# wvangansbeke/LaneDetection_End2End

Hardware: AMD Instinct MI355X
Metric: images/sec fwd+bwd, 256x512 2-lane bs32 (higher is better)
Workload: dtype f32; 1 GPU; BEV ERFNet + fused WLS fit + Area loss, 2 lanes, 256x512, batch 32 per GPU, fp32, train mode (BN batch stats, Dropout2d on), fwd+bwd, optimizer excluded; global_batch=32, parallelism=dp1, grad_allreduce=none

## Files before the change

### lanedetection_end2end_amd/_lib.py

```python
import ctypes
import os
from ctypes import c_char_p, c_double, c_int, c_long, c_size_t, c_void_p

import torch

_HERE = os.path.dirname(os.path.abspath(__file__))
LIB_PATH = os.path.join(_HERE, "liblanefit_hip.so")
_lib = None


class LaneFitLibraryError(RuntimeError):
    pass


def _declare(lib):
    P, I, L, D = c_void_p, c_int, c_long, c_double
    sig = {
        "lf_abi_version": (c_int, []),
        "lf_last_error": (c_char_p, []),
        "lf_wls_workspace_bytes": (c_size_t, [I, I, I]),
        "lf_wls_fwd": (I, [P, P, L, I, I, I, I, I, I, D, D, I, I, P, P, P, P, P, P]),
        "lf_wls_bwd": (I, [P, P, L, I, I, I, I, I, I, D, I, P, P, P, P, P]),
        "lf_gels_workspace_bytes": (c_size_t, [I, I]),
        "lf_gels_fwd": (I, [P, P, I, L, I, P, P, P, P, P]),
        "lf_gels_bwd": (I, [P, P, P, P, P, I, L, I, P, P, P]),
        "lf_area_loss": (I, [P, L, P, I, I, I, I, P, P, P]),
        "lf_mse_loss": (I, [P, P, L, I, P, P, P]),
        "lf_backproj_loss": (I, [P, L, P, P, P, P, P, I, I, I, P, P, P, P]),
        "lf_ce2d_fwd": (I, [P, P, P, I, I, I, I, P, P, P]),
        "lf_ce2d_bwd": (I, [P, P, P, I, I, I, I, P, P, P, P]),
        "lf_erfnet_plan_create": (P, [I, I, I, I, I, I]),
        "lf_erfnet_plan_destroy": (None, [P]),
        "lf_erfnet_workspace_bytes": (c_size_t, [P]),
        "lf_erfnet_workspace_bytes_for": (c_size_t, [P, I]),
        "lf_erfnet_activation_floats": (L, [P]),
        "lf_erfnet_num_params": (I, [P]),
        "lf_erfnet_num_bn": (I, [P]),
        "lf_erfnet_num_dropout": (I, [P]),
        "lf_erfnet_dropmask_floats": (L, [P]),
        "lf_erfnet_dropmask_offset": (L, [P, I]),
        "lf_erfnet_dropmask_channels": (I, [P, I]),
        "lf_erfnet_encoder_offset": (L, [P]),
        "lf_erfnet_activation_offset": (L, [P, I, I]),
        "lf_erfnet_bn_vector_offset": (L, [P, I, I, I]),
        "lf_erfnet_forward": (I, [P, P, P, P, P, P, I, I, P, P, c_size_t, P]),
        "lf_erfnet_backward": (I, [P, P, P, P, P, P, P, I, I, P, c_size_t, P]),
        "lf_convchain_plan_create": (P, [I, I, I, I, P, P]),
        "lf_convchain_plan_destroy": (None, [P]),
        "lf_convchain_workspace_bytes": (c_size_t, [P]),
        "lf_convchain_forward": (I, [P, P, P, P, P, I, ctypes.c_float, ctypes.c_float, P, P, c_size_t, P]),
        "lf_convchain_backward": (I, [P, P, P, P, P, P, P, I, P, c_size_t, P]),
        "lf_poolflat_fwd": (I, [P, I, I, I, I, I, P, P]),
        "lf_poolflat_bwd": (I, [P, P, I, I, I, I, I, P, P]),
        "lf_convchain_workspace_bytes_for": (c_size_t, [P, I]),
        "lf_convchain_set_precision": (I, [P, I]),
        "lf_poolflat_bf16_fwd": (I, [P, I, I, I, I, I, P, P]),
        "lf_poolflat_bf16_bwd": (I, [P, P, I, I, I, I, I, P, P]),
        "lf_lane_decode": (I, [P, P, P, P, D, P, P, D, D, D, I, I, I, I, P, P, P]),
        "lf_trapezoid": (I, [P, P, I, D, D, I, I, P, P]),
        "lf_pipeline_plan_create": (P, [I, I, I, I, I, I]),
        "lf_pipeline_plan_destroy": (None, [P]),
        "lf_pipeline_table_bytes": (c_size_t, [P]),
        "lf_pipeline_upload": (I, [P, P, P]),
        "lf_pipeline_tables_host": (I, [P, P, P, P, P, P, P, P, P]),
        "lf_pipeline_image": (I, [P, P, I, P, P, P, P]),
        "lf_pipeline_label": (I, [P, P, I, P, P, I, P, P, P, P]),
        "lf_pipeline_image_indexed": (I, [P, P, L, P, I, P, P, P, P, P]),
        "lf_pipeline_label_indexed": (I, [P, P, L, P, I, P, P, I, P, P, P, P, P]),
        "lf_nhwc_to_nchw": (I, [P, P, I, I, I, I, P]),
        "lf_pointwise_fwd": (I, [P, P, P, P, I, I, I, I, I, P]),
        "lf_pointwise_scratch_floats": (L, [I, I, I, I, I]),
        "lf_pointwise_bwd": (I, [P, P, P, P, P, P, I, I, I, I, I, P, P]),
        "lf_pointwise_bf16_fwd": (I, [P, P, P, P, I, I, I, I, I, P]),
        "lf_pointwise_bf16_bwd": (I, [P, P, P, P, P, P, I, I, I, I, I, P, P]),
        "lf_adam_chunk": (I, []),
        "lf_adam_step": (I, [P, P, I, ctypes.c_float, ctypes.c_float, ctypes.c_float, ctypes.c_float, ctypes.c_float,
                             I, ctypes.c_float, P]),
        "lf_sgd_step": (I, [P, P, I, ctypes.c_float, ctypes.c_float, ctypes.c_float, ctypes.c_float, P]),
        "lf_rmsprop_step": (I, [P, P, I, ctypes.c_float, ctypes.c_float, ctypes.c_float, ctypes.c_float, ctypes.c_float,
                                ctypes.c_float, P]),
        "lf_conv1d_scratch_floats": (L, [I, I, I, I]),
        "lf_conv1d_fwd": (I, [P, P, P, P, I, I, I, I, I, I, I, P, P]),
        "lf_conv1d_bwd_data": (I, [P, P, P, P, I, I, I, I, I, I, P, P]),
        "lf_conv1d_bwd_weight": (I, [P, P, P, P, I, I, I, I, I, I, P, P]),
        "lf_erfnet_num_layers": (I, [P]),
        "lf_erfnet_range_workspace_bytes": (c_size_t, [P, I, I]),
        "lf_erfnet_layer_io": (I, [P, I, P]),
        "lf_erfnet_forward_range": (I, [P, I, I, I, P, P, P, P, P, I, P, P, c_size_t, P]),
        "lf_erfnet_backward_range": (I, [P, I, I, I, P, P, P, P, P, I, P, P, c_size_t, P]),
        "lf_linear_fwd": (I, [P, P, P, P, I, I, I, I, P]),
        "lf_linear_bwd": (I, [P, P, P, P, P, P, P, I, I, I, I, P]),
        "lf_seg_maps": (I, [P, P, P, I, I, I, I, I, I, P]),
        "lf_erfnet_set_precision": (I, [P, I]),
        "lf_erfnet_profile": (I, [P, I]),
        "lf_erfnet_profile_read": (I, [P, P, c_char_p]),
        "lf_erfnet_infer_workspace_bytes": (c_size_t, [P, I]),
        "lf_erfnet_infer_encoder_offset": (L, [P]),
        "lf_erfnet_infer": (I, [P, P, P, P, P, I, P, P, c_size_t, P]),
        "lf_erfnet_infer_range_workspace_bytes": (c_size_t, [P, I, I, I]),
        "lf_erfnet_infer_range": (I, [P, I, I, I, P, P, P, P, P, P, c_size_t, P]),
        "lf_convchain_infer_workspace_bytes": (c_size_t, [P, I]),
        "lf_convchain_infer": (I, [P, P, P, P, P, ctypes.c_float, P, P, c_size_t, P]),
        "lf_head_fit": (I, [P, I, P, P, P, L, I, I, I, I, I, I, D, D, I, I, P, P, P, P, P, P]),
        "lf_lane_infer_workspace_bytes": (c_size_t, [P, I, I, I]),
        "lf_lane_infer": (I, [P, P, P, P, P, P, L, I, I, D, D, I, I, P, P, P, P, c_size_t, P]),
        "lf_theta_grid": (I, [P, L, P, P, I, I, I, P, P]),
        "lf_theta_grid_bwd_workspace_bytes": (c_size_t, [I]),
        "lf_theta_grid_bwd": (I, [P, L, P, P, P, I, I, I, P, P, P]),
        "lf_wls_fwd_theta": (I, [P, P, L, P, P, I, I, I, I, I, I, D, D, I, I, P, P, P, P, P, P]),
        "lf_wls_bwd_theta_workspace_bytes": (c_size_t, [I, I]),
        "lf_wls_bwd_theta": (I, [P, P, L, P, P, I, I, I, I, I, I, D, I, P, P, P, P, P, P, P]),
        "lf_wls_bwd_grid": (I, [P, P, L, I, I, I, I, I, I, D, I, P, P, P, P, P]),
        "lf_lane_eval": (I, [P, P, P, P, P, P, L, P, I, I, I, I, I, D, D, P, P, P, P, P, P]),
        "lf_lane_decode_bev": (I, [P, I, P, P, P, P, L, P, P, I, D, P, P, I, I, I, I, I, I, I, I, I, I, P, P, P]),
        "lf_step_loss_workspace_bytes": (c_size_t, []),
        "lf_step_loss": (I, [I, I, I, I, I, I, I, P, L, I, P, P, L, I, P, P, P, P, P, P, P, I, D, D, P, P, P, P, P, P]),
        "lf_step_loss_bwd": (I, [P, I, L, L, P, P, P]),
        "lf_seg_step_workspace_bytes": (c_size_t, [I, I, I, I, I, I]),
        "lf_seg_step": (I, [P, P, P, P, L, P, I, I, I, I, I, I, I, D, D, I, P, P, P, P, P, P, P, P]),
        "lf_seg_step_bwd": (I, [P, L, P, P]),
        "lf_label_batch_bp": (I, [P, P, P, P, P, P, P, L, P, P, I, I, P, P, P, P, P, P, P, P, P]),
        "lf_label_batch_bev": (I, [P, P, P, P, P, L, P, P, I, P, P, P, P, P, P, P]),
    }
    dbg = {
        "lf_debug_set_split_any_size": (None, [I]),
        "lf_debug_set_bf16_lds": (None, [I]),
        "lf_debug_set_bf16_no_partial_fast": (None, [I]),
        "lf_debug_stride2_epi": (I, [I, I, P, P, P, P, I, P, P, P, P, I, I, I, I, I, P, P]),
        "lf_debug_stride2_wgrad_scratch_floats": (L, [I, I, I, I, I, I, I]),
        "lf_debug_stride2_wgrad": (I, [I, I, P, P, P, P, I, I, I, I, I, P, P]),
        "lf_debug_stem_wgrad_scratch_floats": (L, [I, I, I, I]),
        "lf_debug_stem_wgrad": (I, [I, P, P, P, P, I, I, I, I, P, P]),
        "lf_debug_head_wgrad_scratch_floats": (L, [I, I, I, I]),
        "lf_debug_head_wgrad": (I, [I, P, P, P, P, I, I, I, I, P, P]),
        "lf_debug_set_ops_precision": (None, [I]),
        "lf_debug_conv1d_fwd_phases": (I, [P, P, P, P, I, I, I, I, I, I, P, P, P]),
        "lf_debug_conv1d_wgrad_phases": (I, [P, P, I, I, I, I, I, I, P, P, P]),
        "lf_debug_conv1d_fwd_pro": (I, [P, P, P, P, P, P, I, I, I, I, I, I, P, P]),
        "lf_debug_set_wgrad_ro": (None, [I, I, I]),
        "lf_debug_set_fp32_stream": (None, [I, I]),
        "lf_debug_conv1d_bwd_data_epi3": (I, [P, P, P, P, P, P, P, I, I, I, I, I, I, P, P]),
        "lf_debug_conv1d_epi": (I, [P, P, P, P, I, I, P, P, P, P, P, P, I, I, I, I, I, I, P, P]),
        "lf_debug_conv1d_wgrad_pro": (I, [P, P, P, P, P, P, I, I, I, I, I, I, P, P]),
        "lf_debug_bias_residual_launches": (L, []),
        "lf_debug_partial_fast_launches": (L, []),
    }
    for table in (sig, dbg):
        for name, (res, args) in table.items():
            fn = getattr(lib, name)
            fn.restype = res
            fn.argtypes = args
    return sig


def exported_symbols():
    return list(_declare(load()).keys()) + list(_extra_symbols)


_extra_symbols = []


def load():
    global _lib
    if _lib is None:
        if not os.path.exists(LIB_PATH):
            raise LaneFitLibraryError(
                "%s not found: build it with `python -m lanedetection_end2end_amd.build` "
                "(there is no fallback path)" % LIB_PATH)
        lib = ctypes.CDLL(LIB_PATH)
        _declare(lib)
        _lib = lib
    return _lib


def check(rc, what):
    if rc != 0:
        raise LaneFitLibraryError("%s failed: %s" % (what, load().lf_last_error().decode()))


def ptr(t, rows=False):
    if t is None:
        return None
    if not t.is_cuda:
        raise LaneFitLibraryError("lanefit ops need tensors on the MI355X (got a %s tensor); "
                                  "there is no CPU path" % t.device)
    if rows:
        assert t.dim() == 2 and t.stride(1) == 1, "internal: tensor rows must be contiguous"
    else:
        assert t.is_contiguous(), "internal: tensor must be contiguous"
    return c_void_p(t.data_ptr())


def stream():
    return c_void_p(torch.cuda.current_stream().cuda_stream)


class DeferredRead:

    def __init__(self, t):
        if t.is_cuda:
            self.host = torch.empty(t.shape, dtype=t.dtype, pin_memory=True)
            self.host.copy_(t, non_blocking=True)
            self.event = torch.cuda.Event()
            self.event.record()
        else:
            self.host = t.detach().clone()
            self.event = None

    def ready(self):
        return self.event is None or self.event.query()

    def get(self):
        if self.event is not None:
            self.event.synchronize()
        return self.host
```

### lanedetection_end2end_amd/csrc/lf_conv.h

```cpp
#pragma once
#include "lf_common.h"

#define LF_MAX_TAPS 9
struct TapIdx { int v[LF_MAX_TAPS]; };

struct LfTapGeom {
    int N, Hl, Wl;
    int Hs, Ws, s_pix, s_choff;
    int ssh, ssw;
    int Hd, Wd, d_pix, d_choff;
    int dsh, dsw, dah, daw;
    int Cs, Cd;
    int ntaps;
    int tdh[LF_MAX_TAPS], tdw[LF_MAX_TAPS];
};

enum { LF_PRO_NONE = 0, LF_PRO_BNRELU = 1 };
enum {
    LF_EPI_RELU = 1,
    LF_EPI_MASK = 2,
    LF_EPI_ADD = 4,
    LF_EPI_STATS_SQ = 8,
    LF_EPI_MASKBN = 16,
    LF_EPI_STATS_XHAT = 32,
    LF_EPI_BIAS = 64
};

struct LfTapArgs {
    const float* src;
    const float* wp;
    int s16;
    const void* wp16;
    int split;
    const void* wp48;
    const float* bias;
    float* dst;
    const float* pro_sc;
    const float* pro_sh;
    const float* mask_src;
    const float* add_src;
    const float* aux;
    const float* msc;
    const float* msh;
    const float* asc;
    const float* ash;
    const float* dm;
    float* stats;
    int stats_ld;
    unsigned long long* dbg;
};

void lf_tapgemm_set_split_any_size(int v);
void lf_tapgemm_set_bf16_lds(int v);
void lf_tapgemm_set_bf16_no_partial_fast(int v);
long lf_tapgemm_partial_fast_launches();
void lf_tapgemm_set_fp32_stream(int mode, int max_workgroups);
int lf_tapgemm_stat_rows(const LfTapGeom& g);
int lf_tapgemm_stat_rows_for(const LfTapGeom& g, const LfTapArgs& a);
int lf_tapgemm_launch(const LfTapGeom& g, const LfTapArgs& a, int pro, int epi, hipStream_t st);
int lf_tapgemm_launch_unordered(const LfTapGeom& g, const LfTapArgs& a, int pro, int epi, hipStream_t st);

struct LfWgradArgs {
    const float* x;
    const float* g;
    const float* pro_sc;
    const float* pro_sh;
    int s16;
    int split;
    float* partial;
    float* bias_partial;
    unsigned long long* dbg = nullptr;
};
int lf_tapwgrad_splits(const LfTapGeom& g);
int lf_tapwgrad_splits_bound(const LfTapGeom& g, int s16);
int lf_tapwgrad_splits_for(const LfTapGeom& g, const LfWgradArgs& a, int pro);
int lf_tapwgrad_launch(const LfTapGeom& g, const LfWgradArgs& a, int pro, hipStream_t st);

bool lf_tapwgrad_ro_ok(const LfTapGeom& g, int s16);
int lf_tapwgrad_ro_rows_bound(const LfTapGeom& g);
int lf_tapwgrad_ro_rows(const LfTapGeom& g);
int lf_tapwgrad_ro_launch(const LfTapGeom& g, const LfWgradArgs& a, int pro, hipStream_t st);
void lf_tapwgrad_ro_set(int mode, int cap64, int cap128);

int lf_wgrad_reduce_launch(const float* partial, int splits, int ntaps, int Cs, int Cd, float* grad, long sk, long sn,
                           const int* tapidx_host, const float* bias_rows, int n_bias_rows, float* bias_grad,
                           int bias_accumulate, hipStream_t st);
#define LF_REDUCE_BATCH 32
struct LfReduceJob {
    const float* partial; float* grad; const float* bias_rows; float* bias_grad;
    long sk, sn;
    int splits, ntaps, Cs, Cd, n_bias_rows;
    int tapidx[LF_MAX_TAPS];
};
int lf_wgrad_reduce_batch_launch(const LfReduceJob* jobs_host, int njobs, hipStream_t st);
int lf_rows_reduce_launch(const float* rows, int nrows, int C, float* dst, int accumulate, hipStream_t st);

struct LfPackEntry {
    long src_off;
    long dst_off;
    int Kc, Nc, ntaps;
    long sk, sn;
    int tapidx[LF_MAX_TAPS];
    int param;
    long dst16_off;
};
int lf_pack_weights_launch(const LfPackEntry* entries_dev, int nentries, const float* const* params_dev, float* arena,
                           hipStream_t st);
long lf_pack_bf16_elems(int Kc, int Nc, int ntaps);
int lf_pack_weights_split_launch(const LfPackEntry* entries_dev, int nentries, const float* const* params_dev, void* arena48,
                                 hipStream_t st);
bool lf_tapgemm_split_ok(const LfTapGeom& g);
long lf_tapgemm_bias_residual_launches();

struct LfFoldEntry {
    LfPackEntry pk;
    int ch_off, C;
    const float* gamma;
    const float* beta;
    const float* mean;
    const float* var;
    const float* bias;
    long out_off;
};
int lf_fold_pack_launch(const LfFoldEntry* entries_dev, int nentries, const float* const* params_dev, float eps, float* vec, float* arena,
                        void* arena16, void* arena48, hipStream_t st);
int lf_pack_weights_bf16_launch(const LfPackEntry* entries_dev, int nentries, const float* const* params_dev, void* arena16,
                                hipStream_t st);
```

### lanedetection_end2end_amd/csrc/lf_conv.hip

```cpp
#include <stdlib.h>
#include <string.h>

#include <atomic>
#include <map>
#include <mutex>
#include <tuple>
#include <type_traits>
#include <utility>

#include <hip/hip_ext.h>

#include "lf_conv.h"
#include "lf_ldsdma.h"
#include "lf_types.h"

typedef float f32x4 __attribute__((ext_vector_type(4)));

namespace {

constexpr int MT = 4;
constexpr int WG_WAVES = 4;
constexpr int PIX_PER_WG = WG_WAVES * MT * 16;

__device__ __forceinline__ f32x4 ldg4(const float* p) { return *reinterpret_cast<const f32x4*>(p); }
// ... 1834 lines not shown
                const int sy = pi[m] * g.ssh + dh, sx = pj[m] * g.ssw + dw;
                in3[t][m] = pv[m] && sy >= 0 && sy < g.Hs && sx >= 0 && sx < g.Ws;
                const int syc = min(max(sy, 0), g.Hs - 1), sxc = min(max(sx, 0), g.Ws - 1);
                const unsigned off = (unsigned)(((pn[m] * g.Hs + syc) * g.Ws + sxc) * g.s_pix + g.s_choff + kq * 4) * 4u;
                x3[t][m] = ldb4(rxl, (PROC == 0 && !in3[t][m]) ? LF_OOB : off, 0u);
            }
        }
        f32x4 sc = zero4(), sh = zero4();
        if (pro == LF_PRO_BNRELU) { sc = ldg4(a.pro_sc + kq * 4); sh = ldg4(a.pro_sh + kq * 4); }
#pragma unroll
        for (int t = 0; t < 3; ++t) {
            if constexpr (PROC != 0) {
#pragma unroll
                for (int m = 0; m < MT; ++m) {
                    f32x4 v = x3[t][m];
                    if (pro == LF_PRO_BNRELU) v = max0(v * sc + sh);
                    v.x = in3[t][m] ? v.x : 0.f; v.y = in3[t][m] ? v.y : 0.f; v.z = in3[t][m] ? v.z : 0.f; v.w = in3[t][m] ? v.w : 0.f;
                    x3[t][m] = v;
                }
            }
            f32x4 part[NT][MT];
#pragma unroll
            for (int s4 = 0; s4 < 4; ++s4)
#pragma unroll
                for (int n = 0; n < NT; ++n)
#pragma unroll
                    for (int m = 0; m < MT; ++m)
                        part[n][m] = __builtin_amdgcn_mfma_f32_16x16x4f32(w3[t][n][s4], x3[t][m][s4], s4 ? part[n][m] : zero4(), 0, 0, 0);
#pragma unroll
            for (int n = 0; n < NT; ++n)
#pragma unroll
                for (int m = 0; m < MT; ++m) acc[n][m] = t ? acc[n][m] + part[n][m] : part[n][m];
        }
    } else
    for (int t = 0; t < g.ntaps; ++t) {
        const int dh = g.tdh[t], dw = g.tdw[t];
        unsigned xo[MT];
        bool in[MT];
#pragma unroll
        for (int m = 0; m < MT; ++m) {
            const int sy = pi[m] * g.ssh + dh, sx = pj[m] * g.ssw + dw;
            in[m] = pv[m] && sy >= 0 && sy < g.Hs && sx >= 0 && sx < g.Ws;
            const int syc = min(max(sy, 0), g.Hs - 1), sxc = min(max(sx, 0), g.Ws - 1);
            xo[m] = (unsigned)(((pn[m] * g.Hs + syc) * g.Ws + sxc) * g.s_pix + g.s_choff + kq * 4);
        }
        for (int cg = 0; cg < ncg; ++cg) {
            f32x4 w[NT], x[MT];
#pragma unroll
            for (int n = 0; n < NT; ++n) w[n] = ldg4(wp + n * 64);
            wp += (long)g.Cd * 16;
#pragma unroll
            for (int m = 0; m < MT; ++m) x[m] = ldg4(a.src + xo[m] + cg * 16);
            if (pro == LF_PRO_BNRELU) {
                const f32x4 sc = ldg4(a.pro_sc + cg * 16 + kq * 4), sh = ldg4(a.pro_sh + cg * 16 + kq * 4);
#pragma unroll
                for (int m = 0; m < MT; ++m) x[m] = max0(x[m] * sc + sh);
            }
#pragma unroll
            for (int m = 0; m < MT; ++m) {
                x[m].x = in[m] ? x[m].x : 0.f; x[m].y = in[m] ? x[m].y : 0.f;
                x[m].z = in[m] ? x[m].z : 0.f; x[m].w = in[m] ? x[m].w : 0.f;
            }
            if ((cg & 1) == 0) {
#pragma unroll
                for (int n = 0; n < NT; ++n)
#pragma unroll
                    for (int m = 0; m < MT; ++m) { acc[n][m] += seg[n][m]; seg[n][m] = zero4(); }
            }
#pragma unroll
            for (int s = 0; s < 4; ++s)
#pragma unroll
                for (int n = 0; n < NT; ++n)
#pragma unroll
                    for (int m = 0; m < MT; ++m)
                        seg[n][m] = __builtin_amdgcn_mfma_f32_16x16x4f32(w[n][s], x[m][s], seg[n][m], 0, 0, 0);
        }
    }
    if (!(g.Cs == 16 && g.ntaps == 3)) {
#pragma unroll
        for (int n = 0; n < NT; ++n)
#pragma unroll
            for (int m = 0; m < MT; ++m) acc[n][m] += seg[n][m];
    }
    LF_TAPGEMM_EPILOGUE
}

int g_split_any_size = 0;
std::atomic<long> g_bres_launches{0};
int g_bf16_lds = 4;
std::atomic<long> g_part_fast_launches{0};
int g_bf16_no_partial_fast = 0;

int pick_nt(int Cd) {
    const int tiles = Cd / 16;
    if (tiles % 4 == 0) return 4;
    if (tiles % 3 == 0) return 3;
    if (tiles % 2 == 0) return 2;
    return 1;
}

}

void lf_tapgemm_set_split_any_size(int v) { g_split_any_size = v; }
long lf_tapgemm_bias_residual_launches() { return g_bres_launches.load(); }
void lf_tapgemm_set_bf16_lds(int v) { g_bf16_lds = v; }
void lf_tapgemm_set_bf16_no_partial_fast(int v) { g_bf16_no_partial_fast = v; }
long lf_tapgemm_partial_fast_launches() { return g_part_fast_launches.load(); }

bool lf_tapgemm_split_ok(const LfTapGeom& g) {
    const long npix = (long)g.N * g.Hl * g.Wl;
    const long wgs = npix / (2 * PIX_PER_WG) * (g.Cd / 64);
    return g.Cs % 32 == 0 && g.Cd % 64 == 0 && g.s_pix % 4 == 0 && g.s_choff % 4 == 0 && npix % (2 * PIX_PER_WG) == 0 &&
           (wgs >= 192 || g_split_any_size);
}

int lf_tapgemm_stat_rows(const LfTapGeom& g) {
    const long npix = (long)g.N * g.Hl * g.Wl;
    return lf_cdiv(npix, PIX_PER_WG);
}
int lf_tapgemm_stat_rows_for(const LfTapGeom& g, const LfTapArgs& a) {
    (void)a;
    return lf_cdiv((long)g.N * g.Hl * g.Wl, PIX_PER_WG);
}

namespace {
std::mutex g_launch_state_mutex;
int current_device() {
    int dev = 0;
    return hipGetDevice(&dev) == hipSuccess ? dev : -1;
}
template <typename K>
int resident_workgroups(K kernel, size_t lds, int block = 256) {
    static std::map<std::tuple<int, const void*, size_t>, int> cache;
    const int dev = current_device();
    const std::tuple<int, const void*, size_t> key(dev, reinterpret_cast<const void*>(kernel), lds);
    std::lock_guard<std::mutex> lock(g_launch_state_mutex);
    auto it = cache.find(key);
    if (it != cache.end()) return it->second;
    int cus = 0, nb = 0;
    if (dev < 0 || hipDeviceGetAttribute(&cus, hipDeviceAttributeMultiprocessorCount, dev) != hipSuccess ||
        hipOccupancyMaxActiveBlocksPerMultiprocessor(&nb, kernel, block, lds) != hipSuccess || nb < 1 || cus < 1)
        return cache[key] = 1 << 30;
    return cache[key] = nb * cus;
}
bool allow_big_lds(const void* kernel, int bytes) {
    static std::map<std::pair<int, const void*>, bool> done;
    const std::pair<int, const void*> key(current_device(), kernel);
    std::lock_guard<std::mutex> lock(g_launch_state_mutex);
    auto it = done.find(key);
    if (it != done.end()) return it->second;
    return done[key] = hipFuncSetAttribute(kernel, hipFuncAttributeMaxDynamicSharedMemorySize, bytes) == hipSuccess;
}
thread_local unsigned g_launch_flags = 0;
template <typename K, typename... Args>
bool launch_resident(K kernel, dim3 grid, unsigned block, size_t lds, int lds_attr, unsigned max_wgs, unsigned flags, hipStream_t st, const Args&... args) {
    if (lds_attr > 0 && !allow_big_lds(reinterpret_cast<const void*>(kernel), lds_attr)) return false;
    const unsigned res = (unsigned)resident_workgroups(kernel, lds, (int)block) / grid.y;
    if (grid.x > res && res >= 8) grid.x = res & ~7u;
    if (max_wgs > 0 && grid.x > max_wgs) grid.x = max_wgs;
    if (flags) hipExtLaunchKernelGGL(kernel, grid, dim3(block), (unsigned)lds, st, nullptr, nullptr, flags, args...);
    else hipLaunchKernelGGL(kernel, grid, dim3(block), lds, st, args...);
    return true;
}
constexpr int BIG_LDS = 160 * 1024 - 4096;
template <typename K>
void launch_tapgemm(K kernel, dim3 grid, size_t lds, hipStream_t st, const LfTapGeom& g, const LfTapArgs& a, int pro, int epi) {
    launch_resident(kernel, grid, 256, lds, 0, 0, g_launch_flags, st, g, a, pro, epi);
}
template <int EPIV, bool DBGV = false>
void launch_bf16_ring(unsigned nitems, hipStream_t st, const LfTapGeom& g, const LfTapArgs& a, int pro, int epi) {
    launch_resident(tapgemm_bf16_ring_kernel<EPIV, DBGV>, dim3(nitems), 256, (size_t)LB_STAGES * LB_STAGE_BYTES, 0, 0, 0, st, g, a, pro, epi);
}
template <int CBV, int EPIV, int PROV = 0>
bool launch_bf16_wl(unsigned nitems, hipStream_t st, const LfTapGeom& g, const LfTapArgs& a, int pro, int epi) {
    return launch_resident(tapgemm_bf16_wl_kernel<CBV, EPIV, PROV>, dim3(nitems), 256, WlCfg<CBV, EPIV, PROV>::LDS, BIG_LDS, 0, 0, st, g, a, pro, epi);
}
template <int EPIV>
bool launch_bf16_wv(unsigned ntiles, hipStream_t st, const LfTapGeom& g, const LfTapArgs& a, int pro, int epi) {
    return launch_resident(tapgemm_bf16_wv_kernel<EPIV>, dim3(ntiles), 256, WvCfg<EPIV>::LDS, BIG_LDS, 0, 0, st, g, a, pro, epi);
}
std::atomic<int> g_stream_mode{1}, g_stream_cap{0};
enum { LF_STREAM_RELU = 1, LF_STREAM_STATS = 2, LF_STREAM_MASK = 4, LF_STREAM_PRO = 8, LF_STREAM_X48 = 16, LF_STREAM_X38 = 32 };
constexpr int g_stream_routed[2] = {LF_STREAM_RELU | LF_STREAM_STATS | LF_STREAM_MASK | LF_STREAM_PRO | LF_STREAM_X48 | LF_STREAM_X38,
                                    0};
template <int CS, int PROV, int EPIV>
bool launch_tapstream(hipStream_t st, const LfTapGeom& g, const LfTapArgs& a) {
    constexpr int G = CS == 128 ? 2 : 1;
    const size_t lds = (size_t)3 * (CS / 16) * 4096 + (PROV == LF_PRO_BNRELU ? 2 * CS * sizeof(float) : 0);
    const unsigned ntiles = (unsigned)lf_cdiv((long)g.N * g.Hl * g.Wl, PIX_PER_WG);
    return launch_resident(tapstream_kernel<CS, PROV, EPIV, G>, dim3((ntiles + G - 1) / G, CS / 64), 256 * G, lds, BIG_LDS,
                           (unsigned)g_stream_cap.load(), g_launch_flags, st, g, a);
}
template <int CS>
bool route_tapstream(int variant, hipStream_t st, const LfTapGeom& g, const LfTapArgs& a) {
    switch (variant) {
        case LF_STREAM_RELU: return launch_tapstream<CS, 0, LF_EPI_RELU>(st, g, a);
        case LF_STREAM_STATS: return launch_tapstream<CS, 0, LF_EPI_STATS_SQ>(st, g, a);
        case LF_STREAM_MASK: return launch_tapstream<CS, 0, LF_EPI_MASK>(st, g, a);
        case LF_STREAM_PRO: return launch_tapstream<CS, 1, LF_EPI_RELU>(st, g, a);
        case LF_STREAM_X48: if constexpr (CS == 64) return launch_tapstream<CS, 0, LF_EPI_MASKBN | LF_EPI_STATS_XHAT>(st, g, a); else return false;
        case LF_STREAM_X38: if constexpr (CS == 64) return launch_tapstream<CS, 0, LF_EPI_ADD | LF_EPI_MASK | LF_EPI_STATS_XHAT>(st, g, a); else return false;
        default: return false;
    }
}

constexpr int BRES = LF_EPI_ADD | LF_EPI_RELU | LF_EPI_BIAS;
template <int V> using IntC = std::integral_constant<int, V>;
template <bool WITH_BRES, typename F>
auto with_epi(int epis, F&& f) {
    switch (epis) {
        case 0: return f(IntC<0>{});
        case LF_EPI_RELU: return f(IntC<LF_EPI_RELU>{});
        case LF_EPI_MASK: return f(IntC<LF_EPI_MASK>{});
        case LF_EPI_ADD: return f(IntC<LF_EPI_ADD>{});
        case LF_EPI_STATS_SQ: return f(IntC<LF_EPI_STATS_SQ>{});
        case LF_EPI_MASK | LF_EPI_STATS_XHAT: return f(IntC<LF_EPI_MASK | LF_EPI_STATS_XHAT>{});
        case LF_EPI_ADD | LF_EPI_MASK | LF_EPI_STATS_XHAT: return f(IntC<LF_EPI_ADD | LF_EPI_MASK | LF_EPI_STATS_XHAT>{});
        case LF_EPI_MASKBN | LF_EPI_STATS_XHAT: return f(IntC<LF_EPI_MASKBN | LF_EPI_STATS_XHAT>{});
        case BRES: return f(IntC<WITH_BRES ? BRES : -1>{});
        default: return f(IntC<-1>{});
    }
}
template <bool WITH_BRES, typename F>
void with_pro_epi(int pro, int epi, int epis, F&& f) {
    if (pro == LF_PRO_BNRELU && epi == LF_EPI_RELU) f(IntC<1>{}, IntC<LF_EPI_RELU>{});
    else if (pro == LF_PRO_BNRELU) f(IntC<1>{}, IntC<-1>{});
    else with_epi<WITH_BRES>(epis, [&](auto e) { f(IntC<0>{}, e); });
}

int launch_split_route(const LfTapGeom& g, const LfTapArgs& a, int pro, int epi, int epis, long npix, hipStream_t st) {
    LF_REQUIRE(a.split == 9, "tapgemm: split must be 9 (got %d; the 6-term form was removed in round 6)", a.split);
    LfTapArgs b = a;
    b.wp16 = a.wp48;
    const dim3 grid2((unsigned)(npix / (2 * PIX_PER_WG)), g.Cd / 64);
    if (a.dbg) {
        LF_REQUIRE(pro == LF_PRO_NONE && epi == 0, "tapgemm: phase stamps are compiled into the plain convolution only");
        hipLaunchKernelGGL((tapgemm_split_kernel<4, 0, 0, true>), grid2, dim3(512), 0, st, g, b, pro, epi);
    } else {
        with_pro_epi<false>(pro, epi, epis, [&](auto p, auto e) {
            hipLaunchKernelGGL((tapgemm_split_kernel<4, decltype(p)::value, decltype(e)::value>), grid2, dim3(512), 0, st, g, b, pro, epi);
        });
    }
    LF_CHECK_LAUNCH("tapgemm_split");
    return 0;
}

template <int NTV, int PROV, int EPIV = -1, bool FAST = false>
void launch_bf16_stream(dim3 grid, hipStream_t st, const LfTapGeom& g, const LfTapArgs& a, int pro, int epi) {
    hipLaunchKernelGGL((tapgemm_bf16_kernel<NTV, PROV, EPIV, FAST>), grid, dim3(256), 0, st, g, a, pro, epi);
}
template <int NTV>
void launch_bf16_stream_rt(dim3 grid, hipStream_t st, const LfTapGeom& g, const LfTapArgs& a, int pro, int epi) {
    if (pro == LF_PRO_BNRELU) launch_bf16_stream<NTV, 1>(grid, st, g, a, pro, epi);
    else launch_bf16_stream<NTV, 0>(grid, st, g, a, pro, epi);
}

int launch_bf16_route(const LfTapGeom& g, const LfTapArgs& a, int pro, int epi, int epis, long npix, int nt, dim3 grid, hipStream_t st) {
    LF_REQUIRE(a.s16, "tapgemm: the bf16 matrix-core kernels take bf16 tensors (s16); bf16 operands on fp32 tensors were removed in round 6");
    LF_REQUIRE(g.Cs >= 8 && g.s_pix >= g.s_choff + 8, "tapgemm bf16: needs at least 8 source channels");
    const bool in_offsets = (long)g.N * g.Hs * g.Ws * g.s_pix * 2 < (long)LF_OOB;
    if (a.s16 && g_bf16_lds >= 3 && !a.dbg && g.Cs == 16 && g.Cd == 16 && g.ntaps == 3 && g.Wl % 16 == 0 && g.s_pix % 8 == 0 && g.s_choff % 8 == 0 && in_offsets) {
        with_epi<true>(epis, [&](auto e) {
            constexpr int E = decltype(e)::value;
            if (pro == LF_PRO_BNRELU) hipLaunchKernelGGL((tapgemm_bf16_lean_kernel<1, E>), grid, dim3(256), 0, st, g, a, pro, epi);
            else hipLaunchKernelGGL((tapgemm_bf16_lean_kernel<0, E>), grid, dim3(256), 0, st, g, a, pro, epi);
        });
        if (epis == BRES) ++g_bres_launches;
        LF_CHECK_LAUNCH("tapgemm_bf16_lean");
        return 0;
    }
    const bool fast16 = nt == 4 && a.s16 && pro != LF_PRO_BNRELU && g.Cs % 32 == 0 && in_offsets;
    const bool fast16p = nt == 4 && a.s16 && pro == LF_PRO_BNRELU && epi == LF_EPI_RELU && g.Cs == 128 && in_offsets;
    const bool line3 = g_bf16_lds >= 3 && !a.dbg && g.ntaps == 3 && g.Cs == g.Cd && (g.Cd == 64 || g.Cd == 128) && g.Wl % 16 == 0 &&
                       g.ssh == 1 && g.ssw == 1 && g.dsh == 1 && g.dsw == 1 && g.dah == 0 && g.daw == 0 && g.Hs == g.Hl && g.Ws == g.Wl &&
                       g.Hd == g.Hl && g.Wd == g.Wl && g.s_pix % 8 == 0 && g.s_choff % 8 == 0 && g.d_pix % 8 == 0 && g.d_choff % 8 == 0 &&
                       (long)g.N * g.Hd * g.Wd * g.d_pix * 2 < (long)LF_OOB;
    const bool wv = line3 && g_bf16_lds == 4 && g.Cd == 64 && fast16;
    const bool wl = line3 && (fast16 || fast16p);
    const unsigned ntiles = (unsigned)lf_cdiv(npix, PIX_PER_WG);
    if (wv) {
        const bool launched = with_epi<true>(epis, [&](auto e) {
            constexpr int E = decltype(e)::value;
            if constexpr (E == (LF_EPI_ADD | LF_EPI_MASK | LF_EPI_STATS_XHAT)) return false;
            else return launch_bf16_wv<E>(ntiles, st, g, a, pro, epi);
        });
        if (launched) {
            if (epis == BRES) ++g_bres_launches;
            LF_CHECK_LAUNCH("tapgemm_bf16_wv");
            return 0;
        }
    }
    if (wl && fast16p) {
        if (launch_bf16_wl<4, LF_EPI_RELU, 1>(ntiles, st, g, a, pro, epi)) {
            LF_CHECK_LAUNCH("tapgemm_bf16_wl (prologue)");
            return 0;
        }
    } else if (wl) {
        const bool launched = with_epi<true>(epis, [&](auto e) {
            constexpr int E = decltype(e)::value;
            return g.Cs == 128 ? launch_bf16_wl<4, E>(ntiles, st, g, a, pro, epi) : launch_bf16_wl<2, E>(ntiles, st, g, a, pro, epi);
        });
        if (launched) {
            if (epis == BRES) ++g_bres_launches;
            LF_CHECK_LAUNCH("tapgemm_bf16_wl");
            return 0;
        }
    }
    const bool part_fast = !g_bf16_no_partial_fast && g.ntaps * ((g.Cs + 31) / 32) <= LF_MAX_TAPS;
    const bool ring = fast16 && g_bf16_lds >= 2 && g.Wl % 16 == 0 && g.Cd % 64 == 0;
    const unsigned nitems = ntiles * (unsigned)(g.Cd / 64);
    if (ring && a.dbg) {
        LF_REQUIRE(epis == 0, "tapgemm bf16 ring: stamps are compiled into the plain convolution only");
        launch_bf16_ring<0, true>(nitems, st, g, a, pro, epi);
    } else if (ring) {
        with_epi<false>(epis, [&](auto e) { launch_bf16_ring<decltype(e)::value>(nitems, st, g, a, pro, epi); });
    } else if (fast16) {
        with_epi<false>(epis, [&](auto e) { launch_bf16_stream<4, 0, decltype(e)::value, true>(grid, st, g, a, pro, epi); });
    } else if (nt == 4 && a.s16 && pro != LF_PRO_BNRELU && g.Cs == 16 && (epis == (LF_EPI_MASK | LF_EPI_STATS_XHAT) || epis == 0) && part_fast && in_offsets) {
        if (epis == 0) launch_bf16_stream<4, 0, 0, true>(grid, st, g, a, pro, epi);
        else launch_bf16_stream<4, 0, LF_EPI_MASK | LF_EPI_STATS_XHAT, true>(grid, st, g, a, pro, epi);
        ++g_part_fast_launches;
    } else if (nt == 3 && a.s16 && pro != LF_PRO_BNRELU && g.Cs == 16 && (epis == LF_EPI_STATS_SQ || epis == LF_EPI_RELU || epis == 0) && part_fast && in_offsets) {
        if (epis == 0) launch_bf16_stream<3, 0, 0, true>(grid, st, g, a, pro, epi);
        else if (epis == LF_EPI_RELU) launch_bf16_stream<3, 0, LF_EPI_RELU, true>(grid, st, g, a, pro, epi);
        else launch_bf16_stream<3, 0, LF_EPI_STATS_SQ, true>(grid, st, g, a, pro, epi);
        ++g_part_fast_launches;
    } else if (nt == 4 && a.s16 && pro == LF_PRO_BNRELU && epi == LF_EPI_RELU) {
        launch_bf16_stream<4, 1, LF_EPI_RELU, false>(grid, st, g, a, pro, epi);
    } else if (nt == 1 && a.s16 && pro != LF_PRO_BNRELU && ((g.Cs + 31) / 32 * 32 + g.s_choff <= g.s_pix) && in_offsets &&
               (g.Cs % 32 == 0 || part_fast) &&
               (epis == 0 || epis == LF_EPI_STATS_SQ || epis == LF_EPI_ADD || epis == LF_EPI_RELU)) {
        if (epis == 0) launch_bf16_stream<1, 0, 0, true>(grid, st, g, a, pro, epi);
        else if (epis == LF_EPI_STATS_SQ) launch_bf16_stream<1, 0, LF_EPI_STATS_SQ, true>(grid, st, g, a, pro, epi);
        else if (epis == LF_EPI_RELU) launch_bf16_stream<1, 0, LF_EPI_RELU, true>(grid, st, g, a, pro, epi);
        else launch_bf16_stream<1, 0, LF_EPI_ADD, true>(grid, st, g, a, pro, epi);
        if (g.Cs % 32 != 0) ++g_part_fast_launches;
    } else {
        switch (nt) {
            case 4: launch_bf16_stream_rt<4>(grid, st, g, a, pro, epi); break;
            case 3: launch_bf16_stream_rt<3>(grid, st, g, a, pro, epi); break;
            case 2: launch_bf16_stream_rt<2>(grid, st, g, a, pro, epi); break;
            default: launch_bf16_stream_rt<1>(grid, st, g, a, pro, epi); break;
        }
    }
    LF_CHECK_LAUNCH("tapgemm_bf16");
    return 0;
}

template <int NTV>
void launch_tapgemm_rt(dim3 grid, size_t tap_lds, hipStream_t st, const LfTapGeom& g, const LfTapArgs& a, int pro, int epi) {
    if (pro == LF_PRO_BNRELU) launch_tapgemm(tapgemm_kernel<NTV, 1>, grid, tap_lds, st, g, a, pro, epi);
    else launch_tapgemm(tapgemm_kernel<NTV, 0>, grid, tap_lds, st, g, a, pro, epi);
}

int launch_fp32_route(const LfTapGeom& g, const LfTapArgs& a, int pro, int epi, int epis, int nt, dim3 grid, hipStream_t st) {
    const size_t tap_lds = LF_TAP_LDS_PER_TAP * g.ntaps;
    if (a.dbg) {
        LF_REQUIRE(nt == 4 && pro == LF_PRO_NONE && epi == 0 && !a.wp16, "tapgemm: phase stamps are compiled into the plain fp32 convolution only");
        if ((g.Wl & 63) == 0) hipLaunchKernelGGL((tapgemm_kernel<4, 0, 0, true, true>), grid, dim3(256), tap_lds, st, g, a, pro, epi);
        else hipLaunchKernelGGL((tapgemm_kernel<4, 0, 0, false, true>), grid, dim3(256), tap_lds, st, g, a, pro, epi);
        LF_CHECK_LAUNCH("tapgemm (stamps)");
        return 0;
    }
    if (g_stream_mode.load() != 0 && nt == 4 && g.ntaps == 3 && g.Cs == g.Cd && (g.Cs == 64 || g.Cs == 128) && (g.Wl & 63) == 0) {
        const int variant = pro == LF_PRO_BNRELU ? (epi == LF_EPI_RELU ? LF_STREAM_PRO : 0)
                          : epis == LF_EPI_RELU ? LF_STREAM_RELU : epis == LF_EPI_STATS_SQ ? LF_STREAM_STATS : epis == LF_EPI_MASK ? LF_STREAM_MASK
                          : epis == (LF_EPI_MASKBN | LF_EPI_STATS_XHAT) ? LF_STREAM_X48 : epis == (LF_EPI_ADD | LF_EPI_MASK | LF_EPI_STATS_XHAT) ? LF_STREAM_X38 : 0;
        if (variant && (g_stream_mode.load() == 2 || (g_stream_routed[g.Cs == 128] & variant)) &&
            (g.Cs == 64 ? route_tapstream<64>(variant, st, g, a) : route_tapstream<128>(variant, st, g, a))) {
            LF_CHECK_LAUNCH("tapstream");
            return 0;
        }
    }
    switch (nt) {
        case 4:
            with_pro_epi<true>(pro, epi, epis, [&](auto p, auto e) {
                constexpr int P = decltype(p)::value, E = decltype(e)::value;
                if ((g.Wl & 63) == 0) launch_tapgemm(tapgemm_kernel<4, P, E, true>, grid, tap_lds, st, g, a, pro, epi);
                else launch_tapgemm(tapgemm_kernel<4, P, E, false>, grid, tap_lds, st, g, a, pro, epi);
                if constexpr (E == BRES) ++g_bres_launches;
            });
            break;
        case 3: launch_tapgemm_rt<3>(grid, tap_lds, st, g, a, pro, epi); break;
        case 2: launch_tapgemm_rt<2>(grid, tap_lds, st, g, a, pro, epi); break;
        default:
            with_pro_epi<true>(pro, epi, epis, [&](auto p, auto e) {
                constexpr int P = decltype(p)::value, E = decltype(e)::value;
                hipLaunchKernelGGL((tapgemm_lean_kernel<1, P, E>), grid, dim3(256), 0, st, g, a, pro, epi);
                if constexpr (E == BRES) ++g_bres_launches;
            });
            break;
    }
    LF_CHECK_LAUNCH("tapgemm");
    return 0;
}
}

void lf_tapgemm_set_fp32_stream(int mode, int max_workgroups) { g_stream_mode = mode; g_stream_cap = max_workgroups > 0 ? max_workgroups : 0; }

int lf_tapgemm_launch_unordered(const LfTapGeom& g, const LfTapArgs& a, int pro, int epi, hipStream_t st) {
    g_launch_flags = hipExtAnyOrderLaunch;
    const int rc = lf_tapgemm_launch(g, a, pro, epi, st);
    g_launch_flags = 0;
    return rc;
}

int lf_tapgemm_launch(const LfTapGeom& g, const LfTapArgs& a, int pro, int epi, hipStream_t st) {
    LF_REQUIRE(g.Cs % 16 == 0 && g.Cd % 16 == 0, "tapgemm: channels must be multiples of 16 (Cs=%d Cd=%d)", g.Cs, g.Cd);
    LF_REQUIRE(g.s_pix % 4 == 0 && g.s_choff % 4 == 0 && g.d_pix % 4 == 0 && g.d_choff % 4 == 0, "tapgemm: unaligned channel layout");
    LF_REQUIRE(g.ntaps >= 1 && g.ntaps <= LF_MAX_TAPS, "tapgemm: bad tap count %d", g.ntaps);
    const long npix = (long)g.N * g.Hl * g.Wl;
    LF_REQUIRE(npix < (1L << 30), "tapgemm: too many pixels (%ld)", npix);
    const int nt = pick_nt(g.Cd);
    const dim3 grid(lf_cdiv(npix, PIX_PER_WG), g.Cd / (16 * nt));
    LF_REQUIRE((long)g.N * g.Hs * g.Ws * g.s_pix * 4 < (long)LF_OOB, "tapgemm: source tensor too large for 32-bit byte offsets");
    LF_REQUIRE((long)g.N * g.Hd * g.Wd * g.d_pix * 4 < (long)LF_OOB, "tapgemm: destination tensor too large for 32-bit byte offsets");
    const int epis = (epi == (LF_EPI_ADD | LF_EPI_RELU) && a.bias) ? BRES
                   : ((epi & (LF_EPI_MASK | LF_EPI_ADD | LF_EPI_MASKBN | LF_EPI_STATS_XHAT)) && a.bias) ? -2 : epi;
    LF_REQUIRE(!a.s16 || a.wp16, "tapgemm: bf16 tensors need the bf16 matrix-core kernel (wp16)");
    if (a.split && a.wp48 && !a.wp16 && lf_tapgemm_split_ok(g)) return launch_split_route(g, a, pro, epi, epis, npix, st);
    LF_REQUIRE(!a.s16 || (g.s_pix % 8 == 0 && g.s_choff % 8 == 0), "tapgemm: bf16 source layout must be 16-byte aligned per pixel");
    if (a.wp16) return launch_bf16_route(g, a, pro, epi, epis, npix, nt, grid, st);
    return launch_fp32_route(g, a, pro, epi, epis, nt, grid, st);
}

namespace {

template <bool S16>
__device__ __forceinline__ f32x4 wg_ld4(__amdgpu_buffer_rsrc_t r, unsigned off) { return epi_ld<S16>(r, off); }
template <bool S16>
__device__ __forceinline__ float wg_ld1(__amdgpu_buffer_rsrc_t r, unsigned off, unsigned soff = 0u) {
    if constexpr (S16) return __uint_as_float((unsigned)__builtin_amdgcn_raw_buffer_load_b16(r, (int)(off * 2u), (int)(soff * 2u), 0) << 16);
    else return __builtin_bit_cast(float, __builtin_amdgcn_raw_buffer_load_b32(r, (int)(off * 4u), (int)(soff * 4u), 0));
}
__device__ __forceinline__ uint2 wg_ldraw(__amdgpu_buffer_rsrc_t r, unsigned off) {
    return __builtin_bit_cast(uint2, __builtin_amdgcn_raw_buffer_load_b64(r, (int)(off * 2u), 0, 0));
}

typedef short s16x4 __attribute__((ext_vector_type(4)));

template <bool XV, bool GV, int XT, int GT, int U, bool S16, bool BFM = false, int PROT = -1, bool DBG = false>
__global__ __launch_bounds__(256, 2) void tapwgrad_kernel(const LfTapGeom g, const LfWgradArgs a, const int pro_rt,
                                                      const long pps, const int write_bias, const int gxs) {
    constexpr int XTiles = XV ? 4 : XT, GTiles = GV ? 4 : GT;
    const int pro = PROT >= 0 ? (PROT ? LF_PRO_BNRELU : LF_PRO_NONE) : pro_rt;
    constexpr int XB = XTiles * 16, GB = GTiles * 16;
    const int lane = threadIdx.x & 63, wave = threadIdx.x >> 6;
    const int pl = lane & 15, kq = lane >> 4;
    unsigned long long tstamp[4] = {0ull, 0ull, 0ull, 0ull};
    if constexpr (DBG) tstamp[0] = __builtin_amdgcn_s_memrealtime();
    const int ncob = g.Cd / GB;
    unsigned ord = blockIdx.x;
    if ((gridDim.x & 7u) == 0) ord = (ord & 7u) * (gridDim.x >> 3) + (ord >> 3);
    const unsigned nz = (unsigned)((g.Cs / XB) * ncob);
    const int t = (int)(ord % (unsigned)g.ntaps);
    const int bz = (int)((ord / (unsigned)g.ntaps) % nz);
    const unsigned bxs = ord / ((unsigned)g.ntaps * nz);
    (void)gxs;
    const int cib = bz / ncob, cob = bz % ncob;
    const long npix = (long)g.N * g.Hl * g.Wl;
    const int wave_u = __builtin_amdgcn_readfirstlane(wave);
    const long sub = (long)bxs * WG_WAVES + wave_u;
    const long p_begin = sub * pps;
    long p_end = p_begin + pps;
    if (p_end > npix) p_end = npix;
    const int niter = p_end > p_begin ? (int)((p_end - p_begin) / (4 * U)) : 0;

    f32x4 acc[XTiles][GTiles];
#pragma unroll
    for (int r = 0; r < XTiles; ++r)
#pragma unroll
        for (int q = 0; q < GTiles; ++q) acc[r][q] = zero4();
    float bsum[GTiles];
#pragma unroll
    for (int q = 0; q < GTiles; ++q) bsum[q] = 0.f;

    int pj, pi, pn;
    {
        const unsigned q = niter ? (unsigned)p_begin : 0u;
        const unsigned r = q / (unsigned)g.Wl;
        pj = (int)(q - r * (unsigned)g.Wl);
        pn = (int)(r / (unsigned)g.Hl);
        pi = (int)(r - (unsigned)pn * (unsigned)g.Hl);
        pj = __builtin_amdgcn_readfirstlane(pj); pi = __builtin_amdgcn_readfirstlane(pi); pn = __builtin_amdgcn_readfirstlane(pn);
    }
    const int dh = g.tdh[t], dw = g.tdw[t];
    const int xch = g.s_choff + cib * XB + (XV ? 4 * pl : pl);
    const int gch = g.d_choff + cob * GB + (GV ? 4 * pl : pl);
    const __amdgpu_buffer_rsrc_t rx = make_rsrc(a.x, (unsigned)((long)g.N * g.Hs * g.Ws * g.s_pix << (S16 ? 1 : 2))),
                                 rg = make_rsrc(a.g, (unsigned)((long)g.N * g.Hd * g.Wd * g.d_pix << (S16 ? 1 : 2)));
    f32x4 psc, psh;
    float psc1[XTiles], psh1[XTiles];
    if (pro == LF_PRO_BNRELU) {
        if constexpr (XV) { psc = ldg4(a.pro_sc + cib * XB + 4 * pl); psh = ldg4(a.pro_sh + cib * XB + 4 * pl); }
        else {
#pragma unroll
            for (int r = 0; r < XTiles; ++r) { psc1[r] = a.pro_sc[cib * XB + r * 16 + pl]; psh1[r] = a.pro_sh[cib * XB + r * 16 + pl]; }
        }
    }

    const unsigned gvoff = (unsigned)(kq * g.dsw * g.d_pix + gch), gstep = (unsigned)(4 * g.dsw * g.d_pix);
    const unsigned xvoff = (unsigned)(kq * g.ssw * g.s_pix + xch), xstep = (unsigned)(4 * g.ssw * g.s_pix);
    constexpr unsigned ESH = S16 ? 1 : 2;
    static_assert(!BFM || (S16 && XV && GV && U == 4), "BFM needs bf16 tensors, vector mode, U = 4");
    struct WStep {
        uint2 xr[BFM ? U : 1], gr[BFM ? U : 1];
        f32x4 x4[XV ? U : 1], g4[GV ? U : 1];
        float xs[XV ? 1 : U][XTiles], gs[GV ? 1 : U][GTiles];
        unsigned xmask;
    };
    constexpr unsigned OOBE = LF_OOB >> ESH;
    auto ldx = [&](WStep& S, int u, unsigned voff, unsigned soff) __attribute__((always_inline)) {
        if constexpr (BFM) S.xr[u] = __builtin_bit_cast(uint2, __builtin_amdgcn_raw_buffer_load_b64(rx, (int)(voff << 1), (int)(soff << 1), 0));
        else if constexpr (XV) {
            if constexpr (S16) S.x4[u] = epi_ld<true>(rx, voff, soff);
            else S.x4[u] = ldb4(rx, voff << 2, soff << 2);
        } else {
#pragma unroll
            for (int r = 0; r < XTiles; ++r) S.xs[u][r] = wg_ld1<S16>(rx, voff + r * 16, soff);
        }
    };
    auto wload = [&](WStep& S) __attribute__((always_inline)) {
        const unsigned gso = (unsigned)(((pn * g.Hd + pi * g.dsh + g.dah) * g.Wd + pj * g.dsw + g.daw) * g.d_pix);
#pragma unroll
        for (int u = 0; u < U; ++u) {
            const unsigned so = gso + u * gstep;
            if constexpr (BFM) S.gr[u] = __builtin_bit_cast(uint2, __builtin_amdgcn_raw_buffer_load_b64(rg, (int)(gvoff << 1), (int)(so << 1), 0));
            else if constexpr (GV) {
                if constexpr (S16) S.g4[u] = epi_ld<true>(rg, gvoff, so);
                else S.g4[u] = ldb4(rg, gvoff << 2, so << 2);
            } else {
#pragma unroll
                for (int q = 0; q < GTiles; ++q) S.gs[u][q] = wg_ld1<S16>(rg, gvoff + q * 16, so);
            }
        }
        const int sy = pi * g.ssh + dh;
        const bool yin = sy >= 0 && sy < g.Hs;
        const int sx0 = pj * g.ssw + dw, sxl = sx0 + (4 * U - 1) * g.ssw;
        if (yin && sx0 >= 0 && sxl < g.Ws) {
            const unsigned xso = (unsigned)(((pn * g.Hs + sy) * g.Ws + sx0) * g.s_pix);
#pragma unroll
            for (int u = 0; u < U; ++u) ldx(S, u, xvoff, xso + u * xstep);
            S.xmask = 0xfu;
        } else {
            const int syc = min(max(sy, 0), g.Hs - 1);
            const unsigned xso = (unsigned)((pn * g.Hs + syc) * g.Ws * g.s_pix);
            unsigned xm = 0;
#pragma unroll
            for (int u = 0; u < U; ++u) {
                const int sx = sx0 + (kq + 4 * u) * g.ssw;
                const bool in = yin && sx >= 0 && sx < g.Ws;
                xm |= (in ? 1u : 0u) << u;
                const unsigned oc = (unsigned)(min(max(sx, 0), g.Ws - 1) * g.s_pix + xch);
                ldx(S, u, (in || pro == LF_PRO_BNRELU) ? oc : OOBE, xso);
            }
            S.xmask = xm;
        }
    };
// ... 447 lines not shown
    long p_end = p_begin + pps;
    if (p_end > npix) p_end = npix;
    const int niter = p_end > p_begin ? (int)((p_end - p_begin + 15) / 16) : 0;
    f32x4 acc[NTAPS];
#pragma unroll
    for (int t = 0; t < NTAPS; ++t) acc[t] = zero4();
    float bsum = 0.f;
    const i32x4s rx = make_rsrc_words(a.x, (unsigned)min((long)g.N * g.Hs * g.Ws * g.s_pix * 4, (long)LF_OOB)),
                 rg = make_rsrc_words(a.g, (unsigned)min((long)g.N * g.Hd * g.Wd * g.d_pix * 4, (long)LF_OOB));
    const unsigned lds0 = (unsigned)(size_t)(__attribute__((address_space(3))) unsigned char*)lf_tap_lds + (unsigned)(wave * W16F_STAGES * W16F_STAGE);
    typedef __attribute__((address_space(3))) float* lds_f32_p;
    lds_f32_p const frag = (lds_f32_p)((__attribute__((address_space(3))) unsigned char*)lf_tap_lds + wave * W16F_STAGES * W16F_STAGE + kq * 64 + pl * 4);
    const int tdh0 = g.tdh[0], tdh1 = g.tdh[1], tdh2 = g.tdh[2], tdw0 = g.tdw[0], tdw1 = g.tdw[1], tdw2 = g.tdw[2];
    long p_ld = p_begin;
    int pj, pi, pn;
    {
        const unsigned q = niter ? (unsigned)p_begin : 0u;
        const unsigned r = q / (unsigned)g.Wl;
        pj = __builtin_amdgcn_readfirstlane((int)(q - r * (unsigned)g.Wl));
        pn = __builtin_amdgcn_readfirstlane((int)(r / (unsigned)g.Hl));
        pi = __builtin_amdgcn_readfirstlane((int)r) - pn * g.Hl;
    }
    int cj = pj, ci = pi;
    const int px = lane >> 2, chunk = lane & 3;
    auto issue = [&](const int slot) __attribute__((always_inline)) {
        const bool ok = p_ld < p_end;
        const int j = pj + px;
        const unsigned dst = lds0 + (unsigned)(slot * W16F_STAGE);
        const unsigned go = (unsigned)((((pn * g.Hd + pi * g.dsh + g.dah) * g.Wd + j * g.dsw + g.daw) * g.d_pix + g.d_choff + chunk * 4) * 4);
        lds_dma16(rg, dst, ok ? go : LF_OOB, 0u);
#pragma unroll
        for (int t = 0; t < NTAPS; ++t) {
            const int dh = t == 0 ? tdh0 : t == 1 ? tdh1 : tdh2, dw = t == 0 ? tdw0 : t == 1 ? tdw1 : tdw2;
            const int sy = pi * g.ssh + dh, sx = j * g.ssw + dw;
            const bool in = ok && sy >= 0 && sy < g.Hs && sx >= 0 && sx < g.Ws;
            const unsigned xo = (unsigned)((((pn * g.Hs + sy) * g.Ws + sx) * g.s_pix + g.s_choff + chunk * 4) * 4);
            lds_dma16(rx, dst + (unsigned)((1 + t) * 1024), in ? xo : LF_OOB, 0u);
        }
        p_ld += 16;
        pj += 16;
        if (pj >= g.Wl) { pj = 0; if (++pi >= g.Hl) { pi = 0; ++pn; } }
    };
    float psc = 1.f, psh = 0.f;
    if constexpr (PRO) {
        psc = a.pro_sc[pl]; psh = a.pro_sh[pl];
        asm volatile("" ::"v"(psc), "v"(psh) : "memory");
    }
#pragma unroll
    for (int q = 0; q < W16F_STAGES - 1; ++q) issue(q);
    for (int it0 = 0; it0 < niter; it0 += W16F_STAGES) {
#pragma unroll
        for (int sl = 0; sl < W16F_STAGES; ++sl) {
            if (it0 + sl >= niter) break;
            asm volatile("s_waitcnt vmcnt(8) lgkmcnt(0)" ::: "memory");
            issue((sl + W16F_STAGES - 1) % W16F_STAGES);
            float gv[4], xv[NTAPS][4];
#pragma unroll
            for (int u = 0; u < 4; ++u) {
                gv[u] = frag[(sl * W16F_STAGE + u * 256) / 4];
#pragma unroll
                for (int t = 0; t < NTAPS; ++t) xv[t][u] = frag[(sl * W16F_STAGE + (1 + t) * 1024 + u * 256) / 4];
            }
            if constexpr (PRO) {
#pragma unroll
                for (int t = 0; t < NTAPS; ++t) {
                    const int dh = t == 0 ? tdh0 : t == 1 ? tdh1 : tdh2, dw = t == 0 ? tdw0 : t == 1 ? tdw1 : tdw2;
                    const bool rowok = (unsigned)(ci * g.ssh + dh) < (unsigned)g.Hs;
                    const int c0 = cj * g.ssw + dw;
                    const bool edge = c0 < 0 || c0 + 15 * g.ssw >= g.Ws;
#pragma unroll
                    for (int u = 0; u < 4; ++u) {
                        float v = fmaxf(xv[t][u] * psc + psh, 0.f);
                        if (edge) v = (unsigned)(c0 + (4 * u + kq) * g.ssw) < (unsigned)g.Ws ? v : 0.f;
                        xv[t][u] = rowok ? v : 0.f;
                    }
                }
                cj += 16;
                if (cj >= g.Wl) { cj = 0; if (++ci >= g.Hl) ci = 0; }
            }
#pragma unroll
            for (int u = 0; u < 4; ++u) {
#pragma unroll
                for (int t = 0; t < NTAPS; ++t) acc[t] = __builtin_amdgcn_mfma_f32_16x16x4f32(xv[t][u], gv[u], acc[t], 0, 0, 0);
                bsum += gv[u];
            }
        }
    }
    asm volatile("s_waitcnt vmcnt(0)" ::: "memory");
    __shared__ float red[WG_WAVES - 1][NTAPS * 4][64];
    __shared__ float bred[WG_WAVES][64];
    if (wave > 0) {
#pragma unroll
        for (int t = 0; t < NTAPS; ++t)
#pragma unroll
            for (int e = 0; e < 4; ++e) red[wave - 1][t * 4 + e][lane] = acc[t][e];
    }
    bred[wave][lane] = bsum;
    __syncthreads();
    if (wave == 0) {
#pragma unroll
        for (int t = 0; t < NTAPS; ++t) {
            float* out = a.partial + ((long)blockIdx.x * NTAPS + t) * g.Cs * g.Cd;
#pragma unroll
            for (int e = 0; e < 4; ++e) {
                float v = acc[t][e];
#pragma unroll
                for (int w = 0; w < WG_WAVES - 1; ++w) v += red[w][t * 4 + e][lane];
                out[(long)(4 * kq + e) * g.Cd + pl] = v;
            }
        }
        if (write_bias && a.bias_partial) {
            float v = bred[0][lane] + bred[1][lane] + bred[2][lane] + bred[3][lane];
            v += __shfl_xor(v, 16, 64);
            v += __shfl_xor(v, 32, 64);
            if (kq == 0) a.bias_partial[(long)blockIdx.x * g.Cd + pl] = v;
        }
    }
}

struct WgradCfg { int xv, gv, xt, gt, gx, u; long pps; };

WgradCfg wgrad_cfg(const LfTapGeom& g) {
    WgradCfg c;
    c.xv = (g.Cs % 64 == 0);
    c.gv = (g.Cd % 64 == 0);
    c.xt = c.xv ? 4 : g.Cs / 16;
    c.gt = c.gv ? 4 : g.Cd / 16;
    const int xb = c.xt * 16, gb = c.gt * 16;
    const bool small16 = (g.Cs == 16 && g.Cd == 16 && g.ntaps == 3 && g.Wl % 16 == 0);
    const int jobs = small16 ? 1 : g.ntaps * (g.Cs / xb) * (g.Cd / gb);
    const long npix = (long)g.N * g.Hl * g.Wl;
    int gx = (small16 ? 4096 : 2048) / (jobs * WG_WAVES);
    if (gx < 1) gx = 1;
    const long maxgx = (npix + 64 * WG_WAVES - 1) / (64 * WG_WAVES);
    if (gx > maxgx) gx = (int)maxgx;
    if (gx < 1) gx = 1;
    if (!small16) {
        int mlt = 8;
        for (int d = 2; d <= 8; d *= 2) if (jobs % d == 0) mlt = 8 / d;
        if (gx >= mlt) gx = gx / mlt * mlt;
    }
    c.u = (g.Wl % 16 == 0) ? 4 : 1;
    const int gran = 4 * c.u;
    long pps = (npix + (long)gx * WG_WAVES - 1) / ((long)gx * WG_WAVES);
    pps = (pps + gran - 1) / gran * gran;
    c.gx = (int)((npix + pps * WG_WAVES - 1) / (pps * WG_WAVES));
    c.pps = pps;
    return c;
}

template <bool XV, bool GV, int XT, int GT>
void launch_wgrad(const LfTapGeom& g, const LfWgradArgs& a, int pro, const WgradCfg& c, dim3 grid, int wb, hipStream_t st) {
    constexpr bool VV = XV && GV;
    auto go = [&](auto kern) { hipLaunchKernelGGL(kern, grid, dim3(256), 0, st, g, a, pro, c.pps, wb, c.gx); };
    if (a.s16 && c.u == 4 && VV) go(tapwgrad_kernel<XV, GV, XT, GT, 4, true, VV>);
    else if (a.s16 && c.u == 4) go(tapwgrad_kernel<XV, GV, XT, GT, 4, true>);
    else if (a.s16) go(tapwgrad_kernel<XV, GV, XT, GT, 1, true>);
    else if (c.u == 4 && VV) {
        if constexpr (VV) {
            if (pro == LF_PRO_BNRELU) go(tapwgrad_kernel<XV, GV, XT, GT, 4, false, false, 1>);
            else go(tapwgrad_kernel<XV, GV, XT, GT, 4, false, false, 0>);
        }
    } else if (c.u == 4) go(tapwgrad_kernel<XV, GV, XT, GT, 4, false>);
    else go(tapwgrad_kernel<XV, GV, XT, GT, 1, false>);
}

}

int lf_tapwgrad_splits(const LfTapGeom& g) { return wgrad_cfg(g).gx; }
int lf_tapwgrad_splits_bound(const LfTapGeom& g, int s16) {
    const int a = lf_tapwgrad_splits(g), c = s16 ? lf_tapwgrad_ro_rows_bound(g) : 0;
    return a > c ? a : c;
}
int lf_tapwgrad_splits_for(const LfTapGeom& g, const LfWgradArgs& a, int pro) {
    if (lf_tapwgrad_ro_ok(g, a.s16) && !a.dbg) return lf_tapwgrad_ro_rows(g);
    (void)pro;
    return wgrad_cfg(g).gx;
}

int lf_tapwgrad_launch(const LfTapGeom& g, const LfWgradArgs& a, int pro, hipStream_t st) {
    LF_REQUIRE(g.Cs % 16 == 0 && g.Cd % 16 == 0, "tapwgrad: channels must be multiples of 16");
    LF_REQUIRE(g.Wl % 4 == 0, "tapwgrad: logical width %d must be a multiple of 4", g.Wl);
    LF_REQUIRE((long)g.N * g.Hs * g.Ws * g.s_pix < (long)(LF_OOB >> 2) && (long)g.N * g.Hd * g.Wd * g.d_pix < (long)(LF_OOB >> 2),
               "tapwgrad: tensor too large for 32-bit byte offsets");
    if (lf_tapwgrad_ro_ok(g, a.s16) && !a.dbg) return lf_tapwgrad_ro_launch(g, a, pro, st);
    const int wb = a.bias_partial != nullptr;
    const WgradCfg c = wgrad_cfg(g);
    const int xb = c.xt * 16, gb = c.gt * 16;
    if (g.Cs == 16 && g.Cd == 16 && g.ntaps == 3 && g.Wl % 16 == 0) {
        const bool ring_ok = g_bf16_lds >= 3 && g.s_pix % 8 == 0 && g.s_choff % 8 == 0 && g.d_pix % 8 == 0 && g.d_choff % 8 == 0 &&
                             (long)g.N * g.Hs * g.Ws * g.s_pix * (a.s16 ? 2 : 4) < (long)LF_OOB && (long)g.N * g.Hd * g.Wd * g.d_pix * (a.s16 ? 2 : 4) < (long)LF_OOB;
        const size_t ring_lds = (size_t)WG_WAVES * W16_STAGES * W16_STAGE;
        static_assert(W16F_STAGES * W16F_STAGE == W16_STAGES * W16_STAGE, "the two 16-channel rings share their LDS budget");
        const bool pr = pro == LF_PRO_BNRELU;
        auto ring = [&](auto kern) {
            if (!allow_big_lds(reinterpret_cast<const void*>(kern), 128 * 1024)) return false;
            hipLaunchKernelGGL(kern, dim3(c.gx), dim3(256), ring_lds, st, g, a, c.pps, wb);
            return true;
        };
        bool launched = false;
        if (ring_ok && a.s16) launched = pr ? ring(tapwgrad16_tr_kernel<true>) : ring(tapwgrad16_tr_kernel<false>);
        else if (ring_ok) launched = pr ? ring(tapwgrad16_f32_kernel<true>) : ring(tapwgrad16_f32_kernel<false>);
        if (!launched) {
            if (a.s16) hipLaunchKernelGGL((tapwgrad16_kernel<3, true>), dim3(c.gx), dim3(256), 0, st, g, a, pro, c.pps, wb);
            else hipLaunchKernelGGL((tapwgrad16_kernel<3, false>), dim3(c.gx), dim3(256), 0, st, g, a, pro, c.pps, wb);
        }
        LF_CHECK_LAUNCH("tapwgrad16");
        return 0;
    }
    dim3 grid(c.gx * g.ntaps * (g.Cs / xb) * (g.Cd / gb));
    if (a.dbg) {
        LF_REQUIRE(c.xv && c.gv && c.u == 4 && !a.s16 && pro == LF_PRO_NONE, "tapwgrad: phase stamps are compiled into the plain fp32 kernel only");
        hipLaunchKernelGGL((tapwgrad_kernel<true, true, 4, 4, 4, false, false, 0, true>), grid, dim3(256), 0, st, g, a, pro, c.pps, wb, c.gx);
        LF_CHECK_LAUNCH("tapwgrad (stamps)");
        return 0;
    }
    if (c.xv && c.gv) launch_wgrad<true, true, 4, 4>(g, a, pro, c, grid, wb, st);
    else if (c.xv && c.gt == 1) launch_wgrad<true, false, 4, 1>(g, a, pro, c, grid, wb, st);
    else if (c.xv && c.gt == 3) launch_wgrad<true, false, 4, 3>(g, a, pro, c, grid, wb, st);
    else if (!c.xv && c.xt == 1 && c.gv) launch_wgrad<false, true, 1, 4>(g, a, pro, c, grid, wb, st);
    else if (!c.xv && c.xt == 1 && c.gt == 1) launch_wgrad<false, false, 1, 1>(g, a, pro, c, grid, wb, st);
    else if (!c.xv && c.xt == 1 && c.gt == 3) launch_wgrad<false, false, 1, 3>(g, a, pro, c, grid, wb, st);
    else if (!c.xv && c.xt == 3 && c.gt == 1) launch_wgrad<false, false, 3, 1>(g, a, pro, c, grid, wb, st);
    else if (!c.xv && c.xt == 3 && c.gv) launch_wgrad<false, true, 3, 4>(g, a, pro, c, grid, wb, st);
    else return lf_fail("tapwgrad: unsupported channel combination Cs=%d Cd=%d", g.Cs, g.Cd);
    LF_CHECK_LAUNCH("tapwgrad");
    return 0;
}

namespace {

__global__ __launch_bounds__(1024) void wgrad_reduce_kernel(const float* __restrict__ partial, int splits, int ntaps,
                                                           int Cs, int Cd, float* __restrict__ grad, long sk, long sn,
                                                           TapIdx ti, int wblocks, const float* __restrict__ brows,
                                                           int nbrows, float* __restrict__ bgrad, int baccum) {
    constexpr int SG = 16;
    __shared__ float sw[SG][64];
    const int og = threadIdx.x & 63, sg = threadIdx.x >> 6;
    if ((int)blockIdx.x >= wblocks) {
        const int c = (blockIdx.x - wblocks) * 64 + og;
        float s = 0.f;
        if (c < Cd)
            for (int r = sg; r < nbrows; r += SG) s += brows[(long)r * Cd + c];
        sw[sg][og] = s;
        __syncthreads();
        if (sg == 0 && c < Cd) {
            float v = 0.f;
#pragma unroll
            for (int k = 0; k < SG; ++k) v += sw[k][og];
            bgrad[c] = baccum ? bgrad[c] + v : v;
        }
        return;
    }
    const long per = (long)ntaps * Cs * Cd;
    for (long base = (long)blockIdx.x * 64; base < per; base += (long)wblocks * 64) {
        const long i = base + og;
        float s0 = 0.f, s1 = 0.f;
        if (i < per) {
            int r = sg;
            for (; r + SG < splits; r += 2 * SG) { s0 += partial[(long)r * per + i]; s1 += partial[(long)(r + SG) * per + i]; }
            for (; r < splits; r += SG) s0 += partial[(long)r * per + i];
        }
        sw[sg][og] = s0 + s1;
        __syncthreads();
        if (sg == 0 && i < per) {
            float v = 0.f;
#pragma unroll
            for (int k = 0; k < SG; ++k) v += sw[k][og];
            const int n = (int)(i % Cd);
            const long r2 = i / Cd;
            const int k2 = (int)(r2 % Cs), t = (int)(r2 / Cs);
            grad[k2 * sk + n * sn + ti.v[t]] = v;
        }
        __syncthreads();
    }
}

struct ReduceBatch { LfReduceJob j[LF_REDUCE_BATCH]; int blk0[LF_REDUCE_BATCH + 1]; };

__global__ __launch_bounds__(256) void wgrad_reduce_batch_kernel(const ReduceBatch B) {
    __shared__ float sw[4][64];
    int jb = 0;
    while (jb + 1 < LF_REDUCE_BATCH && (int)blockIdx.x >= B.blk0[jb + 1]) ++jb;
    const LfReduceJob& J = B.j[jb];
    const int blk = blockIdx.x - B.blk0[jb];
    const int og = threadIdx.x & 63, sg = threadIdx.x >> 6;
    const long per = (long)J.ntaps * J.Cs * J.Cd;
    const int wblocks = (int)((per + 63) / 64);
    const float* __restrict__ rows;
    long width, i;
    int nrows;
    if (blk < wblocks) { rows = J.partial; width = per; i = (long)blk * 64 + og; nrows = J.splits; }
    else { rows = J.bias_rows; width = J.Cd; i = (long)(blk - wblocks) * 64 + og; nrows = J.n_bias_rows; }
    float s0 = 0.f, s1 = 0.f, s2 = 0.f, s3 = 0.f;
    if (i < width) {
        int r = sg;
        for (; r + 12 < nrows; r += 16) {
            s0 += rows[(long)r * width + i]; s1 += rows[(long)(r + 4) * width + i];
            s2 += rows[(long)(r + 8) * width + i]; s3 += rows[(long)(r + 12) * width + i];
        }
        for (; r < nrows; r += 4) s0 += rows[(long)r * width + i];
    }
    sw[sg][og] = (s0 + s1) + (s2 + s3);
    __syncthreads();
    if (sg == 0 && i < width) {
        const float v = (sw[0][og] + sw[1][og]) + (sw[2][og] + sw[3][og]);
        if (blk < wblocks) {
            const int n = (int)(i % J.Cd);
            const long r2 = i / J.Cd;
            const int k2 = (int)(r2 % J.Cs), t = (int)(r2 / J.Cs);
            J.grad[k2 * J.sk + n * J.sn + J.tapidx[t]] = v;
        } else {
            J.bias_grad[i] = v;
        }
    }
}

__global__ __launch_bounds__(256) void rows_reduce_kernel(const float* __restrict__ rows, int nrows, int C,
                                                         float* __restrict__ dst, int accumulate) {
    const int c = blockIdx.x * 64 + (threadIdx.x & 63), rg = threadIdx.x >> 6;
    __shared__ float sb[4][64];
    float s0 = 0.f, s1 = 0.f;
    if (c < C) {
        int r = rg;
        for (; r + 4 < nrows; r += 8) { s0 += rows[(long)r * C + c]; s1 += rows[(long)(r + 4) * C + c]; }
        for (; r < nrows; r += 4) s0 += rows[(long)r * C + c];
    }
    sb[rg][threadIdx.x & 63] = s0 + s1;
    __syncthreads();
    if (rg == 0 && c < C) {
        const float v = (sb[0][threadIdx.x] + sb[1][threadIdx.x]) + (sb[2][threadIdx.x] + sb[3][threadIdx.x]);
        dst[c] = accumulate ? dst[c] + v : v;
    }
}

__global__ __launch_bounds__(256) void pack_weights_kernel(const LfPackEntry* __restrict__ entries,
                                                          const float* const* __restrict__ params,
                                                          float* __restrict__ arena) {
    const LfPackEntry e = entries[blockIdx.x];
    const float* w = params[e.param];
    float* dst = arena + e.dst_off;
    const unsigned total = (unsigned)(e.ntaps * e.Kc * e.Nc), Nc = (unsigned)e.Nc, kbn = (unsigned)(e.Kc >> 2);
    for (unsigned i = blockIdx.y * 256u + threadIdx.x; i < total; i += gridDim.y * 256u) {
        const unsigned k4 = i & 3u, r = i >> 2, r2 = r / Nc, n = r - r2 * Nc, t = r2 / kbn, kb = r2 - t * kbn;
        const unsigned k = kb * 4u + k4;
        dst[i] = w[(long)k * e.sk + (long)n * e.sn + e.tapidx[t]];
    }
}

__global__ __launch_bounds__(256) void pack_weights_bf16_kernel(const LfPackEntry* __restrict__ entries,
                                                               const float* const* __restrict__ params,
                                                               __bf16* __restrict__ arena) {
    const LfPackEntry e = entries[blockIdx.x];
    const float* w = params[e.param];
    __bf16* dst = arena + e.dst16_off;
    const int kb_per_tap = ((e.Kc + 31) >> 5) * 4;
    const unsigned total = (unsigned)(e.ntaps * kb_per_tap * e.Nc * 8), Nc = (unsigned)e.Nc, kbn = (unsigned)kb_per_tap;
    for (unsigned i = blockIdx.y * 256u + threadIdx.x; i < total; i += gridDim.y * 256u) {
        const unsigned k8 = i & 7u, r = i >> 3, r2 = r / Nc, n = r - r2 * Nc, t = r2 / kbn, kb = r2 - t * kbn;
        const int k = (int)(kb * 8u + k8);
        dst[i] = (__bf16)(k < e.Kc ? w[(long)k * e.sk + (long)n * e.sn + e.tapidx[t]] : 0.f);
    }
}

__global__ __launch_bounds__(256) void pack_weights_split_kernel(const LfPackEntry* __restrict__ entries,
                                                                const float* const* __restrict__ params,
                                                                __bf16* __restrict__ arena) {
    const LfPackEntry e = entries[blockIdx.x];
    if (e.Kc % 32 != 0) return;
    const float* w = params[e.param];
    __bf16* dst = arena + 3 * e.dst16_off;
    const int kb_per_tap = e.Kc >> 3;
    const long total = (long)e.ntaps * kb_per_tap * e.Nc * 8;
    for (long i = (long)blockIdx.y * 256 + threadIdx.x; i < total; i += (long)gridDim.y * 256) {
        const int k8 = (int)(i & 7);
        long r = i >> 3;
        const int n = (int)(r % e.Nc);
        const long row = r;
        r /= e.Nc;
        const int kb = (int)(r % kb_per_tap);
        const int t = (int)(r / kb_per_tap);
        const float v = w[(kb * 8 + k8) * e.sk + n * e.sn + e.tapidx[t]];
        const __bf16 vh = (__bf16)v;
        const float r1 = v - (float)vh;
        const __bf16 vm = (__bf16)r1;
        const float r2 = r1 - (float)vm;
        dst[row * 24 + k8] = vh; dst[row * 24 + 8 + k8] = vm; dst[row * 24 + 16 + k8] = (__bf16)r2;
    }
}

__device__ __forceinline__ double fold_scale(const LfFoldEntry& f, int n, float eps) {
    if (!f.gamma) return 1.0;
    const int c = f.ch_off + n;
    return (double)f.gamma[c] / sqrt((double)f.var[c] + (double)eps);
}
__device__ __forceinline__ float fold_w(const LfFoldEntry& f, const float* w, int k, int n, int t, float eps) {
    const float v = w[(long)k * f.pk.sk + (long)n * f.pk.sn + f.pk.tapidx[t]];
    return f.gamma ? (float)((double)v * fold_scale(f, n, eps)) : v;
}
__global__ __launch_bounds__(256) void fold_pack_kernel(const LfFoldEntry* __restrict__ entries, const float* const* __restrict__ params,
                                                       float eps, float* __restrict__ vec, float* __restrict__ arena, __bf16* __restrict__ arena16,
                                                       __bf16* __restrict__ arena48) {
    const LfFoldEntry f = entries[blockIdx.x];
    const LfPackEntry& e = f.pk;
    if (blockIdx.y == 0) {
        for (int n = threadIdx.x; n < f.C; n += 256) {
            const double s = fold_scale(f, n, eps);
            const int c = f.ch_off + n;
            float* out = vec + f.out_off;
            if (e.ntaps > 0) {
                out[n] = f.gamma ? (float)(((double)f.bias[n] - (double)f.mean[c]) * s + (double)f.beta[c]) : f.bias[n];
            } else {
                out[n] = (float)s;
                out[f.C + n] = (float)((double)f.beta[c] - (double)f.mean[c] * s);
            }
        }
    }
    if (e.ntaps == 0) return;
    const float* w = params[e.param];
    const unsigned Nc = (unsigned)e.Nc;
    if (arena) {
        float* dst = arena + e.dst_off;
        const unsigned total = (unsigned)(e.ntaps * e.Kc * e.Nc), kbn = (unsigned)(e.Kc >> 2);
        for (unsigned i = blockIdx.y * 256u + threadIdx.x; i < total; i += gridDim.y * 256u) {
            const unsigned k4 = i & 3u, r = i >> 2, r2 = r / Nc, n = r - r2 * Nc, t = r2 / kbn, kb = r2 - t * kbn;
            dst[i] = fold_w(f, w, (int)(kb * 4u + k4), (int)n, (int)t, eps);
        }
    }
    if (arena16) {
        __bf16* dst = arena16 + e.dst16_off;
        const unsigned kbn = (unsigned)(((e.Kc + 31) >> 5) * 4), total = (unsigned)e.ntaps * kbn * Nc * 8u;
        for (unsigned i = blockIdx.y * 256u + threadIdx.x; i < total; i += gridDim.y * 256u) {
            const unsigned k8 = i & 7u, r = i >> 3, r2 = r / Nc, n = r - r2 * Nc, t = r2 / kbn, kb = r2 - t * kbn;
            const int k = (int)(kb * 8u + k8);
            dst[i] = (__bf16)(k < e.Kc ? fold_w(f, w, k, (int)n, (int)t, eps) : 0.f);
        }
    }
    if (arena48 && e.Kc % 32 == 0) {
        __bf16* dst = arena48 + 3 * e.dst16_off;
        const unsigned kbn = (unsigned)(e.Kc >> 3), total = (unsigned)e.ntaps * kbn * Nc * 8u;
        for (unsigned i = blockIdx.y * 256u + threadIdx.x; i < total; i += gridDim.y * 256u) {
            const unsigned k8 = i & 7u, row = i >> 3, r2 = row / Nc, n = row - r2 * Nc, t = r2 / kbn, kb = r2 - t * kbn;
            const float v = fold_w(f, w, (int)(kb * 8u + k8), (int)n, (int)t, eps);
            const __bf16 vh = (__bf16)v;
            const float r1 = v - (float)vh;
            const __bf16 vm = (__bf16)r1;
            dst[row * 24u + k8] = vh; dst[row * 24u + 8u + k8] = vm; dst[row * 24u + 16u + k8] = (__bf16)(r1 - (float)vm);
        }
    }
}

}

int lf_fold_pack_launch(const LfFoldEntry* entries_dev, int nentries, const float* const* params_dev, float eps, float* vec, float* arena,
                        void* arena16, void* arena48, hipStream_t st) {
    if (nentries <= 0) return 0;
    LF_REQUIRE(vec, "fold_pack: null vector region");
    hipLaunchKernelGGL(fold_pack_kernel, dim3(nentries, 16), dim3(256), 0, st, entries_dev, params_dev, eps, vec, arena,
                       reinterpret_cast<__bf16*>(arena16), reinterpret_cast<__bf16*>(arena48));
    LF_CHECK_LAUNCH("fold_pack");
    return 0;
}

int lf_wgrad_reduce_launch(const float* partial, int splits, int ntaps, int Cs, int Cd, float* grad, long sk, long sn,
                           const int* tapidx_host, const float* bias_rows, int n_bias_rows, float* bias_grad,
                           int bias_accumulate, hipStream_t st) {
    TapIdx ti;
    for (int i = 0; i < LF_MAX_TAPS; ++i) ti.v[i] = i < ntaps ? tapidx_host[i] : 0;
    const long per = (long)ntaps * Cs * Cd;
    int wblocks = lf_cdiv(per, 64);
    if (wblocks > 4096) wblocks = 4096;
    const int bblocks = (bias_rows && bias_grad) ? lf_cdiv(Cd, 64) : 0;
    hipLaunchKernelGGL(wgrad_reduce_kernel, dim3(wblocks + bblocks), dim3(1024), 0, st, partial, splits, ntaps, Cs, Cd, grad,
                       sk, sn, ti, wblocks, bias_rows, n_bias_rows, bias_grad, bias_accumulate);
    LF_CHECK_LAUNCH("wgrad_reduce");
    return 0;
}

int lf_wgrad_reduce_batch_launch(const LfReduceJob* jobs_host, int njobs, hipStream_t st) {
    for (int j0 = 0; j0 < njobs; j0 += LF_REDUCE_BATCH) {
        const int n = njobs - j0 < LF_REDUCE_BATCH ? njobs - j0 : LF_REDUCE_BATCH;
        ReduceBatch B;
        memset(&B, 0, sizeof(B));
        int blocks = 0;
        for (int i = 0; i < LF_REDUCE_BATCH; ++i) {
            B.blk0[i] = blocks;
            if (i >= n) continue;
            const LfReduceJob& J = jobs_host[j0 + i];
            B.j[i] = J;
            blocks += lf_cdiv((long)J.ntaps * J.Cs * J.Cd, 64) + ((J.bias_rows && J.bias_grad) ? lf_cdiv(J.Cd, 64) : 0);
        }
        B.blk0[LF_REDUCE_BATCH] = blocks;
        hipLaunchKernelGGL(wgrad_reduce_batch_kernel, dim3(blocks), dim3(256), 0, st, B);
        LF_CHECK_LAUNCH("wgrad_reduce_batch");
    }
    return 0;
}

int lf_rows_reduce_launch(const float* rows, int nrows, int C, float* dst, int accumulate, hipStream_t st) {
    hipLaunchKernelGGL(rows_reduce_kernel, dim3(lf_cdiv(C, 64)), dim3(256), 0, st, rows, nrows, C, dst, accumulate);
    LF_CHECK_LAUNCH("rows_reduce");
    return 0;
}

int lf_pack_weights_launch(const LfPackEntry* entries_dev, int nentries, const float* const* params_dev, float* arena,
                           hipStream_t st) {
    hipLaunchKernelGGL(pack_weights_kernel, dim3(nentries, 16), dim3(256), 0, st, entries_dev, params_dev, arena);
    LF_CHECK_LAUNCH("pack_weights");
    return 0;
}

int lf_pack_weights_bf16_launch(const LfPackEntry* entries_dev, int nentries, const float* const* params_dev, void* arena16,
                                hipStream_t st) {
    hipLaunchKernelGGL(pack_weights_bf16_kernel, dim3(nentries, 16), dim3(256), 0, st, entries_dev, params_dev,
                       reinterpret_cast<__bf16*>(arena16));
    LF_CHECK_LAUNCH("pack_weights_bf16");
    return 0;
}

int lf_pack_weights_split_launch(const LfPackEntry* entries_dev, int nentries, const float* const* params_dev, void* arena48,
                                 hipStream_t st) {
    hipLaunchKernelGGL(pack_weights_split_kernel, dim3(nentries, 16), dim3(256), 0, st, entries_dev, params_dev,
                       reinterpret_cast<__bf16*>(arena48));
    LF_CHECK_LAUNCH("pack_weights_split");
    return 0;
}

long lf_pack_bf16_elems(int Kc, int Nc, int ntaps) { return (long)ntaps * (((Kc + 31) >> 5) * 32) * Nc; }
```

### lanedetection_end2end_amd/csrc/lf_debug.h

```cpp
#pragma once
#ifdef __cplusplus
extern "C" {
#endif
void lf_debug_set_split_any_size(int v);
void lf_debug_set_bf16_lds(int v);
void lf_debug_set_bf16_no_partial_fast(int v);
long lf_debug_partial_fast_launches(void);
void lf_debug_set_ops_precision(int mode);
int lf_debug_conv1d_fwd_phases(const float* x, const float* w, const float* bias, float* y, int N, int H, int W, int C,
                               int axis, int dilation, float* scratch, unsigned long long* dbg, void* stream);
int lf_debug_conv1d_fwd_pro(const float* x, const float* w, const float* bias, const float* sc, const float* sh, float* y, int N, int H,
                            int W, int C, int axis, int dilation, float* scratch, void* stream);
void lf_debug_set_wgrad_ro(int mode, int cap64, int cap128);
void lf_debug_set_fp32_stream(int mode, int max_workgroups);
int lf_debug_conv1d_wgrad_pro(const float* x, const float* gy, const float* sc, const float* sh, float* gw, float* gb, int N, int H, int W,
                              int C, int axis, int dilation, float* scratch, void* stream);
int lf_debug_conv1d_bwd_data_epi3(const float* gy, const float* w, const float* mask_src, const float* add_src, const float* aux,
                                  float* gx, float* stats, int N, int H, int W, int C, int axis, int dilation, float* scratch, void* stream);
int lf_debug_conv1d_epi(const float* src, const float* w, const float* bias, float* dst, int transposed, int epi, const float* mask_src,
                        const float* add_src, const float* aux, const float* msc, const float* msh, float* stats, int N, int H, int W, int C,
                        int axis, int dilation, float* scratch, void* stream);
int lf_debug_stride2_epi(int kind, int phase, const float* src, const float* w, const float* bias, float* dst, int epi, const float* mask_src,
                         const float* add_src, const float* aux, float* stats, int N, int H, int W, int Cin, int Cout, float* scratch,
                         void* stream);
long lf_debug_stride2_wgrad_scratch_floats(int kind, int reduce, int N, int H, int W, int Cin, int Cout);
int lf_debug_stride2_wgrad(int kind, int reduce, const float* x, const float* g, float* gw, float* gb, int N, int H, int W, int Cin,
                           int Cout, float* scratch, void* stream);
long lf_debug_stem_wgrad_scratch_floats(int N, int Cin, int H, int W);
int lf_debug_stem_wgrad(int reduce, const float* img, const float* gcat, float* gw, float* gb, int N, int Cin, int H, int W, float* scratch,
                        void* stream);
long lf_debug_head_wgrad_scratch_floats(int N, int h, int w, int K);
int lf_debug_head_wgrad(int reduce, const float* x, const float* gout, float* gw, float* gb, int N, int h, int w, int K, float* scratch,
                        void* stream);
long lf_debug_bias_residual_launches(void);
int lf_debug_conv1d_wgrad_phases(const float* x, const float* gy, int N, int H, int W, int C, int axis, int dilation,
                                 float* scratch, unsigned long long* dbg, void* stream);
#ifdef __cplusplus
}
#endif
```

### lanedetection_end2end_amd/csrc/lf_eltwise.hip

```cpp
#include "lf_eltwise.h"
#include "lf_types.h"
#include "lf_plan.h"

typedef float f32x4 __attribute__((ext_vector_type(4)));

namespace {

__device__ __forceinline__ f32x4 ld4(const float* p) { return *reinterpret_cast<const f32x4*>(p); }
__device__ __forceinline__ void st4(float* p, f32x4 v) { *reinterpret_cast<f32x4*>(p) = v; }
__device__ __forceinline__ f32x4 z4() { f32x4 z = {0.f, 0.f, 0.f, 0.f}; return z; }
__device__ __forceinline__ f32x4 relu4(f32x4 v) {
    v.x = fmaxf(v.x, 0.f); v.y = fmaxf(v.y, 0.f); v.z = fmaxf(v.z, 0.f); v.w = fmaxf(v.w, 0.f); return v;
}
__device__ __forceinline__ f32x4 pos4(f32x4 v, f32x4 m) {
    v.x = m.x > 0.f ? v.x : 0.f; v.y = m.y > 0.f ? v.y : 0.f; v.z = m.z > 0.f ? v.z : 0.f; v.w = m.w > 0.f ? v.w : 0.f; return v;
}

template <int NQ>
__device__ __forceinline__ void block_reduce_quads(f32x4 (&a1)[NQ], f32x4 (&a2)[NQ], int U, float (*sm)[8 * NQ]) {
    const int tid = threadIdx.x;
#pragma unroll
    for (int q = 0; q < NQ; ++q) {
        sm[tid][8 * q + 0] = a1[q].x; sm[tid][8 * q + 1] = a1[q].y; sm[tid][8 * q + 2] = a1[q].z; sm[tid][8 * q + 3] = a1[q].w;
        sm[tid][8 * q + 4] = a2[q].x; sm[tid][8 * q + 5] = a2[q].y; sm[tid][8 * q + 6] = a2[q].z; sm[tid][8 * q + 7] = a2[q].w;
// ... 368 lines not shown
            for (int ci = 0; ci < 16; ++ci)
#pragma unroll
                for (int ab = 0; ab < 4; ++ab) o[ab] = fmaf(xv[ci], sw[(ci * K + k) * 4 + ab], o[ab]);
            float* op = out + (((long)n * K + k) * (2 * h) + 2 * i) * (2 * wd) + 2 * j;
            *reinterpret_cast<float2*>(op) = make_float2(o[0], o[1]);
            *reinterpret_cast<float2*>(op + 2 * wd) = make_float2(o[2], o[3]);
        }
    }
}

template <typename T>
__global__ __launch_bounds__(256) void head_bwd_data_kernel(const float* __restrict__ gout, const float* __restrict__ w,
                                                           T* __restrict__ gx, int N, int h, int wd, int K) {
    __shared__ float sw[16 * HEAD_MAXK * 4];
    for (int i = threadIdx.x; i < 16 * K * 4; i += 256) sw[i] = w[i];
    __syncthreads();
    const long npix = (long)N * h * wd;
    for (long p = (long)blockIdx.x * 256 + threadIdx.x; p < npix; p += (long)gridDim.x * 256) {
        const int j = (int)(p % wd);
        const long r = p / wd;
        const int i = (int)(r % h), n = (int)(r / h);
        float acc[16];
#pragma unroll
        for (int ci = 0; ci < 16; ++ci) acc[ci] = 0.f;
        for (int k = 0; k < K; ++k) {
            const float* gp = gout + (((long)n * K + k) * (2 * h) + 2 * i) * (2 * wd) + 2 * j;
            const float2 g0 = *reinterpret_cast<const float2*>(gp);
            const float2 g1 = *reinterpret_cast<const float2*>(gp + 2 * wd);
#pragma unroll
            for (int ci = 0; ci < 16; ++ci) {
                const float* wk = sw + (ci * K + k) * 4;
                acc[ci] = fmaf(g0.x, wk[0], fmaf(g0.y, wk[1], fmaf(g1.x, wk[2], fmaf(g1.y, wk[3], acc[ci]))));
            }
        }
#pragma unroll
        for (int q = 0; q < 4; ++q) {
            f32x4 v = {acc[q * 4], acc[q * 4 + 1], acc[q * 4 + 2], acc[q * 4 + 3]};
            lf_stv(gx + p * 16 + q * 4, v);
        }
    }
}

constexpr int LF_STREAM_BLOCKS = 16384;
inline int grid_for(long units, int cap) {
    long g = (units + 255) / 256;
    if (g > cap) g = cap;
    if (g < 1) g = 1;
    return (int)g;
}
inline bool quad_ok(int C) { return C % 4 == 0 && 256 % (C / 4) == 0; }
inline bool oct_ok(int s16, int C) { return s16 && C % 8 == 0 && 256 % (C / 8) == 0; }
template <typename T> inline const T* as(const float* p) { return reinterpret_cast<const T*>(p); }
template <typename T> inline T* as(float* p) { return reinterpret_cast<T*>(p); }
#define LF_BY_STORAGE(s16, CALL_BF16, CALL_F32) do { if (s16) { CALL_BF16; } else { CALL_F32; } } while (0)
#define LF_BY_STORAGE3(s16, oct, CALL_BF16X8, CALL_BF16, CALL_F32) do { if (oct) { CALL_BF16X8; } else if (s16) { CALL_BF16; } else { CALL_F32; } } while (0)

}

int lf_bn_finalize_fwd(const LfStatPart* parts, int nparts, int C, double count, const float* gamma, const float* beta,
                       float* running_mean, float* running_var, float momentum, float eps, int training, float* scale,
                       float* shift, float* asc, float* ash, hipStream_t st) {
    LF_REQUIRE(nparts >= 0 && nparts <= 2, "bn_finalize: at most 2 partial sources");
    StatParts sp;
    sp.n = nparts;
    for (int i = 0; i < nparts; ++i) sp.p[i] = parts[i];
    for (int i = 0; i < nparts; ++i) LF_REQUIRE(parts[i].C % 4 == 0 && parts[i].ch_off % 4 == 0, "bn_finalize: channel ranges must be multiples of 4");
    for (int i = 0; i < nparts; ++i)
        LF_REQUIRE(parts[i].tile_pix == 0 || (parts[i].seg_rows > 0 && parts[i].seg_pix > 0 && parts[i].nrows % parts[i].seg_rows == 0),
                   "bn_finalize: centred rows need the launch geometry (seg_rows, seg_pix)");
    for (int i = 0; i < nparts; ++i)
        LF_REQUIRE(parts[i].ld >= parts[i].nrows && parts[i].ld % 4 == 0 && ((size_t)parts[i].rows & 15) == 0,
                   "bn_finalize: channel-major rows need a 16-byte aligned base and a leading dimension >= nrows, multiple of 4 (ld=%d nrows=%d)", parts[i].ld, parts[i].nrows);
    hipLaunchKernelGGL(bn_finalize_fwd_kernel, dim3(C), dim3(FIN_THREADS), 0, st, sp, C, count, gamma, beta,
                       running_mean, running_var, momentum, eps, training, scale, shift, asc, ash);
    LF_CHECK_LAUNCH("bn_finalize_fwd");
    return 0;
}

int lf_bn_act(const float* x, const float* sc, const float* sh, const float* dm, const float* res, float* y, long npix,
              int C, long pix_per_image, int s16, hipStream_t st) {
    LF_REQUIRE(C % 4 == 0, "bn_act: C %% 4");
    const bool oct = oct_ok(s16, C);
    const int V = oct ? 8 : 4;
    const long units = npix * (C / V);
    const dim3 grid(grid_for(units, LF_STREAM_BLOCKS));
    LF_BY_STORAGE3(s16, oct,
        hipLaunchKernelGGL((bn_act_kernel<lf_bf16, 2>), grid, dim3(256), 0, st, as<lf_bf16>(x), sc, sh, dm, as<lf_bf16>(res), as<lf_bf16>(y), units, C / V, pix_per_image),
        hipLaunchKernelGGL((bn_act_kernel<lf_bf16, 1>), grid, dim3(256), 0, st, as<lf_bf16>(x), sc, sh, dm, as<lf_bf16>(res), as<lf_bf16>(y), units, C / V, pix_per_image),
        hipLaunchKernelGGL((bn_act_kernel<float, 1>), grid, dim3(256), 0, st, x, sc, sh, dm, res, y, units, C / V, pix_per_image));
    LF_CHECK_LAUNCH("bn_act");
    return 0;
}

int lf_bn_bwd_reduce_rows(long npix) { return grid_for(npix * 4, 1024); }

int lf_bn_bwd_reduce(const float* g, const float* y, const float* t, const float* asc, const float* ash, const float* dm,
                     float* rows, int ld, long npix, int C, long pix_per_image, int s16, hipStream_t st) {
    LF_REQUIRE(quad_ok(C), "bn_bwd_reduce: unsupported channel count %d", C);
    const dim3 grid(lf_bn_bwd_reduce_rows(npix));
    const bool oct = oct_ok(s16, C);
    const int V = oct ? 8 : 4;
    LF_BY_STORAGE3(s16, oct,
        hipLaunchKernelGGL((bn_bwd_reduce_kernel<lf_bf16, 2>), grid, dim3(256), 0, st, as<lf_bf16>(g), as<lf_bf16>(y), as<lf_bf16>(t), asc, ash, dm, rows, ld, npix, C / V, pix_per_image),
        hipLaunchKernelGGL((bn_bwd_reduce_kernel<lf_bf16, 1>), grid, dim3(256), 0, st, as<lf_bf16>(g), as<lf_bf16>(y), as<lf_bf16>(t), asc, ash, dm, rows, ld, npix, C / V, pix_per_image),
        hipLaunchKernelGGL((bn_bwd_reduce_kernel<float, 1>), grid, dim3(256), 0, st, g, y, t, asc, ash, dm, rows, ld, npix, C / V, pix_per_image));
    LF_CHECK_LAUNCH("bn_bwd_reduce");
    return 0;
}

int lf_bn_bwd_finalize(const LfStatPart* parts, int nparts, int C, double count, const float* asc, const float* ash, float* c1,
                       float* c2, float* ggamma, float* gbeta, int training, hipStream_t st) {
    LF_REQUIRE(nparts >= 1 && nparts <= 2, "bn_bwd_finalize: 1..2 partial sources");
    StatParts sp;
    sp.n = nparts;
    for (int i = 0; i < nparts; ++i) sp.p[i] = parts[i];
    for (int i = 0; i < nparts; ++i) LF_REQUIRE(parts[i].C % 4 == 0 && parts[i].ch_off % 4 == 0, "bn_bwd_finalize: channel ranges must be multiples of 4");
    for (int i = 0; i < nparts; ++i)
        LF_REQUIRE(parts[i].ld >= parts[i].nrows && parts[i].ld % 4 == 0 && ((size_t)parts[i].rows & 15) == 0,
                   "bn_bwd_finalize: channel-major rows need a 16-byte aligned base and a leading dimension >= nrows, multiple of 4 (ld=%d nrows=%d)", parts[i].ld, parts[i].nrows);
    hipLaunchKernelGGL(bn_bwd_finalize_kernel, dim3(C), dim3(FIN_THREADS), 0, st, sp, C, training ? 1.0 / count : 0.0, asc, ash,
                       c1, c2, ggamma, gbeta);
    LF_CHECK_LAUNCH("bn_bwd_finalize");
    return 0;
}

int lf_bn_bwd_apply(const float* g, const float* y, const float* t, const float* asc, const float* ash, const float* gamma,
                    const float* c1, const float* c2, const float* dm, float* g_t, float* g_z, long npix, int C,
                    long pix_per_image, int s16, hipStream_t st) {
    LF_REQUIRE(C % 4 == 0, "bn_bwd_apply: C %% 4");
    const bool oct = oct_ok(s16, C);
    const int V = oct ? 8 : 4;
    const long units = npix * (C / V);
    const dim3 grid(grid_for(units, LF_STREAM_BLOCKS));
    LF_BY_STORAGE3(s16, oct,
        hipLaunchKernelGGL((bn_bwd_apply_kernel<lf_bf16, 2>), grid, dim3(256), 0, st, as<lf_bf16>(g), as<lf_bf16>(y), as<lf_bf16>(t), asc, ash, gamma, c1, c2, dm, as<lf_bf16>(g_t), as<lf_bf16>(g_z), units, C / V, pix_per_image),
        hipLaunchKernelGGL((bn_bwd_apply_kernel<lf_bf16, 1>), grid, dim3(256), 0, st, as<lf_bf16>(g), as<lf_bf16>(y), as<lf_bf16>(t), asc, ash, gamma, c1, c2, dm, as<lf_bf16>(g_t), as<lf_bf16>(g_z), units, C / V, pix_per_image),
        hipLaunchKernelGGL((bn_bwd_apply_kernel<float, 1>), grid, dim3(256), 0, st, g, y, t, asc, ash, gamma, c1, c2, dm, g_t, g_z, units, C / V, pix_per_image));
    LF_CHECK_LAUNCH("bn_bwd_apply");
    return 0;
}

int lf_pool_rows(long npix_out) { return grid_for(npix_out * 4, 1024); }

int lf_pool_concat_fwd(const float* x, int N, int H, int W, int Cin, float* cat, int cat_pix, int choff, float* rows, int ld,
                       int s16, hipStream_t st) {
    LF_REQUIRE(quad_ok(Cin) && H % 2 == 0 && W % 2 == 0, "pool_concat: unsupported shape");
    const long npo = (long)N * (H / 2) * (W / 2);
    const dim3 grid(lf_pool_rows(npo));
    const bool oct = oct_ok(s16, Cin) && cat_pix % 8 == 0 && choff % 8 == 0;
    const int V = oct ? 8 : 4;
    LF_BY_STORAGE3(s16, oct,
        hipLaunchKernelGGL((pool_concat_fwd_kernel<lf_bf16, 2>), grid, dim3(256), 0, st, as<lf_bf16>(x), N, H, W, Cin / V, as<lf_bf16>(cat), cat_pix, choff, rows, ld),
        hipLaunchKernelGGL((pool_concat_fwd_kernel<lf_bf16, 1>), grid, dim3(256), 0, st, as<lf_bf16>(x), N, H, W, Cin / V, as<lf_bf16>(cat), cat_pix, choff, rows, ld),
        hipLaunchKernelGGL((pool_concat_fwd_kernel<float, 1>), grid, dim3(256), 0, st, x, N, H, W, Cin / V, cat, cat_pix, choff, rows, ld));
    LF_CHECK_LAUNCH("pool_concat_fwd");
    return 0;
}

int lf_pool_affine_fwd(const float* x, int N, int H, int W, int Cin, float* cat, int cat_pix, int choff, const float* sc,
                       const float* sh, int s16, hipStream_t st) {
    LF_REQUIRE(quad_ok(Cin) && H % 2 == 0 && W % 2 == 0 && sc && sh, "pool_affine: unsupported shape");
    const long npo = (long)N * (H / 2) * (W / 2);
    const bool oct = oct_ok(s16, Cin) && cat_pix % 8 == 0 && choff % 8 == 0;
    const int V = oct ? 8 : 4;
    const long units = npo * (Cin / V);
    const dim3 grid(grid_for(units, LF_STREAM_BLOCKS));
    LF_BY_STORAGE3(s16, oct,
        hipLaunchKernelGGL((pool_affine_fwd_kernel<lf_bf16, 2>), grid, dim3(256), 0, st, as<lf_bf16>(x), N, H, W, Cin / V, as<lf_bf16>(cat), cat_pix, choff, sc, sh, units),
        hipLaunchKernelGGL((pool_affine_fwd_kernel<lf_bf16, 1>), grid, dim3(256), 0, st, as<lf_bf16>(x), N, H, W, Cin / V, as<lf_bf16>(cat), cat_pix, choff, sc, sh, units),
        hipLaunchKernelGGL((pool_affine_fwd_kernel<float, 1>), grid, dim3(256), 0, st, x, N, H, W, Cin / V, cat, cat_pix, choff, sc, sh, units));
    LF_CHECK_LAUNCH("pool_affine_fwd");
    return 0;
}

int lf_pool_bwd(const float* x, const float* gcat, int N, int H, int W, int Cin, int cat_pix, int choff, float* gx,
                int s16, hipStream_t st) {
    const bool oct = oct_ok(s16, Cin) && cat_pix % 8 == 0 && choff % 8 == 0;
    const int V = oct ? 8 : 4;
    const long units = (long)N * (H / 2) * (W / 2) * (Cin / V);
    const dim3 grid(grid_for(units, 4096));
    LF_BY_STORAGE3(s16, oct,
        hipLaunchKernelGGL((pool_bwd_kernel<lf_bf16, 2>), grid, dim3(256), 0, st, as<lf_bf16>(x), as<lf_bf16>(gcat), N, H, W, Cin / V, cat_pix, choff, as<lf_bf16>(gx)),
        hipLaunchKernelGGL((pool_bwd_kernel<lf_bf16, 1>), grid, dim3(256), 0, st, as<lf_bf16>(x), as<lf_bf16>(gcat), N, H, W, Cin / V, cat_pix, choff, as<lf_bf16>(gx)),
        hipLaunchKernelGGL((pool_bwd_kernel<float, 1>), grid, dim3(256), 0, st, x, gcat, N, H, W, Cin / V, cat_pix, choff, gx));
    LF_CHECK_LAUNCH("pool_bwd");
    return 0;
}

int lf_head_fwd(const float* x, const float* w, const float* b, float* out, int N, int h, int w_, int K, int s16,
                hipStream_t st) {
    LF_REQUIRE(K >= 1 && K <= HEAD_MAXK, "head: out_channels %d not in 1..%d", K, HEAD_MAXK);
    const dim3 grid(grid_for((long)N * h * w_, 4096));
    LF_BY_STORAGE(s16,
        hipLaunchKernelGGL(head_fwd_kernel<lf_bf16>, grid, dim3(256), 0, st, as<lf_bf16>(x), w, b, out, N, h, w_, K),
        hipLaunchKernelGGL(head_fwd_kernel<float>, grid, dim3(256), 0, st, x, w, b, out, N, h, w_, K));
    LF_CHECK_LAUNCH("head_fwd");
    return 0;
}

int lf_head_bwd_data(const float* gout, const float* w, float* gx, int N, int h, int w_, int K, int s16, hipStream_t st) {
    LF_REQUIRE(K >= 1 && K <= HEAD_MAXK, "head: out_channels %d not in 1..%d", K, HEAD_MAXK);
    const dim3 grid(grid_for((long)N * h * w_, 4096));
    LF_BY_STORAGE(s16,
        hipLaunchKernelGGL(head_bwd_data_kernel<lf_bf16>, grid, dim3(256), 0, st, gout, w, as<lf_bf16>(gx), N, h, w_, K),
        hipLaunchKernelGGL(head_bwd_data_kernel<float>, grid, dim3(256), 0, st, gout, w, gx, N, h, w_, K));
    LF_CHECK_LAUNCH("head_bwd_data");
    return 0;
}

namespace {
constexpr int PW_MAXK = 8, PW_MAXC = 256;

template <typename T>
__global__ __launch_bounds__(256) void pointwise_fwd_kernel(const T* __restrict__ x, const float* __restrict__ w,
                                                           const float* __restrict__ b, float* __restrict__ y, long npix,
                                                           long pix_per_image, int C, int K) {
    __shared__ float sw[PW_MAXK * PW_MAXC];
    for (int i = threadIdx.x; i < K * C; i += 256) sw[i] = w[i];
    __syncthreads();
    for (long p = (long)blockIdx.x * 256 + threadIdx.x; p < npix; p += (long)gridDim.x * 256) {
        float acc[PW_MAXK];
        for (int k = 0; k < K; ++k) acc[k] = b ? b[k] : 0.f;
        const T* xp = x + p * C;
        for (int c = 0; c < C; c += 4) {
            const lf_f32x4 v = lf_ldv(xp + c);
            for (int k = 0; k < K; ++k) {
                const float* wk = sw + k * C + c;
                acc[k] = fmaf(v.x, wk[0], fmaf(v.y, wk[1], fmaf(v.z, wk[2], fmaf(v.w, wk[3], acc[k]))));
            }
        }
        const long n = p / pix_per_image, q = p - n * pix_per_image;
        for (int k = 0; k < K; ++k) y[(n * K + k) * pix_per_image + q] = acc[k];
    }
}

template <typename T>
__global__ __launch_bounds__(256) void pointwise_bwd_data_kernel(const float* __restrict__ gy, const float* __restrict__ w,
                                                                T* __restrict__ gx, long npix, long pix_per_image, int C,
                                                                int K) {
    __shared__ float sw[PW_MAXK * PW_MAXC];
    for (int i = threadIdx.x; i < K * C; i += 256) sw[i] = w[i];
    __syncthreads();
    for (long p = (long)blockIdx.x * 256 + threadIdx.x; p < npix; p += (long)gridDim.x * 256) {
        const long n = p / pix_per_image, q = p - n * pix_per_image;
        float g[PW_MAXK];
        for (int k = 0; k < K; ++k) g[k] = gy[(n * K + k) * pix_per_image + q];
        T* gp = gx + p * C;
        for (int c = 0; c < C; c += 4) {
            lf_f32x4 v = {0.f, 0.f, 0.f, 0.f};
            for (int k = 0; k < K; ++k) {
                const float* wk = sw + k * C + c;
                v.x = fmaf(g[k], wk[0], v.x); v.y = fmaf(g[k], wk[1], v.y); v.z = fmaf(g[k], wk[2], v.z); v.w = fmaf(g[k], wk[3], v.w);
            }
            lf_stv(gp + c, v);
        }
    }
}

template <typename T>
__global__ __launch_bounds__(256) void pointwise_wgrad_kernel(const T* __restrict__ x, const float* __restrict__ gy,
                                                             float* __restrict__ wrows, float* __restrict__ brows, long npix,
                                                             long pix_per_image, int C, int K, int pix_per_block) {
    const int c = threadIdx.x;
    const long p0 = (long)blockIdx.x * pix_per_block;
    float acc[PW_MAXK], bs[PW_MAXK];
    for (int k = 0; k < K; ++k) { acc[k] = 0.f; bs[k] = 0.f; }
    for (int i = 0; i < pix_per_block; ++i) {
        const long p = p0 + i;
        if (p >= npix) break;
        const long n = p / pix_per_image, q = p - n * pix_per_image;
        const float xv = c < C ? lf_ld1(x + p * C + c) : 0.f;
        for (int k = 0; k < K; ++k) {
            const float g = gy[(n * K + k) * pix_per_image + q];
            acc[k] = fmaf(g, xv, acc[k]);
            bs[k] += g;
        }
    }
    if (c < C)
        for (int k = 0; k < K; ++k) wrows[((long)blockIdx.x * K + k) * C + c] = acc[k];
    if (c == 0)
        for (int k = 0; k < K; ++k) brows[(long)blockIdx.x * K + k] = bs[k];
}
}

extern "C" {
int lf_pointwise_fwd(const float* x, const float* w, const float* b, float* y, int N, int h, int w_, int C, int K, void* stream) {
    LF_REQUIRE(x && w && y && C % 4 == 0 && C <= PW_MAXC && K >= 1 && K <= PW_MAXK, "lf_pointwise_fwd: bad arguments (C=%d K=%d)", C, K);
    const long npix = (long)N * h * w_;
    hipLaunchKernelGGL(pointwise_fwd_kernel<float>, dim3(grid_for(npix, 4096)), dim3(256), 0, (hipStream_t)stream, x, w, b, y, npix,
                       (long)h * w_, C, K);
    LF_CHECK_LAUNCH("pointwise_fwd");
    return 0;
}
long lf_pointwise_scratch_floats(int N, int h, int w_, int C, int K) {
    const long npix = (long)N * h * w_;
    return (long)lf_cdiv(npix, 256) * (K * C + K);
}
int lf_pointwise_bwd(const float* x, const float* gy, const float* w, float* gx, float* gw, float* gb, int N, int h, int w_,
                     int C, int K, float* scratch, void* stream) {
    LF_REQUIRE(x && gy && w && C % 4 == 0 && C <= PW_MAXC && K >= 1 && K <= PW_MAXK, "lf_pointwise_bwd: bad arguments (C=%d K=%d)", C, K);
    hipStream_t st = (hipStream_t)stream;
    const long npix = (long)N * h * w_;
    if (gx) {
        hipLaunchKernelGGL(pointwise_bwd_data_kernel<float>, dim3(grid_for(npix, 4096)), dim3(256), 0, st, gy, w, gx, npix, (long)h * w_, C, K);
        LF_CHECK_LAUNCH("pointwise_bwd_data");
    }
    if (gw || gb) {
        LF_REQUIRE(scratch, "lf_pointwise_bwd: scratch missing");
        const int rows = lf_cdiv(npix, 256);
        float* brows = scratch + (long)rows * K * C;
        hipLaunchKernelGGL(pointwise_wgrad_kernel<float>, dim3(rows), dim3(256), 0, st, x, gy, scratch, brows, npix, (long)h * w_, C, K, 256);
        LF_CHECK_LAUNCH("pointwise_wgrad");
        if (gw) LF_TRY(lf_rows_reduce_launch(scratch, rows, K * C, gw, 0, st));
        if (gb) LF_TRY(lf_rows_reduce_launch(brows, rows, K, gb, 0, st));
    }
    return 0;
}

int lf_pointwise_bf16_fwd(const uint16_t* x, const float* w, const float* b, float* y, int N, int h, int w_, int C, int K, void* stream) {
    LF_REQUIRE(x && w && y && C % 8 == 0 && C <= PW_MAXC && K >= 1 && K <= PW_MAXK, "lf_pointwise_bf16_fwd: bad arguments (C=%d K=%d)", C, K);
    const long npix = (long)N * h * w_;
    hipLaunchKernelGGL(pointwise_fwd_kernel<lf_bf16>, dim3(grid_for(npix, 4096)), dim3(256), 0, (hipStream_t)stream,
                       reinterpret_cast<const lf_bf16*>(x), w, b, y, npix, (long)h * w_, C, K);
    LF_CHECK_LAUNCH("pointwise_bf16_fwd");
    return 0;
}
int lf_pointwise_bf16_bwd(const uint16_t* x, const float* gy, const float* w, uint16_t* gx, float* gw, float* gb, int N, int h, int w_,
                          int C, int K, float* scratch, void* stream) {
    LF_REQUIRE(x && gy && w && C % 8 == 0 && C <= PW_MAXC && K >= 1 && K <= PW_MAXK, "lf_pointwise_bf16_bwd: bad arguments (C=%d K=%d)", C, K);
    hipStream_t st = (hipStream_t)stream;
    const long npix = (long)N * h * w_;
    const lf_bf16* xb = reinterpret_cast<const lf_bf16*>(x);
    if (gx) {
        hipLaunchKernelGGL(pointwise_bwd_data_kernel<lf_bf16>, dim3(grid_for(npix, 4096)), dim3(256), 0, st, gy, w,
                           reinterpret_cast<lf_bf16*>(gx), npix, (long)h * w_, C, K);
        LF_CHECK_LAUNCH("pointwise_bf16_bwd_data");
    }
    if (gw || gb) {
        LF_REQUIRE(scratch, "lf_pointwise_bf16_bwd: scratch missing");
        const int rows = lf_cdiv(npix, 256);
        float* brows = scratch + (long)rows * K * C;
        hipLaunchKernelGGL(pointwise_wgrad_kernel<lf_bf16>, dim3(rows), dim3(256), 0, st, xb, gy, scratch, brows, npix, (long)h * w_, C, K, 256);
        LF_CHECK_LAUNCH("pointwise_bf16_wgrad");
        if (gw) LF_TRY(lf_rows_reduce_launch(scratch, rows, K * C, gw, 0, st));
        if (gb) LF_TRY(lf_rows_reduce_launch(brows, rows, K, gb, 0, st));
    }
    return 0;
}
}
```

### lanedetection_end2end_amd/csrc/lf_erfnet.hip

```cpp
#include <stdlib.h>

#include <vector>

#include "lf_conv.h"
#include "lf_eltwise.h"
#include "lf_plan.h"
#include "lf_types.h"

namespace {

constexpr float BN_EPS = 1e-3f, BN_MOM = 0.1f;
enum { K_DOWN = 0, K_NB = 1, K_UP = 2 };

struct GemmOp {
    LfTapGeom geom;
    int pack;
};
struct BNRef {
    int p_g, p_b, idx, C;
    long sc, sh, asc, ash, c1, c2;
};
struct ConvRef {
    int p_w, p_b;
    GemmOp fwd;
    GemmOp dg[4];
    int ndg;
    GemmOp fph[4];
    int nfph;
};
struct Layer {
    int kind, Cin, Cout, Hin, Win, Hout, Wout, dil, drop_idx;
    long reg_lo;
    long x;
    long b[5];
    ConvRef cv[4];
    BNRef bn[2];
    int fi[4];
    int fv;
};
struct FoldSrc {
    int p_g, p_b, bn;
    int p_bias;
    long out_off;
};

}

struct lf_erfnet_plan {
    int N, H, W, Cin, Cout;
    std::vector<Layer> layers;
    std::vector<LfPackEntry> packs;
    int n_params, n_bn, n_drop;
    int p_head_w[2], p_head_b[2], n_heads;
    long off_entries, off_packed, packed_floats;
    long off_packed16, packed16_elems;
    long off_packed48;
    mutable int precision = 0;
    long off_stat0, off_stat1, stat_floats;
    long off_wpart, wpart_floats, off_bpart, bpart_floats;
    long off_wpart_all, wpart_all_floats[2], bpart_all_floats[2];
    long off_globals;
    long off_gA, off_gB, off_gC, gbuf_floats;
    long total_floats;
    long head_in;
    std::vector<long> drop_off;
    long drop_floats;
    mutable int prof_on = 0;
    struct ProfRec { hipEvent_t a, b; int family; double flops; int layer; int Cs, Cd, ntaps; long npix; int epi; };
    mutable int prof_layer = -1;
    mutable std::vector<ProfRec> prof;
    std::vector<LfFoldEntry> fold;
    std::vector<FoldSrc> fold_src;
    long infer_packed_floats = 0, infer_packed16_elems = 0, infer_vec_floats = 0;
    long infer_enc_floats = 0;
    mutable std::vector<LfFoldEntry> fold_call;
    mutable std::vector<const void*> fold_key;
};

namespace {

int add_pack(lf_erfnet_plan* P, int param, int Kc, int Nc, long sk, long sn, const LfTapGeom& g, const int* tapidx) {
    LfPackEntry e;
    memset(&e, 0, sizeof(e));
    e.param = param; e.Kc = Kc; e.Nc = Nc; e.ntaps = g.ntaps; e.sk = sk; e.sn = sn;
    for (int t = 0; t < g.ntaps; ++t) e.tapidx[t] = tapidx[t];
    e.dst_off = P->packed_floats;
    P->packed_floats += (long)g.ntaps * Kc * Nc;
    e.dst16_off = P->packed16_elems;
    P->packed16_elems += lf_pack_bf16_elems(Kc, Nc, g.ntaps);
    P->packs.push_back(e);
    return (int)P->packs.size() - 1;
}

void build_conv1d(lf_erfnet_plan* P, ConvRef& c, int N, int H, int W, int C, int axis, int d) {
    LfTapGeom g = lf_base_geom(N, H, W, H, W, C, H, W, C, C, C);
    g.ntaps = 3;
    int idx_f[3], idx_d[3];
    for (int t = 0; t < 3; ++t) {
        g.tdh[t] = axis == 0 ? (t - 1) * d : 0;
        g.tdw[t] = axis == 1 ? (t - 1) * d : 0;
        idx_f[t] = t;
        idx_d[t] = 2 - t;
    }
    c.fwd.geom = g;
    c.fwd.pack = add_pack(P, c.p_w, C, C,  3,  (long)C * 3, g, idx_f);
    c.nfph = 0;
    c.ndg = 1;
    c.dg[0].geom = g;
    c.dg[0].pack = add_pack(P, c.p_w, C, C,  (long)C * 3,  3, g, idx_d);
}

int add_pack(lf_erfnet_plan* P, int param, const LfStride2Op& op) {
    return add_pack(P, param, op.Kc, op.Nc, op.sk, op.sn, op.geom, op.tapidx);
}

void build_down_conv(lf_erfnet_plan* P, ConvRef& c, int N, int H, int W, int Cin, int Cc, int Ccat) {
    LfStride2Op fwd, dg[4];
    lf_down_conv_ops(N, H, W, Cin, Cc, Ccat, fwd, dg);
    c.fwd.geom = fwd.geom;
    c.fwd.pack = add_pack(P, c.p_w, fwd);
    c.nfph = 0;
    c.ndg = 4;
    for (int i = 0; i < 4; ++i) {
        c.dg[i].geom = dg[i].geom;
        c.dg[i].pack = add_pack(P, c.p_w, dg[i]);
    }
}

void build_up_conv(lf_erfnet_plan* P, ConvRef& c, int N, int Hi, int Wi, int Cin, int Co) {
    LfStride2Op fph[4], dg;
    lf_up_conv_ops(N, Hi, Wi, Cin, Co, fph, dg);
    c.nfph = 4;
    for (int i = 0; i < 4; ++i) {
        c.fph[i].geom = fph[i].geom;
        c.fph[i].pack = add_pack(P, c.p_w, fph[i]);
    }
    c.ndg = 1;
    c.dg[0].geom = dg.geom;
    c.dg[0].pack = add_pack(P, c.p_w, dg);
    c.fwd = c.fph[0];
}

void bn_alloc(LfBump& ws, BNRef& b) {
    b.sc = ws.take(b.C); b.sh = ws.take(b.C); b.asc = ws.take(b.C); b.ash = ws.take(b.C);
    b.c1 = ws.take(b.C); b.c2 = ws.take(b.C);
}

void account_fwd_stats(lf_erfnet_plan* P, const LfTapGeom& g) {
    P->stat_floats = lf_maxl(P->stat_floats, (long)lf_tapgemm_stat_rows(g) * 2 * g.Cd);
}
long wneed_of(const LfTapGeom& g, int s16) { return lf_wgrad_wneed(g, s16); }
long bneed_of(const LfTapGeom& g, int s16) { return lf_wgrad_bneed(g, s16); }
void account_wgrad(lf_erfnet_plan* P, const LfTapGeom& g) {
    for (int s16 = 0; s16 < 2; ++s16) {
// ... 103 lines not shown
        P->layers.push_back(L);
        cur = L.b[1]; h /= 2; w /= 2;
    };
    auto add_nb = [&](int c, float pdrop, int d) {
        Layer L;
        memset(&L, 0, sizeof(L));
        L.kind = K_NB; L.Cin = c; L.Cout = c; L.Hin = L.Hout = h; L.Win = L.Wout = w; L.dil = d;
        L.drop_idx = pdrop > 0.f ? drop++ : -1;
        L.x = cur; L.reg_lo = ws.cur;
        const long sz = (long)N * h * w * c;
        for (int i = 0; i < 5; ++i) L.b[i] = ws.take(sz);
        const int axis[4] = {0, 1, 0, 1}, dil[4] = {1, 1, d, d};
        for (int i = 0; i < 4; ++i) {
            if (i == 2) { L.bn[0].p_g = param++; L.bn[0].p_b = param++; L.bn[0].idx = bn++; L.bn[0].C = c; }
            L.cv[i].p_w = param++; L.cv[i].p_b = param++;
            build_conv1d(P, L.cv[i], N, h, w, c, axis[i], dil[i]);
        }
        L.bn[1].p_g = param++; L.bn[1].p_b = param++; L.bn[1].idx = bn++; L.bn[1].C = c;
        bn_alloc(ws, L.bn[0]); bn_alloc(ws, L.bn[1]);
        account_fwd_stats(P, L.cv[0].fwd.geom);
        for (int i = 0; i < 4; ++i) account_wgrad(P, L.cv[i].fwd.geom);
        if (L.drop_idx >= 0) { P->drop_off.push_back(P->drop_floats); P->drop_floats += (long)N * c; }
        P->layers.push_back(L);
        cur = L.b[4];
    };
    auto add_up = [&](int cin, int cout) {
        Layer L;
        memset(&L, 0, sizeof(L));
        L.kind = K_UP; L.Cin = cin; L.Cout = cout; L.Hin = h; L.Win = w; L.Hout = 2 * h; L.Wout = 2 * w; L.drop_idx = -1;
        L.x = cur; L.reg_lo = ws.cur;
        L.cv[0].p_w = param++; L.cv[0].p_b = param++;
        L.bn[0].p_g = param++; L.bn[0].p_b = param++; L.bn[0].idx = bn++; L.bn[0].C = cout;
        const long sz = (long)N * 2 * h * 2 * w * cout;
        L.b[0] = ws.take(sz); L.b[1] = ws.take(sz);
        bn_alloc(ws, L.bn[0]);
        build_up_conv(P, L.cv[0], N, h, w, cin, cout);
        long rows4 = 0;
        for (int ph = 0; ph < 4; ++ph) { rows4 += lf_tapgemm_stat_rows(L.cv[0].fph[ph].geom); account_wgrad(P, L.cv[0].fph[ph].geom); }
        P->stat_floats = lf_maxl(P->stat_floats, rows4 * 2 * cout);
        P->layers.push_back(L);
        cur = L.b[1]; h *= 2; w *= 2;
    };
    add_down(in_channels, 16);
    add_down(16, 64);
    for (int i = 0; i < 5; ++i) add_nb(64, 0.03f, 1);
    add_down(64, 128);
    const int dils[8] = {2, 4, 8, 16, 2, 4, 8, 16};
    for (int i = 0; i < 8; ++i) add_nb(128, 0.3f, dils[i]);
    param += 2;
    add_up(128, 64);
    add_nb(64, 0.f, 1); add_nb(64, 0.f, 1);
    add_up(64, 16);
    add_nb(16, 0.f, 1); add_nb(16, 0.f, 1);
    for (int i = 0; i < n_heads; ++i) { P->p_head_w[i] = param++; P->p_head_b[i] = param++; }
    P->head_in = cur;
    P->n_params = param; P->n_bn = bn; P->n_drop = drop;

    const long npix1 = (long)N * (H / 2) * (W / 2);
    P->stat_floats = lf_maxl(P->stat_floats, (long)lf_stem_rows(N, H, W) * 2 * 16);
    P->stat_floats = lf_maxl(P->stat_floats, (long)lf_pool_rows(npix1) * 2 * 128);
    P->stat_floats = lf_maxl(P->stat_floats, (long)lf_bn_bwd_reduce_rows(npix1) * 2 * 128);
    P->wpart_floats = lf_maxl(P->wpart_floats, (long)lf_stem_wgrad_rows(N, H, W) * 16 * 36);
    P->wpart_floats = lf_maxl(P->wpart_floats, (long)lf_head_wgrad_rows(N, H / 2, W / 2) * 16 * 5 * 4);
    P->bpart_floats = lf_maxl(P->bpart_floats, (long)lf_stem_wgrad_rows(N, H, W) * 16);
    P->bpart_floats = lf_maxl(P->bpart_floats, (long)lf_head_wgrad_rows(N, H / 2, W / 2) * 8);
    for (int s16 = 0; s16 < 2; ++s16) {
        P->wpart_all_floats[s16] += ((long)lf_stem_wgrad_rows(N, H, W) * 16 * 36 + 63) / 64 * 64 + ((long)lf_head_wgrad_rows(N, H / 2, W / 2) * 16 * 5 * 4 + 63) / 64 * 64;
        P->bpart_all_floats[s16] += ((long)lf_stem_wgrad_rows(N, H, W) * 16 + 63) / 64 * 64 + ((long)lf_head_wgrad_rows(N, H / 2, W / 2) * 8 + 63) / 64 * 64;
    }

    P->off_globals = ws.cur;
    P->off_entries = ws.take((long)(P->packs.size() * sizeof(LfPackEntry) + 3) / 4);
    P->off_packed = ws.take(P->packed_floats);
    P->off_packed16 = ws.take((P->packed16_elems + 1) / 2);
    P->off_packed48 = ws.take((3 * P->packed16_elems + 1) / 2);
    P->stat_floats += 2 * 128 * 4;
    P->off_stat0 = ws.take((P->stat_floats + 3) / 4 * 4);
    P->off_stat1 = ws.take((P->stat_floats + 3) / 4 * 4);
    P->off_wpart = ws.take(P->wpart_floats);
    P->off_bpart = ws.take(P->bpart_floats);
    P->gbuf_floats = (long)N * (H / 2) * (W / 2) * 16;
    P->off_gA = ws.take(P->gbuf_floats);
    P->off_gB = ws.take(P->gbuf_floats);
    P->off_gC = ws.take(P->gbuf_floats);
    P->off_wpart_all = ws.cur;
    P->total_floats = wpart_all_end(P, 1);
    build_infer(P);
    return P;
}

void lf_erfnet_plan_destroy(lf_erfnet_plan* P) {
    if (!P) return;
    delete P;
}
size_t lf_erfnet_workspace_bytes(const lf_erfnet_plan* P) { return (size_t)wpart_all_end(P, P->precision == 2) * sizeof(float); }
size_t lf_erfnet_workspace_bytes_for(const lf_erfnet_plan* P, int mode) {
    if (!P || !(mode == 0 || mode == 2 || mode == 3)) return 0;
    return (size_t)wpart_all_end(P, mode == 2) * sizeof(float);
}
int lf_erfnet_set_precision(const lf_erfnet_plan* P, int mode) {
    LF_REQUIRE(P && (mode == 0 || mode == 2 || mode == 3), "lf_erfnet_set_precision: mode must be 0 (fp32 cores), 2 (bf16 tensors) or "
               "3 (fp32 from 9-term split operands on the bf16 cores); modes 1 and 4 were removed in round 6");
    P->precision = mode;
    return 0;
}
long lf_erfnet_activation_floats(const lf_erfnet_plan* P) { return P->off_globals; }
int lf_erfnet_num_params(const lf_erfnet_plan* P) { return P->n_params; }
int lf_erfnet_num_bn(const lf_erfnet_plan* P) { return P->n_bn; }
long lf_erfnet_dropmask_floats(const lf_erfnet_plan* P) { return P->drop_floats; }
int lf_erfnet_num_dropout(const lf_erfnet_plan* P) { return P->n_drop; }
long lf_erfnet_dropmask_offset(const lf_erfnet_plan* P, int i) { return P->drop_off[i]; }
int lf_erfnet_dropmask_channels(const lf_erfnet_plan* P, int i) {
    int k = 0;
    for (const Layer& L : P->layers)
        if (L.drop_idx >= 0 && k++ == i) return L.Cout;
    return -1;
}
long lf_erfnet_encoder_offset(const lf_erfnet_plan* P) {
    for (const Layer& L : P->layers)
        if (L.kind == K_UP) return L.x;
    return -1;
}
long lf_erfnet_activation_offset(const lf_erfnet_plan* P, int layer, int slot) {
    if (layer < 0 || layer >= (int)P->layers.size() || slot < 0 || slot > 4) return -1;
    return P->layers[layer].b[slot];
}
long lf_erfnet_bn_vector_offset(const lf_erfnet_plan* P, int layer, int bn, int which) {
    if (layer < 0 || layer >= (int)P->layers.size() || bn < 0 || bn > 1 || which < 0 || which > 3) return -1;
    const Layer& L = P->layers[layer];
    if (bn == 1 && L.kind != K_NB) return -1;
    const BNRef& b = L.bn[bn];
    return which == 0 ? b.sc : which == 1 ? b.sh : which == 2 ? b.asc : b.ash;
}

}

namespace {

struct Ctx {
    const lf_erfnet_plan* P;
    float* ws;
    const float* const* params;
    float* const* grads;
    float* const* running;
    const float* dropmask;
    int training;
    hipStream_t st;
    const float* g_enc = nullptr;
    int s16 = 0;
    mutable std::vector<LfReduceJob> reduce_jobs;
    mutable long wpart_used = 0, bpart_used = 0;
    mutable int last_rows = 0;
    mutable bool wgrad_launched = false;
    long lo = 0, hi = 0, cut = 0;
    bool no_batch = false;
    float* at(long off) const { return off < cut ? ws + (off - lo) : ws + (hi - lo) + (off - cut); }
    const float* packed(int pack) const { return at(P->off_packed + P->packs[pack].dst_off); }
};

double gemm_flops(const LfTapGeom& g) { return 2.0 * (double)g.N * g.Hl * g.Wl * g.Cs * g.Cd * g.ntaps; }

struct ProfScope {
    const Ctx& c; int idx = -1;
    hipStream_t pst;
    ProfScope(const Ctx& ctx, int family, const LfTapGeom& g, int epi, hipStream_t stream) : c(ctx), pst(stream) {
        if (!c.P->prof_on) return;
        lf_erfnet_plan::ProfRec r;
        r.family = family; r.flops = gemm_flops(g);
        r.layer = c.P->prof_layer; r.Cs = g.Cs; r.Cd = g.Cd; r.ntaps = g.ntaps; r.npix = (long)g.N * g.Hl * g.Wl; r.epi = epi;
        if (hipEventCreate(&r.a) != hipSuccess || hipEventCreate(&r.b) != hipSuccess) return;
        (void)hipEventRecord(r.a, pst);
        c.P->prof.push_back(r);
        idx = (int)c.P->prof.size() - 1;
    }
    ~ProfScope() { if (idx >= 0) (void)hipEventRecord(c.P->prof[idx].b, pst); }
};

int run_gemm(const Ctx& c, const GemmOp& op, const float* src, float* dst, const float* bias, int pro, int epi,
             LfTapArgs extra, bool beside_wgrad = false) {
    extra.src = src; extra.dst = dst; extra.bias = bias; extra.wp = c.packed(op.pack);
    extra.s16 = c.s16;
    if (c.P->precision == 2)
        extra.wp16 = reinterpret_cast<const unsigned short*>(c.at(c.P->off_packed16)) + c.P->packs[op.pack].dst16_off;
    if (c.P->precision == 3) {
        extra.split = 9;
        extra.wp48 = reinterpret_cast<const unsigned short*>(c.at(c.P->off_packed48)) + 3 * c.P->packs[op.pack].dst16_off;
    }
    c.last_rows = lf_tapgemm_stat_rows_for(op.geom, extra);
    ProfScope ps(c, 0, op.geom, epi | (pro << 8), c.st);
    if (beside_wgrad && c.wgrad_launched && !c.P->prof_on) return lf_tapgemm_launch_unordered(op.geom, extra, pro, epi, c.st);
    return lf_tapgemm_launch(op.geom, extra, pro, epi, c.st);
}

int bn_finalize(const Ctx& c, const BNRef& b, const LfStatPart* parts, int nparts, double count) {
    return lf_bn_finalize_fwd(parts, nparts, b.C, count, c.params[b.p_g], c.params[b.p_b], c.running[2 * b.idx],
                              c.running[2 * b.idx + 1], BN_MOM, BN_EPS, c.training, c.at(b.sc), c.at(b.sh), c.at(b.asc),
                              c.at(b.ash), c.st);
}

int encoder_layers(const lf_erfnet_plan* P) {
    int n = 0;
    for (const Layer& L : P->layers) { if (L.kind == K_UP) break; ++n; }
    return n;
}

int forward_layers(const Ctx& c, const float* img, int nlayers, int first = 0) {
    const lf_erfnet_plan* P = c.P;
    const int N = P->N;
    float* stat0 = c.at(P->off_stat0);
    float* stat1 = c.at(P->off_stat1);
    int layer_idx = 0;
    for (const Layer& L : P->layers) {
        if (layer_idx >= nlayers) break;
        if (layer_idx < first) { ++layer_idx; continue; }
        P->prof_layer = layer_idx++;
        const long npo = (long)N * L.Hout * L.Wout;
        if (L.kind == K_DOWN) {
            LfStatPart parts[2];
            int np = 0;
            if (L.x < 0) {
                const int srows = lf_stem_rows(N, L.Hin, L.Win);
                LF_TRY(lf_stem_fwd(img, N, L.Cin, L.Hin, L.Win, c.params[L.cv[0].p_w], c.params[L.cv[0].p_b], c.at(L.b[0]),
                                   c.training ? stat0 : nullptr, lf_stat_ld(srows), c.s16, c.st));
                parts[np++] = {stat0, srows, 16, 0, lf_stat_ld(srows)};
            } else {
                LfTapArgs a = lf_no_args();
                a.stats = stat0; a.stats_ld = lf_stat_ld(lf_tapgemm_stat_rows(L.cv[0].fwd.geom));
                LF_TRY(run_gemm(c, L.cv[0].fwd, c.at(L.x), c.at(L.b[0]), c.params[L.cv[0].p_b], LF_PRO_NONE,
                                c.training ? LF_EPI_STATS_SQ : 0, a));
                parts[np++] = lf_stat_part_tiles(stat0, c.last_rows, a.stats_ld, L.Cout - L.Cin, 0, c.last_rows, npo);
                const int prows = lf_pool_rows(npo);
                LF_TRY(lf_pool_concat_fwd(c.at(L.x), N, L.Hin, L.Win, L.Cin, c.at(L.b[0]), L.Cout, L.Cout - L.Cin,
                                          c.training ? stat1 : nullptr, lf_stat_ld(prows), c.s16, c.st));
                parts[np++] = {stat1, prows, L.Cin, L.Cout - L.Cin, lf_stat_ld(prows)};
            }
            LF_TRY(bn_finalize(c, L.bn[0], parts, np, (double)npo));
            LF_TRY(lf_bn_act(c.at(L.b[0]), c.at(L.bn[0].sc), c.at(L.bn[0].sh), nullptr, nullptr, c.at(L.b[1]), npo, L.Cout,
                             (long)L.Hout * L.Wout, c.s16, c.st));
        } else if (L.kind == K_NB) {
            LfTapArgs a = lf_no_args();
            LF_TRY(run_gemm(c, L.cv[0].fwd, c.at(L.x), c.at(L.b[0]), c.params[L.cv[0].p_b], LF_PRO_NONE, LF_EPI_RELU, a));
            a.stats = stat0; a.stats_ld = lf_stat_ld(lf_tapgemm_stat_rows(L.cv[1].fwd.geom));
            LF_TRY(run_gemm(c, L.cv[1].fwd, c.at(L.b[0]), c.at(L.b[1]), c.params[L.cv[1].p_b], LF_PRO_NONE,
                            c.training ? LF_EPI_STATS_SQ : 0, a));
            LfStatPart p0 = lf_stat_part_tiles(stat0, c.last_rows, a.stats_ld, L.Cout, 0, c.last_rows, npo);
            LF_TRY(bn_finalize(c, L.bn[0], &p0, 1, (double)npo));
            a = lf_no_args();
            a.pro_sc = c.at(L.bn[0].sc); a.pro_sh = c.at(L.bn[0].sh);
            LF_TRY(run_gemm(c, L.cv[2].fwd, c.at(L.b[1]), c.at(L.b[2]), c.params[L.cv[2].p_b], LF_PRO_BNRELU, LF_EPI_RELU, a));
            a = lf_no_args();
            a.stats = stat0; a.stats_ld = lf_stat_ld(lf_tapgemm_stat_rows(L.cv[3].fwd.geom));
            LF_TRY(run_gemm(c, L.cv[3].fwd, c.at(L.b[2]), c.at(L.b[3]), c.params[L.cv[3].p_b], LF_PRO_NONE,
                            c.training ? LF_EPI_STATS_SQ : 0, a));
            p0.nrows = p0.seg_rows = c.last_rows; p0.ld = a.stats_ld;
            LF_TRY(bn_finalize(c, L.bn[1], &p0, 1, (double)npo));
            const float* dm = (c.training && L.drop_idx >= 0 && c.dropmask) ? c.dropmask + P->drop_off[L.drop_idx] : nullptr;
            LF_TRY(lf_bn_act(c.at(L.b[3]), c.at(L.bn[1].sc), c.at(L.bn[1].sh), dm, c.at(L.x), c.at(L.b[4]), npo, L.Cout,
                             (long)L.Hout * L.Wout, c.s16, c.st));
        } else {
            LfStatPart parts[1];
            int rows = 0, rows4 = 0;
            for (int ph = 0; ph < 4; ++ph) rows4 += lf_tapgemm_stat_rows(L.cv[0].fph[ph].geom);
            for (int ph = 0; ph < 4; ++ph) {
                LfTapArgs a = lf_no_args();
                a.stats = stat0 + rows; a.stats_ld = lf_stat_ld(rows4);
                LF_TRY(run_gemm(c, L.cv[0].fph[ph], c.at(L.x), c.at(L.b[0]), c.params[L.cv[0].p_b], LF_PRO_NONE,
                                c.training ? LF_EPI_STATS_SQ : 0, a));
                rows += c.last_rows;
            }
            parts[0] = lf_stat_part_tiles(stat0, rows, lf_stat_ld(rows4), L.Cout, 0, rows / 4, npo / 4);
            LF_TRY(bn_finalize(c, L.bn[0], parts, 1, (double)npo));
            LF_TRY(lf_bn_act(c.at(L.b[0]), c.at(L.bn[0].sc), c.at(L.bn[0].sh), nullptr, nullptr, c.at(L.b[1]), npo, L.Cout,
                             (long)L.Hout * L.Wout, c.s16, c.st));
        }
    }
    return 0;
}

typedef LfBiasChain BiasChain;

int run_wgrad(const Ctx& c, const GemmOp& op, const ConvRef& cv, const float* x, const float* g, const float* pro_sc,
              const float* pro_sh, int bias_accumulate, bool batch_off = false, BiasChain* chain = nullptr) {
    const lf_erfnet_plan* P = c.P;
    c.wgrad_launched = false;
    if (!c.grads[cv.p_w]) return 0;
    hipStream_t ws = c.st;
    LfWgradArgs a;
    a.x = x; a.g = g; a.pro_sc = pro_sc; a.pro_sh = pro_sh; a.s16 = c.s16;
    a.split = 0;
    const long wneed = (wneed_of(op.geom, c.s16) + 63) / 64 * 64, bneed = (bneed_of(op.geom, c.s16) + 63) / 64 * 64;
    const bool batched = !bias_accumulate && !batch_off && !c.no_batch &&
                         c.wpart_used + wneed <= P->wpart_all_floats[c.s16] && c.bpart_used + bneed <= P->bpart_all_floats[c.s16];
    const long off_bpart_all = P->off_wpart_all + P->wpart_all_floats[c.s16];
    a.partial = batched ? c.at(P->off_wpart_all + c.wpart_used) : c.at(P->off_wpart);
    a.bias_partial = c.grads[cv.p_b] ? (batched ? c.at(off_bpart_all + c.bpart_used) : c.at(P->off_bpart)) : nullptr;
    if (chain) {
        if (!batched) return lf_fail("erfnet backward: a chained weight gradient does not fit its partial-row regions");
        float* rows = lf_bias_chain_rows(*chain, c.at(off_bpart_all + c.bpart_used), op.geom.Cd);
        if (a.bias_partial) a.bias_partial = rows;
    }
    {
        ProfScope ps(c, 1, op.geom, 0, ws);
        LF_TRY(lf_tapwgrad_launch(op.geom, a, pro_sc ? LF_PRO_BNRELU : LF_PRO_NONE, ws));
    }
    c.wgrad_launched = true;
    const LfPackEntry& e = P->packs[op.pack];
    const int nsplit = lf_tapwgrad_splits_for(op.geom, a, pro_sc ? LF_PRO_BNRELU : LF_PRO_NONE);
    if (batched) {
        c.wpart_used += wneed; c.bpart_used += bneed;
        LfReduceJob j = lf_wgrad_reduce_job(op.geom, a.partial, nsplit, c.grads[cv.p_w], e.sk, e.sn, e.tapidx, a.bias_partial, c.grads[cv.p_b]);
        if (chain) lf_bias_chain_job(*chain, j, nsplit, a.bias_partial != nullptr);
        c.reduce_jobs.push_back(j);
        return 0;
    }
    LF_TRY(lf_wgrad_reduce_launch(a.partial, nsplit, op.geom.ntaps, op.geom.Cs, op.geom.Cd,
                                  c.grads[cv.p_w], e.sk, e.sn, e.tapidx, a.bias_partial, nsplit,
                                  c.grads[cv.p_b], bias_accumulate, ws));
    return 0;
}

struct RowSums { float* wrows; float* brows; bool batched; };
RowSums row_sum_regions(const Ctx& c, long wneed, long bneed) {
    const lf_erfnet_plan* P = c.P;
    wneed = (wneed + 63) / 64 * 64; bneed = (bneed + 63) / 64 * 64;
    const bool batched = !c.no_batch && c.wpart_used + wneed <= P->wpart_all_floats[c.s16] && c.bpart_used + bneed <= P->bpart_all_floats[c.s16];
    RowSums r;
    r.batched = batched;
    r.wrows = batched ? c.at(P->off_wpart_all + c.wpart_used) : c.at(P->off_wpart);
    r.brows = batched ? c.at(P->off_wpart_all + P->wpart_all_floats[c.s16] + c.bpart_used) : c.at(P->off_bpart);
    if (batched) { c.wpart_used += wneed; c.bpart_used += bneed; }
    return r;
}
int row_sums_finish(const Ctx& c, const RowSums& r, int rows, int nw, float* gw, int nb, float* gb) {
    if (!r.batched) {
        LF_TRY(lf_rows_reduce_launch(r.wrows, rows, nw, gw, 0, c.st));
        if (gb) LF_TRY(lf_rows_reduce_launch(r.brows, rows, nb, gb, 0, c.st));
        return 0;
    }
    c.reduce_jobs.push_back(lf_row_sum_job(r.wrows, rows, nw, gw));
    if (gb) c.reduce_jobs.push_back(lf_row_sum_job(r.brows, rows, nb, gb));
    return 0;
}

int bn_bwd_finalize(const Ctx& c, const BNRef& b, const LfStatPart* parts, int nparts, double count) {
    if (!c.grads[b.p_g] || !c.grads[b.p_b]) return lf_fail("erfnet backward: BatchNorm weight/bias must both require grad");
    return lf_bn_bwd_finalize(parts, nparts, b.C, count, c.at(b.asc), c.at(b.ash), c.at(b.c1), c.at(b.c2), c.grads[b.p_g],
                              c.grads[b.p_b], c.training, c.st);
}

struct Prep {
    const float* y = nullptr;
    const float* pre = nullptr;
    const BNRef* bn = nullptr;
    const float* dm = nullptr;
};

Prep prep_for(const Ctx& c, const Layer& Lp) {
    Prep p;
    if (Lp.kind == K_NB) {
        p.y = c.at(Lp.b[4]); p.pre = c.at(Lp.b[3]); p.bn = &Lp.bn[1];
        p.dm = (Lp.drop_idx >= 0 && c.dropmask) ? c.dropmask + c.P->drop_off[Lp.drop_idx] : nullptr;
    } else {
        p.y = c.at(Lp.b[1]); p.pre = c.at(Lp.b[0]); p.bn = &Lp.bn[0];
    }
    return p;
}

int backward_layers(const Ctx& c, const float* img, float* g0, float* g1, float* g2, int nlayers, int first = 0,
                    float** gin = nullptr) {
    const lf_erfnet_plan* P = c.P;
    const int N = P->N;
    float* stat0 = c.at(P->off_stat0);
    float* bufs[3] = {g0, g1, g2};
    float* in = g0;
    bool prepped = false;
    int prep_rows = 0, prep_ld = 0;
    for (int li = nlayers - 1; li >= first; --li) {
        const Layer& L = P->layers[li];
        P->prof_layer = 100 + li;
        const long npo = (long)N * L.Hout * L.Wout;
        const long ppi = (long)L.Hout * L.Wout;
        const int iin = in == bufs[0] ? 0 : (in == bufs[1] ? 1 : 2);
        float* X = bufs[(iin + 1) % 3];
        float* Y = bufs[(iin + 2) % 3];
        Prep nx;
        const bool can_prep = li > first && (L.kind == K_NB || L.kind == K_UP);
        if (can_prep) nx = prep_for(c, P->layers[li - 1]);
        auto add_prep = [&](LfTapArgs& a, int& epi, const LfTapGeom& dg) {
            if (!can_prep) return;
            a.mask_src = nx.y; a.aux = nx.pre; a.asc = c.at(nx.bn->asc); a.ash = c.at(nx.bn->ash); a.dm = nx.dm;
            a.stats = stat0; a.stats_ld = lf_stat_ld(lf_tapgemm_stat_rows(dg));
            epi |= LF_EPI_MASK | LF_EPI_STATS_XHAT;
        };
        const BNRef& blast = L.kind == K_NB ? L.bn[1] : L.bn[0];
        const float* ylast = c.at(L.kind == K_NB ? L.b[4] : L.b[1]);
        const float* prelast = c.at(L.kind == K_NB ? L.b[3] : L.b[0]);
        const float* dm = (L.kind == K_NB && L.drop_idx >= 0 && c.dropmask) ? c.dropmask + P->drop_off[L.drop_idx] : nullptr;
        const float* gz;
        if (!prepped) {
            const int rrows = lf_bn_bwd_reduce_rows(npo);
            LF_TRY(lf_bn_bwd_reduce(in, ylast, prelast, c.at(blast.asc), c.at(blast.ash), dm, stat0, lf_stat_ld(rrows), npo, L.Cout, ppi, c.s16, c.st));
            LfStatPart rp = {stat0, rrows, L.Cout, 0, lf_stat_ld(rrows)};
            LF_TRY(bn_bwd_finalize(c, blast, &rp, 1, (double)npo));
            LF_TRY(lf_bn_bwd_apply(in, ylast, prelast, c.at(blast.asc), c.at(blast.ash), c.params[blast.p_g], c.at(blast.c1),
                                   c.at(blast.c2), dm, X, L.kind == K_NB ? Y : nullptr, npo, L.Cout, ppi, c.s16, c.st));
            gz = Y;
        } else {
            LfStatPart rp = {stat0, prep_rows, L.Cout, 0, prep_ld};
            LF_TRY(bn_bwd_finalize(c, blast, &rp, 1, (double)npo));
            LF_TRY(lf_bn_bwd_apply(in, nullptr, prelast, c.at(blast.asc), c.at(blast.ash), c.params[blast.p_g], c.at(blast.c1),
                                   c.at(blast.c2), dm, X, nullptr, npo, L.Cout, ppi, c.s16, c.st));
            gz = in;
        }
        float* F = prepped ? Y : in;
        float* out = nullptr;
        prepped = false;
        if (L.kind == K_NB) {
            const float* x = c.at(L.x);
            const float *t1 = c.at(L.b[0]), *t2 = c.at(L.b[1]), *t3 = c.at(L.b[2]);
            const BNRef& b1 = L.bn[0];
            LF_TRY(run_wgrad(c, L.cv[3].fwd, L.cv[3], t3, X, nullptr, nullptr, 0));
            LfTapArgs a = lf_no_args();
            a.mask_src = t3;
            LF_TRY(run_gemm(c, L.cv[3].dg[0], X, F, nullptr, LF_PRO_NONE, LF_EPI_MASK, a, true));
            LF_TRY(run_wgrad(c, L.cv[2].fwd, L.cv[2], t2, F, c.at(b1.sc), c.at(b1.sh), 0));
            a = lf_no_args();
            a.aux = t2; a.msc = c.at(b1.sc); a.msh = c.at(b1.sh); a.asc = c.at(b1.asc); a.ash = c.at(b1.ash);
            a.stats = stat0; a.stats_ld = lf_stat_ld(lf_tapgemm_stat_rows(L.cv[2].dg[0].geom));
            LF_TRY(run_gemm(c, L.cv[2].dg[0], F, X, nullptr, LF_PRO_NONE, LF_EPI_MASKBN | LF_EPI_STATS_XHAT, a, true));
            LfStatPart sp = {stat0, c.last_rows, L.Cout, 0, a.stats_ld};
            LF_TRY(bn_bwd_finalize(c, b1, &sp, 1, (double)npo));
            LF_TRY(lf_bn_bwd_apply(X, nullptr, t2, c.at(b1.asc), c.at(b1.ash), c.params[b1.p_g], c.at(b1.c1), c.at(b1.c2),
                                   nullptr, F , nullptr, npo, L.Cout, ppi, c.s16, c.st));
            LF_TRY(run_wgrad(c, L.cv[1].fwd, L.cv[1], t1, F, nullptr, nullptr, 0));
            a = lf_no_args();
            a.mask_src = t1;
            LF_TRY(run_gemm(c, L.cv[1].dg[0], F, X, nullptr, LF_PRO_NONE, LF_EPI_MASK, a, true));
            LF_TRY(run_wgrad(c, L.cv[0].fwd, L.cv[0], x, X, nullptr, nullptr, 0));
            a = lf_no_args();
            a.add_src = gz;
            int epi = LF_EPI_ADD;
            add_prep(a, epi, L.cv[0].dg[0].geom);
            LF_TRY(run_gemm(c, L.cv[0].dg[0], X, F, nullptr, LF_PRO_NONE, epi, a, true));
            out = F;
            if (can_prep) { prepped = true; prep_rows = c.last_rows; prep_ld = a.stats_ld; }
        } else if (L.kind == K_UP) {
            long wsum = 0, bsum = 0;
            for (int ph = 0; ph < 4; ++ph) {
                wsum += (wneed_of(L.cv[0].fph[ph].geom, c.s16) + 63) / 64 * 64;
                bsum += (bneed_of(L.cv[0].fph[ph].geom, c.s16) + 63) / 64 * 64;
            }
            const bool chained = !c.no_batch && c.wpart_used + wsum <= P->wpart_all_floats[c.s16] && c.bpart_used + bsum <= P->bpart_all_floats[c.s16];
            BiasChain bc;
            for (int ph = 0; ph < 4; ++ph) {
                if (chained) LF_TRY(run_wgrad(c, L.cv[0].fph[ph], L.cv[0], c.at(L.x), X, nullptr, nullptr, 0, false, &bc));
                else LF_TRY(run_wgrad(c, L.cv[0].fph[ph], L.cv[0], c.at(L.x), X, nullptr, nullptr, ph > 0, true));
            }
            LfTapArgs a = lf_no_args();
            int epi = 0;
            if (c.g_enc && L.x == lf_erfnet_encoder_offset(P)) {
                a.add_src = c.g_enc;
                epi |= LF_EPI_ADD;
            }
            add_prep(a, epi, L.cv[0].dg[0].geom);
            LF_TRY(run_gemm(c, L.cv[0].dg[0], X, F, nullptr, LF_PRO_NONE, epi, a));
            out = F;
            if (can_prep) { prepped = true; prep_rows = c.last_rows; prep_ld = a.stats_ld; }
        } else if (L.x < 0) {
            const int Cc = 16 - L.Cin, rows = lf_stem_wgrad_rows(N, L.Hin, L.Win);
            if (c.grads[L.cv[0].p_w]) {
                const RowSums rs = row_sum_regions(c, (long)rows * Cc * L.Cin * 9, (long)rows * Cc);
                LF_TRY(lf_stem_wgrad(img, X, N, L.Cin, L.Hin, L.Win, rs.wrows, rs.brows, c.s16, c.st));
                LF_TRY(row_sums_finish(c, rs, rows, Cc * L.Cin * 9, c.grads[L.cv[0].p_w], Cc, c.grads[L.cv[0].p_b]));
            }
            out = F;
        } else {
            LF_TRY(run_wgrad(c, L.cv[0].fwd, L.cv[0], c.at(L.x), X, nullptr, nullptr, 0));
            LF_TRY(lf_pool_bwd(c.at(L.x), X, N, L.Hin, L.Win, L.Cin, L.Cout, L.Cout - L.Cin, F, c.s16, c.st));
            for (int ph = 0; ph < 4; ++ph) {
                LfTapArgs a = lf_no_args();
                a.add_src = F;
                LF_TRY(run_gemm(c, L.cv[0].dg[ph], X, F, nullptr, LF_PRO_NONE, LF_EPI_ADD, a));
            }
            out = F;
        }
        in = out;
    }
    if (gin) *gin = in;
    return 0;
}

int upload_and_pack(const Ctx& c, const float* const* params_dev) {
    const lf_erfnet_plan* P = c.P;
    LfPackEntry* ent = reinterpret_cast<LfPackEntry*>(c.at(P->off_entries));
    if (hipMemcpyAsync(ent, P->packs.data(), P->packs.size() * sizeof(LfPackEntry), hipMemcpyHostToDevice, c.st) != hipSuccess)
        return lf_fail("erfnet: upload of the pack table failed");
    LF_TRY(lf_pack_weights_launch(ent, (int)P->packs.size(), params_dev, c.at(P->off_packed), c.st));
    if (P->precision == 2)
        LF_TRY(lf_pack_weights_bf16_launch(ent, (int)P->packs.size(), params_dev, c.at(P->off_packed16), c.st));
    if (P->precision == 3)
        LF_TRY(lf_pack_weights_split_launch(ent, (int)P->packs.size(), params_dev, c.at(P->off_packed48), c.st));
    return 0;
}

}

extern "C" {


int lf_erfnet_forward(const lf_erfnet_plan* P, const float* img, const float* const* params_host,
                      const float* const* params_dev, float* const* running_host, const float* dropmask, int training,
                      int head, float* logits, void* workspace, size_t workspace_bytes, void* stream) {
    LF_REQUIRE(P && img && params_host && params_dev && running_host && (logits || head < 0) && workspace, "lf_erfnet_forward: null pointer");
    LF_REQUIRE(workspace_bytes >= lf_erfnet_workspace_bytes(P), "lf_erfnet_forward: workspace too small");
    LF_REQUIRE(head >= -1 && head < P->n_heads, "lf_erfnet_forward: head %d out of range", head);
    Ctx c{P, (float*)workspace, params_host, nullptr, running_host, dropmask, training, (hipStream_t)stream};
    c.s16 = P->precision == 2;
    LF_TRY(upload_and_pack(c, params_dev));
    if (head < 0) return forward_layers(c, img, encoder_layers(P));
    LF_TRY(forward_layers(c, img, (int)P->layers.size()));
    return lf_head_fwd(c.at(P->head_in), params_host[P->p_head_w[head]], params_host[P->p_head_b[head]], logits, P->N, P->H / 2,
                       P->W / 2, P->Cout + head, c.s16, c.st);
}

int lf_erfnet_backward(const lf_erfnet_plan* P, const float* img, const float* grad_logits,
                       const float* grad_encoder, const float* const* params_host, float* const* grads_host,
                       const float* dropmask, int training, int head, void* workspace, size_t workspace_bytes, void* stream) {
    LF_REQUIRE(P && img && (grad_logits || head < 0) && params_host && grads_host && workspace, "lf_erfnet_backward: null pointer");
    LF_REQUIRE(workspace_bytes >= lf_erfnet_workspace_bytes(P), "lf_erfnet_backward: workspace too small");
    LF_REQUIRE(head >= -1 && head < P->n_heads, "lf_erfnet_backward: head %d out of range", head);
    Ctx c{P, (float*)workspace, params_host, grads_host, nullptr, dropmask, training, (hipStream_t)stream};
    c.g_enc = grad_encoder;
    c.s16 = P->precision == 2;
    float *gA = c.at(P->off_gA), *gB = c.at(P->off_gB), *gC = c.at(P->off_gC);
    if (head < 0) {
        LF_REQUIRE(grad_encoder, "lf_erfnet_backward: the encoder-only backward needs grad_encoder");
        const int ne = encoder_layers(P);
        const Layer& Le = P->layers[ne - 1];
        const size_t bytes = (size_t)P->N * Le.Hout * Le.Wout * Le.Cout * (c.s16 ? 2 : sizeof(float));
        if (hipMemcpyAsync(gA, grad_encoder, bytes, hipMemcpyDeviceToDevice, c.st) != hipSuccess)
            return lf_fail("lf_erfnet_backward: copy of grad_encoder failed");
        c.g_enc = nullptr;
        LF_TRY(backward_layers(c, img, gA, gB, gC, ne));
        if (!c.reduce_jobs.empty()) LF_TRY(lf_wgrad_reduce_batch_launch(c.reduce_jobs.data(), (int)c.reduce_jobs.size(), c.st));
        return 0;
    }
    const int h = P->H / 2, w = P->W / 2, K = P->Cout + head;
    const int pw = P->p_head_w[head], pb = P->p_head_b[head];
    if (grads_host[pw]) {
        const int rows = lf_head_wgrad_rows(P->N, h, w);
        const RowSums rs = row_sum_regions(c, (long)rows * 16 * K * 4, (long)rows * K);
        LF_TRY(lf_head_wgrad(c.at(P->head_in), grad_logits, rs.wrows, rs.brows, P->N, h, w, K, c.s16, c.st));
        LF_TRY(row_sums_finish(c, rs, rows, 16 * K * 4, grads_host[pw], K, grads_host[pb]));
    }
    LF_TRY(lf_head_bwd_data(grad_logits, params_host[pw], gA, P->N, h, w, K, c.s16, c.st));
    LF_TRY(backward_layers(c, img, gA, gB, gC, (int)P->layers.size()));
    if (!c.reduce_jobs.empty()) LF_TRY(lf_wgrad_reduce_batch_launch(c.reduce_jobs.data(), (int)c.reduce_jobs.size(), c.st));
    return 0;
}

int lf_erfnet_profile(const lf_erfnet_plan* P, int enable) { P->prof_on = enable; return 0; }
int lf_erfnet_profile_read(const lf_erfnet_plan* P, double* out6, const char* csv_path) {
    for (int i = 0; i < 6; ++i) out6[i] = 0.0;
    FILE* f = nullptr;
    if (csv_path) {
        f = fopen(csv_path, "w");
        if (f) fprintf(f, "family,layer,Cs,Cd,ntaps,npix,epi,us,tflops\n");
    }
    for (auto& r : P->prof) {
        float ms = 0.f;
        if (hipEventSynchronize(r.b) == hipSuccess && hipEventElapsedTime(&ms, r.a, r.b) == hipSuccess) {
            out6[r.family * 3 + 0] += ms; out6[r.family * 3 + 1] += r.flops; out6[r.family * 3 + 2] += 1.0;
            if (f) fprintf(f, "%d,%d,%d,%d,%d,%ld,%d,%.2f,%.2f\n", r.family, r.layer, r.Cs, r.Cd, r.ntaps, r.npix, r.epi,
                           ms * 1e3, r.flops / (ms * 1e-3) / 1e12);
        }
        (void)hipEventDestroy(r.a); (void)hipEventDestroy(r.b);
    }
    if (f) fclose(f);
    P->prof.clear();
    return 0;
}

int lf_nhwc_to_nchw(const float* src, float* dst, int N, int H, int W, int C, void* stream);

}

namespace {
template <typename T>
__global__ __launch_bounds__(256) void nhwc_to_nchw_kernel(const T* __restrict__ s, float* __restrict__ d, int H, int W,
                                                          int C, long total) {
    for (long i = (long)blockIdx.x * 256 + threadIdx.x; i < total; i += (long)gridDim.x * 256) {
        const int w = (int)(i % W);
        long r = i / W;
        const int h = (int)(r % H);
        r /= H;
        const int ch = (int)(r % C);
        const long n = r / C;
        d[i] = lf_ld1(s + ((n * H + h) * W + w) * C + ch);
    }
}
int nhwc_to_nchw(const float* src, float* dst, int N, int H, int W, int C, int s16, hipStream_t st) {
    const long total = (long)N * H * W * C;
    int grid = lf_cdiv(total, 256);
    if (grid > 4096) grid = 4096;
    if (s16) hipLaunchKernelGGL(nhwc_to_nchw_kernel<lf_bf16>, dim3(grid), dim3(256), 0, st, reinterpret_cast<const lf_bf16*>(src), dst, H, W, C, total);
    else hipLaunchKernelGGL(nhwc_to_nchw_kernel<float>, dim3(grid), dim3(256), 0, st, src, dst, H, W, C, total);
    LF_CHECK_LAUNCH("nhwc_to_nchw");
    return 0;
}
}

extern "C" int lf_nhwc_to_nchw(const float* src, float* dst, int N, int H, int W, int C, void* stream) {
    return nhwc_to_nchw(src, dst, N, H, W, C, 0, (hipStream_t)stream);
}

namespace {
template <typename T>
__global__ __launch_bounds__(256) void nchw_to_nhwc_kernel(const float* __restrict__ s, T* __restrict__ d, int H, int W, int C,
                                                          long total) {
    for (long i = (long)blockIdx.x * 256 + threadIdx.x; i < total; i += (long)gridDim.x * 256) {
        const int ch = (int)(i % C);
        long r = i / C;
        const int w = (int)(r % W);
        r /= W;
        const int h = (int)(r % H);
        const long n = r / H;
        lf_st1(d + i, s[((n * C + ch) * H + h) * W + w]);
    }
}
int nchw_to_nhwc(const float* src, float* dst, int N, int H, int W, int C, int s16, hipStream_t st) {
    const long total = (long)N * H * W * C;
    int grid = lf_cdiv(total, 256);
    if (grid > 8192) grid = 8192;
    if (s16) hipLaunchKernelGGL(nchw_to_nhwc_kernel<lf_bf16>, dim3(grid), dim3(256), 0, st, src, reinterpret_cast<lf_bf16*>(dst), H, W, C, total);
    else hipLaunchKernelGGL(nchw_to_nhwc_kernel<float>, dim3(grid), dim3(256), 0, st, src, dst, H, W, C, total);
    LF_CHECK_LAUNCH("nchw_to_nhwc");
    return 0;
}
long layer_out_offset(const Layer& L) { return L.kind == K_NB ? L.b[4] : L.b[1]; }
void range_span(const lf_erfnet_plan* P, int first, int last, long* lo, long* hi) {
    const Layer& Lf = P->layers[first];
    *lo = first > 0 ? (Lf.x < Lf.reg_lo ? Lf.x : Lf.reg_lo) : Lf.reg_lo;
    *hi = last < (int)P->layers.size() ? P->layers[last].reg_lo : P->off_globals;
}
void compact(Ctx& c, int first, int last) {
    range_span(c.P, first, last, &c.lo, &c.hi);
    c.cut = c.P->off_globals;
    c.no_batch = true;
}
int check_range(const lf_erfnet_plan* P, int first, int last, int head, const char* who) {
    LF_REQUIRE(P && first >= 0 && last > first && last <= (int)P->layers.size(), "%s: bad layer range [%d, %d)", who, first, last);
    LF_REQUIRE(head < 0 || (last == (int)P->layers.size() && head < P->n_heads), "%s: the head follows the last layer only", who);
    return 0;
}
}

extern "C" {

int lf_erfnet_num_layers(const lf_erfnet_plan* P) { return (int)P->layers.size(); }
size_t lf_erfnet_range_workspace_bytes(const lf_erfnet_plan* P, int first, int last) {
    if (!P || first < 0 || last <= first || last > (int)P->layers.size()) return 0;
    long lo, hi;
    range_span(P, first, last, &lo, &hi);
    return (size_t)((hi - lo) + (P->off_wpart_all - P->off_globals)) * sizeof(float);
}
int lf_erfnet_layer_io(const lf_erfnet_plan* P, int layer, int* out6) {
    LF_REQUIRE(P && out6 && layer >= 0 && layer < (int)P->layers.size(), "lf_erfnet_layer_io: layer %d out of range", layer);
    const Layer& L = P->layers[layer];
    out6[0] = L.Cin; out6[1] = L.Hin; out6[2] = L.Win; out6[3] = L.Cout; out6[4] = L.Hout; out6[5] = L.Wout;
    return 0;
}

int lf_erfnet_forward_range(const lf_erfnet_plan* P, int first, int last, int head, const float* x,
                            const float* const* params_host, const float* const* params_dev, float* const* running_host,
                            const float* dropmask, int training, float* y, void* workspace, size_t workspace_bytes, void* stream) {
    LF_TRY(check_range(P, first, last, head, "lf_erfnet_forward_range"));
    LF_REQUIRE(x && y && params_host && params_dev && running_host && workspace, "lf_erfnet_forward_range: null pointer");
    LF_REQUIRE(workspace_bytes >= lf_erfnet_range_workspace_bytes(P, first, last), "lf_erfnet_forward_range: workspace too small");
    Ctx c{P, (float*)workspace, params_host, nullptr, running_host, dropmask, training, (hipStream_t)stream};
    compact(c, first, last);
    c.s16 = P->precision == 2;
    LF_TRY(upload_and_pack(c, params_dev));
    const Layer& Lf = P->layers[first];
    if (first > 0) LF_TRY(nchw_to_nhwc(x, c.at(Lf.x), P->N, Lf.Hin, Lf.Win, Lf.Cin, c.s16, c.st));
    LF_TRY(forward_layers(c, x, last, first));
    const Layer& Ll = P->layers[last - 1];
    if (head >= 0)
        return lf_head_fwd(c.at(P->head_in), params_host[P->p_head_w[head]], params_host[P->p_head_b[head]], y, P->N, P->H / 2,
                           P->W / 2, P->Cout + head, c.s16, c.st);
    return nhwc_to_nchw(c.at(layer_out_offset(Ll)), y, P->N, Ll.Hout, Ll.Wout, Ll.Cout, c.s16, c.st);
}

int lf_erfnet_backward_range(const lf_erfnet_plan* P, int first, int last, int head, const float* x, const float* gy,
                             const float* const* params_host, float* const* grads_host, const float* dropmask, int training,
                             float* gx, void* workspace, size_t workspace_bytes, void* stream) {
    LF_TRY(check_range(P, first, last, head, "lf_erfnet_backward_range"));
    LF_REQUIRE(x && gy && params_host && grads_host && workspace, "lf_erfnet_backward_range: null pointer");
    LF_REQUIRE(workspace_bytes >= lf_erfnet_range_workspace_bytes(P, first, last), "lf_erfnet_backward_range: workspace too small");
    Ctx c{P, (float*)workspace, params_host, grads_host, nullptr, dropmask, training, (hipStream_t)stream};
    compact(c, first, last);
    c.s16 = P->precision == 2;
    float *gA = c.at(P->off_gA), *gB = c.at(P->off_gB), *gC = c.at(P->off_gC);
    const Layer& Ll = P->layers[last - 1];
    if (head >= 0) {
        const int h = P->H / 2, w = P->W / 2, K = P->Cout + head;
        const int pw = P->p_head_w[head], pb = P->p_head_b[head];
        if (grads_host[pw]) {
            const int rows = lf_head_wgrad_rows(P->N, h, w);
            const RowSums rs = row_sum_regions(c, (long)rows * 16 * K * 4, (long)rows * K);
            LF_TRY(lf_head_wgrad(c.at(P->head_in), gy, rs.wrows, rs.brows, P->N, h, w, K, c.s16, c.st));
            LF_TRY(row_sums_finish(c, rs, rows, 16 * K * 4, grads_host[pw], K, grads_host[pb]));
        }
        LF_TRY(lf_head_bwd_data(gy, params_host[pw], gA, P->N, h, w, K, c.s16, c.st));
    } else {
        LF_TRY(nchw_to_nhwc(gy, gA, P->N, Ll.Hout, Ll.Wout, Ll.Cout, c.s16, c.st));
    }
    float* gin = nullptr;
    LF_TRY(backward_layers(c, x, gA, gB, gC, last, first, &gin));
    if (!c.reduce_jobs.empty()) LF_TRY(lf_wgrad_reduce_batch_launch(c.reduce_jobs.data(), (int)c.reduce_jobs.size(), c.st));
    const Layer& Lf = P->layers[first];
    if (gx && first > 0) LF_TRY(nhwc_to_nchw(gin, gx, P->N, Lf.Hin, Lf.Win, Lf.Cin, c.s16, c.st));
    return 0;
}

}

namespace {

int infer_fold_table(const lf_erfnet_plan* P, char* ws, const InferLayout& L, const float* const* params_host,
                     float* const* running_host, hipStream_t st) {
    std::vector<const void*> key;
    key.reserve(P->n_params + 2 * P->n_bn);
    for (int i = 0; i < P->n_params; ++i) key.push_back(params_host[i]);
    for (int i = 0; i < 2 * P->n_bn; ++i) key.push_back(running_host[i]);
    if (key != P->fold_key) {
        if (!P->fold_key.empty() && hipStreamSynchronize(st) != hipSuccess) return lf_fail("lf_erfnet_infer: stream synchronisation failed");
        P->fold_call = P->fold;
        for (size_t i = 0; i < P->fold.size(); ++i) {
            LfFoldEntry& f = P->fold_call[i];
            const FoldSrc& s = P->fold_src[i];
            if (s.bn >= 0) {
                f.gamma = params_host[s.p_g]; f.beta = params_host[s.p_b];
                f.mean = running_host[2 * s.bn]; f.var = running_host[2 * s.bn + 1];
            }
            if (s.p_bias >= 0) f.bias = params_host[s.p_bias];
        }
        P->fold_key = key;
    }
    if (hipMemcpyAsync(ws + L.table, P->fold_call.data(), P->fold_call.size() * sizeof(LfFoldEntry), hipMemcpyHostToDevice, st) != hipSuccess)
        return lf_fail("lf_erfnet_infer: upload of the fold table failed");
    return 0;
}

struct InferCtx {
    const lf_erfnet_plan* P;
    char* ws;
    InferLayout L;
    int mode, s16;
    hipStream_t st;
    float* vec(int fi, int which = 0) const {
        return reinterpret_cast<float*>(ws + L.vec) + P->fold_src[fi].out_off + (which ? P->fold[fi].C : 0);
    }
};

int infer_gemm(const InferCtx& c, const GemmOp& op, int fi, const float* src, float* dst, int epi, const float* add) {
    const LfPackEntry& e = c.P->fold[fi].pk;
    LfTapArgs a = lf_no_args();
    a.src = src; a.dst = dst; a.bias = c.vec(fi); a.add_src = add; a.s16 = c.s16;
    if (c.L.a32 >= 0) a.wp = reinterpret_cast<const float*>(c.ws + c.L.a32) + e.dst_off;
    if (c.L.a16 >= 0) a.wp16 = reinterpret_cast<const unsigned short*>(c.ws + c.L.a16) + e.dst16_off;
    if (c.L.a48 >= 0) {
        a.split = 9;
        a.wp48 = reinterpret_cast<const unsigned short*>(c.ws + c.L.a48) + 3 * e.dst16_off;
    }
    return lf_tapgemm_launch(op.geom, a, LF_PRO_NONE, epi, c.st);
}

int forward_infer(const InferCtx& c, const float* img, const float* const* params_host, int nlayers, float** out, int first = 0,
                  float* xin = nullptr) {
    const lf_erfnet_plan* P = c.P;
    const int N = P->N, ne = encoder_layers(P);
    float* bufs[3];
    for (int i = 0; i < 3; ++i) bufs[i] = reinterpret_cast<float*>(c.ws + c.L.buf[i]);
    float* enc = reinterpret_cast<float*>(c.ws + c.L.enc);
    auto other = [&](const float* u, const float* v) {
        for (float* b : bufs) if (b != u && b != v) return b;
        return bufs[0];
    };
    float* x = xin;
    for (int li = first; li < nlayers; ++li) {
        const Layer& L = P->layers[li];
        if (L.kind == K_DOWN && L.x < 0) {
            float* y = bufs[0];
            LF_TRY(lf_stem_fwd_infer(img, N, L.Cin, L.Hin, L.Win, params_host[L.cv[0].p_w], params_host[L.cv[0].p_b], c.vec(L.fv, 0),
                                     c.vec(L.fv, 1), y, c.s16, c.st));
            x = y;
        } else if (L.kind == K_DOWN) {
            float* y = li == ne - 1 ? enc : other(x, nullptr);
            LF_TRY(infer_gemm(c, L.cv[0].fwd, L.fi[0], x, y, LF_EPI_RELU, nullptr));
            LF_TRY(lf_pool_affine_fwd(x, N, L.Hin, L.Win, L.Cin, y, L.Cout, L.Cout - L.Cin, c.vec(L.fv, 0), c.vec(L.fv, 1), c.s16, c.st));
            x = y;
        } else if (L.kind == K_NB) {
            float* t1 = other(x, nullptr);
            float* t2 = other(x, t1);
            float* y = li == ne - 1 ? enc : t2;
            LF_TRY(infer_gemm(c, L.cv[0].fwd, L.fi[0], x, t1, LF_EPI_RELU, nullptr));
            LF_TRY(infer_gemm(c, L.cv[1].fwd, L.fi[1], t1, t2, LF_EPI_RELU, nullptr));
            LF_TRY(infer_gemm(c, L.cv[2].fwd, L.fi[2], t2, t1, LF_EPI_RELU, nullptr));
            LF_TRY(infer_gemm(c, L.cv[3].fwd, L.fi[3], t1, y, LF_EPI_ADD | LF_EPI_RELU, x));
            x = y;
        } else {
            float* y = other(x, nullptr);
            for (int ph = 0; ph < 4; ++ph) LF_TRY(infer_gemm(c, L.cv[0].fph[ph], L.fi[ph], x, y, LF_EPI_RELU, nullptr));
            x = y;
        }
    }
    *out = x;
    return 0;
}

}

extern "C" {

size_t lf_erfnet_infer_workspace_bytes(const lf_erfnet_plan* P, int mode) {
    if (!P || !(mode == 0 || mode == 2 || mode == 3)) return 0;
    return (size_t)infer_layout(P, mode).total;
}
long lf_erfnet_infer_encoder_offset(const lf_erfnet_plan* P) { return P ? infer_layout(P, 0).enc / 4 : -1; }

int lf_erfnet_infer(const lf_erfnet_plan* P, const float* img, const float* const* params_host, const float* const* params_dev,
                    float* const* running_host, int head, float* logits, void* workspace, size_t workspace_bytes, void* stream) {
    LF_REQUIRE(P && img && params_host && params_dev && running_host && (logits || head < 0) && workspace, "lf_erfnet_infer: null pointer");
    LF_REQUIRE(head >= -1 && head < P->n_heads, "lf_erfnet_infer: head %d out of range", head);
    InferCtx c;
    c.P = P; c.ws = (char*)workspace; c.mode = P->precision; c.s16 = P->precision == 2; c.st = (hipStream_t)stream;
    c.L = infer_layout(P, c.mode);
    LF_REQUIRE(workspace_bytes >= (size_t)c.L.total, "lf_erfnet_infer: workspace too small (%zu < %ld)", workspace_bytes, c.L.total);
    LF_TRY(infer_fold_table(P, c.ws, c.L, (const float* const*)params_host, running_host, c.st));
    LF_TRY(lf_fold_pack_launch(reinterpret_cast<const LfFoldEntry*>(c.ws + c.L.table), (int)P->fold.size(), params_dev, BN_EPS,
                               reinterpret_cast<float*>(c.ws + c.L.vec), c.L.a32 >= 0 ? reinterpret_cast<float*>(c.ws + c.L.a32) : nullptr,
                               c.L.a16 >= 0 ? c.ws + c.L.a16 : nullptr, c.L.a48 >= 0 ? c.ws + c.L.a48 : nullptr, c.st));
    float* last = nullptr;
    if (head < 0) return forward_infer(c, img, params_host, encoder_layers(P), &last);
    LF_TRY(forward_infer(c, img, params_host, (int)P->layers.size(), &last));
    return lf_head_fwd(last, params_host[P->p_head_w[head]], params_host[P->p_head_b[head]], logits, P->N, P->H / 2, P->W / 2,
                       P->Cout + head, c.s16, c.st);
}

}

namespace {

int infer_begin(InferCtx& c, const lf_erfnet_plan* P, void* workspace, const float* const* params_host, const float* const* params_dev,
                float* const* running_host, void* stream) {
    c.P = P; c.ws = (char*)workspace; c.mode = P->precision; c.s16 = P->precision == 2; c.st = (hipStream_t)stream;
    c.L = infer_layout(P, c.mode);
    LF_TRY(infer_fold_table(P, c.ws, c.L, params_host, running_host, c.st));
    return lf_fold_pack_launch(reinterpret_cast<const LfFoldEntry*>(c.ws + c.L.table), (int)P->fold.size(), params_dev, BN_EPS,
                               reinterpret_cast<float*>(c.ws + c.L.vec), c.L.a32 >= 0 ? reinterpret_cast<float*>(c.ws + c.L.a32) : nullptr,
                               c.L.a16 >= 0 ? c.ws + c.L.a16 : nullptr, c.L.a48 >= 0 ? c.ws + c.L.a48 : nullptr, c.st);
}

struct LaneLayout { long partials, zinv, total; };
LaneLayout lane_layout(const lf_erfnet_plan* P, int mode, int K, int order) {
    auto al = [](long b) { return (b + 255) / 256 * 256; };
    LaneLayout L;
    long cur = infer_layout(P, mode).total;
    L.partials = cur; cur += al((long)lf_wls_workspace_bytes(P->N, K, order));
    L.zinv = cur; cur += al((long)P->N * K * (order + 1) * (order + 1) * (long)sizeof(double));
    L.total = cur;
    return L;
// ... 62 lines not shown
```

Before: 2019 images/sec.

## Extend any-order kernel launches to independent groups across forward and backward

Adds a generic lf_launch wrapper that issues kernels with hipExtAnyOrderLaunch when a thread-local flag is set. It groups independent launches (up-sampling phase GEMMs, down-block conv plus pool, wgrad beside dgrad, batched reductions, head wgrad plus dgrad) so every launch after the first in a group can run concurrently with its neighbours. The intent is to cut serialisation and idle tail time between small kernels on the same stream. It relies on those kernels truly being independent; any missed dependency would give a race. The path is limited to fp32 precision with profiling off.

```diff
diff --git a/lanedetection_end2end_amd/_lib.py b/lanedetection_end2end_amd/_lib.py
--- a/lanedetection_end2end_amd/_lib.py
+++ b/lanedetection_end2end_amd/_lib.py
@@ -144,6 +144,9 @@
         "lf_debug_conv1d_wgrad_pro": (I, [P, P, P, P, P, P, I, I, I, I, I, I, P, P]),
         "lf_debug_bias_residual_launches": (L, []),
         "lf_debug_partial_fast_launches": (L, []),
+        "lf_debug_set_unordered": (None, [ctypes.c_uint]),
+        "lf_debug_unordered_default": (ctypes.c_uint, []),
+        "lf_debug_unordered_count": (L, [I]),
     }
     for table in (sig, dbg):
         for name, (res, args) in table.items():
diff --git a/lanedetection_end2end_amd/csrc/lf_conv.h b/lanedetection_end2end_amd/csrc/lf_conv.h
--- a/lanedetection_end2end_amd/csrc/lf_conv.h
+++ b/lanedetection_end2end_amd/csrc/lf_conv.h
@@ -1,4 +1,6 @@
 #pragma once
+#include <hip/hip_ext.h>
+
 #include "lf_common.h"
 
 #define LF_MAX_TAPS 9
@@ -58,7 +60,20 @@
 int lf_tapgemm_stat_rows(const LfTapGeom& g);
 int lf_tapgemm_stat_rows_for(const LfTapGeom& g, const LfTapArgs& a);
 int lf_tapgemm_launch(const LfTapGeom& g, const LfTapArgs& a, int pro, int epi, hipStream_t st);
-int lf_tapgemm_launch_unordered(const LfTapGeom& g, const LfTapArgs& a, int pro, int epi, hipStream_t st);
+
+void lf_launch_set_unordered(bool on);
+unsigned lf_launch_flags();
+void lf_launch_count_unordered();
+long lf_launch_unordered_count(int reset);
+template <typename K, typename... Args>
+void lf_launch(K kernel, dim3 grid, dim3 block, size_t lds, hipStream_t st, const Args&... args) {
+    if (const unsigned flags = lf_launch_flags()) {
+        hipExtLaunchKernelGGL(kernel, grid, block, (unsigned)lds, st, nullptr, nullptr, flags, args...);
+        lf_launch_count_unordered();
+    } else {
+        hipLaunchKernelGGL(kernel, grid, block, lds, st, args...);
+    }
+}
 
 struct LfWgradArgs {
     const float* x;
diff --git a/lanedetection_end2end_amd/csrc/lf_conv.hip b/lanedetection_end2end_amd/csrc/lf_conv.hip
--- a/lanedetection_end2end_amd/csrc/lf_conv.hip
+++ b/lanedetection_end2end_amd/csrc/lf_conv.hip
@@ -2010,14 +2010,19 @@
     return done[key] = hipFuncSetAttribute(kernel, hipFuncAttributeMaxDynamicSharedMemorySize, bytes) == hipSuccess;
 }
 thread_local unsigned g_launch_flags = 0;
+std::atomic<long> g_unordered_packets{0};
 template <typename K, typename... Args>
 bool launch_resident(K kernel, dim3 grid, unsigned block, size_t lds, int lds_attr, unsigned max_wgs, unsigned flags, hipStream_t st, const Args&... args) {
     if (lds_attr > 0 && !allow_big_lds(reinterpret_cast<const void*>(kernel), lds_attr)) return false;
     const unsigned res = (unsigned)resident_workgroups(kernel, lds, (int)block) / grid.y;
     if (grid.x > res && res >= 8) grid.x = res & ~7u;
     if (max_wgs > 0 && grid.x > max_wgs) grid.x = max_wgs;
-    if (flags) hipExtLaunchKernelGGL(kernel, grid, dim3(block), (unsigned)lds, st, nullptr, nullptr, flags, args...);
-    else hipLaunchKernelGGL(kernel, grid, dim3(block), lds, st, args...);
+    if (flags) {
+        hipExtLaunchKernelGGL(kernel, grid, dim3(block), (unsigned)lds, st, nullptr, nullptr, flags, args...);
+        ++g_unordered_packets;
+    } else {
+        hipLaunchKernelGGL(kernel, grid, dim3(block), lds, st, args...);
+    }
     return true;
 }
 constexpr int BIG_LDS = 160 * 1024 - 4096;
@@ -2244,7 +2249,7 @@
         default:
             with_pro_epi<true>(pro, epi, epis, [&](auto p, auto e) {
                 constexpr int P = decltype(p)::value, E = decltype(e)::value;
-                hipLaunchKernelGGL((tapgemm_lean_kernel<1, P, E>), grid, dim3(256), 0, st, g, a, pro, epi);
+                lf_launch(tapgemm_lean_kernel<1, P, E>, grid, dim3(256), 0, st, g, a, pro, epi);
                 if constexpr (E == BRES) ++g_bres_launches;
             });
             break;
@@ -2256,12 +2261,10 @@
 
 void lf_tapgemm_set_fp32_stream(int mode, int max_workgroups) { g_stream_mode = mode; g_stream_cap = max_workgroups > 0 ? max_workgroups : 0; }
 
-int lf_tapgemm_launch_unordered(const LfTapGeom& g, const LfTapArgs& a, int pro, int epi, hipStream_t st) {
-    g_launch_flags = hipExtAnyOrderLaunch;
-    const int rc = lf_tapgemm_launch(g, a, pro, epi, st);
-    g_launch_flags = 0;
-    return rc;
-}
+void lf_launch_set_unordered(bool on) { g_launch_flags = on ? hipExtAnyOrderLaunch : 0; }
+unsigned lf_launch_flags() { return g_launch_flags; }
+void lf_launch_count_unordered() { ++g_unordered_packets; }
+long lf_launch_unordered_count(int reset) { return reset ? g_unordered_packets.exchange(0) : g_unordered_packets.load(); }
 
 int lf_tapgemm_launch(const LfTapGeom& g, const LfTapArgs& a, int pro, int epi, hipStream_t st) {
     LF_REQUIRE(g.Cs % 16 == 0 && g.Cd % 16 == 0, "tapgemm: channels must be multiples of 16 (Cs=%d Cd=%d)", g.Cs, g.Cd);
@@ -3015,10 +3018,11 @@
 template <bool XV, bool GV, int XT, int GT>
 void launch_wgrad(const LfTapGeom& g, const LfWgradArgs& a, int pro, const WgradCfg& c, dim3 grid, int wb, hipStream_t st) {
     constexpr bool VV = XV && GV;
-    auto go = [&](auto kern) { hipLaunchKernelGGL(kern, grid, dim3(256), 0, st, g, a, pro, c.pps, wb, c.gx); };
-    if (a.s16 && c.u == 4 && VV) go(tapwgrad_kernel<XV, GV, XT, GT, 4, true, VV>);
-    else if (a.s16 && c.u == 4) go(tapwgrad_kernel<XV, GV, XT, GT, 4, true>);
-    else if (a.s16) go(tapwgrad_kernel<XV, GV, XT, GT, 1, true>);
+    auto go16 = [&](auto kern) { hipLaunchKernelGGL(kern, grid, dim3(256), 0, st, g, a, pro, c.pps, wb, c.gx); };
+    auto go = [&](auto kern) { lf_launch(kern, grid, dim3(256), 0, st, g, a, pro, c.pps, wb, c.gx); };
+    if (a.s16 && c.u == 4 && VV) go16(tapwgrad_kernel<XV, GV, XT, GT, 4, true, VV>);
+    else if (a.s16 && c.u == 4) go16(tapwgrad_kernel<XV, GV, XT, GT, 4, true>);
+    else if (a.s16) go16(tapwgrad_kernel<XV, GV, XT, GT, 1, true>);
     else if (c.u == 4 && VV) {
         if constexpr (VV) {
             if (pro == LF_PRO_BNRELU) go(tapwgrad_kernel<XV, GV, XT, GT, 4, false, false, 1>);
@@ -3058,7 +3062,8 @@
         const bool pr = pro == LF_PRO_BNRELU;
         auto ring = [&](auto kern) {
             if (!allow_big_lds(reinterpret_cast<const void*>(kern), 128 * 1024)) return false;
-            hipLaunchKernelGGL(kern, dim3(c.gx), dim3(256), ring_lds, st, g, a, c.pps, wb);
+            if (a.s16) hipLaunchKernelGGL(kern, dim3(c.gx), dim3(256), ring_lds, st, g, a, c.pps, wb);
+            else lf_launch(kern, dim3(c.gx), dim3(256), ring_lds, st, g, a, c.pps, wb);
             return true;
         };
         bool launched = false;
@@ -3066,7 +3071,7 @@
         else if (ring_ok) launched = pr ? ring(tapwgrad16_f32_kernel<true>) : ring(tapwgrad16_f32_kernel<false>);
         if (!launched) {
             if (a.s16) hipLaunchKernelGGL((tapwgrad16_kernel<3, true>), dim3(c.gx), dim3(256), 0, st, g, a, pro, c.pps, wb);
-            else hipLaunchKernelGGL((tapwgrad16_kernel<3, false>), dim3(c.gx), dim3(256), 0, st, g, a, pro, c.pps, wb);
+            else lf_launch(tapwgrad16_kernel<3, false>, dim3(c.gx), dim3(256), 0, st, g, a, pro, c.pps, wb);
         }
         LF_CHECK_LAUNCH("tapwgrad16");
         return 0;
@@ -3354,7 +3359,8 @@
             blocks += lf_cdiv((long)J.ntaps * J.Cs * J.Cd, 64) + ((J.bias_rows && J.bias_grad) ? lf_cdiv(J.Cd, 64) : 0);
         }
         B.blk0[LF_REDUCE_BATCH] = blocks;
-        hipLaunchKernelGGL(wgrad_reduce_batch_kernel, dim3(blocks), dim3(256), 0, st, B);
+        if (j0 > 0) lf_launch(wgrad_reduce_batch_kernel, dim3(blocks), dim3(256), 0, st, B);
+        else hipLaunchKernelGGL(wgrad_reduce_batch_kernel, dim3(blocks), dim3(256), 0, st, B);
         LF_CHECK_LAUNCH("wgrad_reduce_batch");
     }
     return 0;
diff --git a/lanedetection_end2end_amd/csrc/lf_debug.h b/lanedetection_end2end_amd/csrc/lf_debug.h
--- a/lanedetection_end2end_amd/csrc/lf_debug.h
+++ b/lanedetection_end2end_amd/csrc/lf_debug.h
@@ -35,6 +35,9 @@
 long lf_debug_bias_residual_launches(void);
 int lf_debug_conv1d_wgrad_phases(const float* x, const float* gy, int N, int H, int W, int C, int axis, int dilation,
                                  float* scratch, unsigned long long* dbg, void* stream);
+void lf_debug_set_unordered(unsigned mask);
+unsigned lf_debug_unordered_default(void);
+long lf_debug_unordered_count(int reset);
 #ifdef __cplusplus
 }
 #endif
diff --git a/lanedetection_end2end_amd/csrc/lf_eltwise.hip b/lanedetection_end2end_amd/csrc/lf_eltwise.hip
--- a/lanedetection_end2end_amd/csrc/lf_eltwise.hip
+++ b/lanedetection_end2end_amd/csrc/lf_eltwise.hip
@@ -544,7 +544,7 @@
     LF_BY_STORAGE3(s16, oct,
         hipLaunchKernelGGL((pool_concat_fwd_kernel<lf_bf16, 2>), grid, dim3(256), 0, st, as<lf_bf16>(x), N, H, W, Cin / V, as<lf_bf16>(cat), cat_pix, choff, rows, ld),
         hipLaunchKernelGGL((pool_concat_fwd_kernel<lf_bf16, 1>), grid, dim3(256), 0, st, as<lf_bf16>(x), N, H, W, Cin / V, as<lf_bf16>(cat), cat_pix, choff, rows, ld),
-        hipLaunchKernelGGL((pool_concat_fwd_kernel<float, 1>), grid, dim3(256), 0, st, x, N, H, W, Cin / V, cat, cat_pix, choff, rows, ld));
+        lf_launch(pool_concat_fwd_kernel<float, 1>, grid, dim3(256), 0, st, x, N, H, W, Cin / V, cat, cat_pix, choff, rows, ld));
     LF_CHECK_LAUNCH("pool_concat_fwd");
     return 0;
 }
@@ -574,7 +574,7 @@
     LF_BY_STORAGE3(s16, oct,
         hipLaunchKernelGGL((pool_bwd_kernel<lf_bf16, 2>), grid, dim3(256), 0, st, as<lf_bf16>(x), as<lf_bf16>(gcat), N, H, W, Cin / V, cat_pix, choff, as<lf_bf16>(gx)),
         hipLaunchKernelGGL((pool_bwd_kernel<lf_bf16, 1>), grid, dim3(256), 0, st, as<lf_bf16>(x), as<lf_bf16>(gcat), N, H, W, Cin / V, cat_pix, choff, as<lf_bf16>(gx)),
-        hipLaunchKernelGGL((pool_bwd_kernel<float, 1>), grid, dim3(256), 0, st, x, gcat, N, H, W, Cin / V, cat_pix, choff, gx));
+        lf_launch(pool_bwd_kernel<float, 1>, grid, dim3(256), 0, st, x, gcat, N, H, W, Cin / V, cat_pix, choff, gx));
     LF_CHECK_LAUNCH("pool_bwd");
     return 0;
 }
@@ -595,7 +595,7 @@
     const dim3 grid(grid_for((long)N * h * w_, 4096));
     LF_BY_STORAGE(s16,
         hipLaunchKernelGGL(head_bwd_data_kernel<lf_bf16>, grid, dim3(256), 0, st, gout, w, as<lf_bf16>(gx), N, h, w_, K),
-        hipLaunchKernelGGL(head_bwd_data_kernel<float>, grid, dim3(256), 0, st, gout, w, gx, N, h, w_, K));
+        lf_launch(head_bwd_data_kernel<float>, grid, dim3(256), 0, st, gout, w, gx, N, h, w_, K));
     LF_CHECK_LAUNCH("head_bwd_data");
     return 0;
 }
diff --git a/lanedetection_end2end_amd/csrc/lf_erfnet.hip b/lanedetection_end2end_amd/csrc/lf_erfnet.hip
--- a/lanedetection_end2end_amd/csrc/lf_erfnet.hip
+++ b/lanedetection_end2end_amd/csrc/lf_erfnet.hip
@@ -1,5 +1,6 @@
 #include <stdlib.h>
 
+#include <atomic>
 #include <vector>
 
 #include "lf_conv.h"
@@ -409,6 +410,7 @@
     mutable long wpart_used = 0, bpart_used = 0;
     mutable int last_rows = 0;
     mutable bool wgrad_launched = false;
+    mutable bool wgrad_batched = false;
     long lo = 0, hi = 0, cut = 0;
     bool no_batch = false;
     float* at(long off) const { return off < cut ? ws + (off - lo) : ws + (hi - lo) + (off - cut); }
@@ -433,6 +435,35 @@
     ~ProfScope() { if (idx >= 0) (void)hipEventRecord(c.P->prof[idx].b, pst); }
 };
 
+enum {
+    LF_UNORD_DGRAD = 1,
+    LF_UNORD_UP_FWD = 2,
+    LF_UNORD_DOWN_FWD = 4,
+    LF_UNORD_UP_BWD = 8,
+    LF_UNORD_DOWN_WGRAD = 16,
+    LF_UNORD_DOWN_DGRAD = 32,
+    LF_UNORD_REDUCE = 64,
+    LF_UNORD_HEAD = 128,
+    LF_UNORD_SITES = 255,
+    LF_UNORD_LONGEST_FIRST = 256
+};
+constexpr unsigned LF_UNORD_DEFAULT = LF_UNORD_DGRAD | LF_UNORD_UP_FWD | LF_UNORD_UP_BWD | LF_UNORD_DOWN_WGRAD | LF_UNORD_DOWN_DGRAD;
+std::atomic<unsigned> g_unordered_mask{LF_UNORD_DEFAULT};
+
+struct Group {
+    bool on, first = true;
+    Group(const Ctx& c, unsigned site, bool allowed = true)
+        : on(allowed && (g_unordered_mask.load() & site) && !c.P->prof_on && c.P->precision == 0) {}
+    template <typename F>
+    int run(F&& f, const bool* dispatched = nullptr) {
+        lf_launch_set_unordered(on && !first);
+        const int rc = f();
+        lf_launch_set_unordered(false);
+        if (!dispatched || *dispatched) first = false;
+        return rc;
+    }
+};
+
 int run_gemm(const Ctx& c, const GemmOp& op, const float* src, float* dst, const float* bias, int pro, int epi,
              LfTapArgs extra, bool beside_wgrad = false) {
     extra.src = src; extra.dst = dst; extra.bias = bias; extra.wp = c.packed(op.pack);
@@ -445,7 +476,12 @@
     }
     c.last_rows = lf_tapgemm_stat_rows_for(op.geom, extra);
     ProfScope ps(c, 0, op.geom, epi | (pro << 8), c.st);
-    if (beside_wgrad && c.wgrad_launched && !c.P->prof_on) return lf_tapgemm_launch_unordered(op.geom, extra, pro, epi, c.st);
+    if (beside_wgrad && c.wgrad_launched && !c.P->prof_on && (g_unordered_mask.load() & LF_UNORD_DGRAD)) {
+        lf_launch_set_unordered(true);
+        const int rc = lf_tapgemm_launch(op.geom, extra, pro, epi, c.st);
+        lf_launch_set_unordered(false);
+        return rc;
+    }
     return lf_tapgemm_launch(op.geom, extra, pro, epi, c.st);
 }
 
@@ -483,12 +519,13 @@
             } else {
                 LfTapArgs a = lf_no_args();
                 a.stats = stat0; a.stats_ld = lf_stat_ld(lf_tapgemm_stat_rows(L.cv[0].fwd.geom));
-                LF_TRY(run_gemm(c, L.cv[0].fwd, c.at(L.x), c.at(L.b[0]), c.params[L.cv[0].p_b], LF_PRO_NONE,
-                                c.training ? LF_EPI_STATS_SQ : 0, a));
+                Group grp(c, LF_UNORD_DOWN_FWD);
+                LF_TRY(grp.run([&] { return run_gemm(c, L.cv[0].fwd, c.at(L.x), c.at(L.b[0]), c.params[L.cv[0].p_b], LF_PRO_NONE,
+                                                     c.training ? LF_EPI_STATS_SQ : 0, a); }));
                 parts[np++] = lf_stat_part_tiles(stat0, c.last_rows, a.stats_ld, L.Cout - L.Cin, 0, c.last_rows, npo);
                 const int prows = lf_pool_rows(npo);
-                LF_TRY(lf_pool_concat_fwd(c.at(L.x), N, L.Hin, L.Win, L.Cin, c.at(L.b[0]), L.Cout, L.Cout - L.Cin,
-                                          c.training ? stat1 : nullptr, lf_stat_ld(prows), c.s16, c.st));
+                LF_TRY(grp.run([&] { return lf_pool_concat_fwd(c.at(L.x), N, L.Hin, L.Win, L.Cin, c.at(L.b[0]), L.Cout, L.Cout - L.Cin,
+                                                               c.training ? stat1 : nullptr, lf_stat_ld(prows), c.s16, c.st); }));
                 parts[np++] = {stat1, prows, L.Cin, L.Cout - L.Cin, lf_stat_ld(prows)};
             }
             LF_TRY(bn_finalize(c, L.bn[0], parts, np, (double)npo));
@@ -516,13 +553,17 @@
                              (long)L.Hout * L.Wout, c.s16, c.st));
         } else {
             LfStatPart parts[1];
-            int rows = 0, rows4 = 0;
-            for (int ph = 0; ph < 4; ++ph) rows4 += lf_tapgemm_stat_rows(L.cv[0].fph[ph].geom);
-            for (int ph = 0; ph < 4; ++ph) {
+            int rows = 0, rows4 = 0, row0[4];
+            for (int ph = 0; ph < 4; ++ph) { row0[ph] = rows4; rows4 += lf_tapgemm_stat_rows(L.cv[0].fph[ph].geom); }
+            Group grp(c, LF_UNORD_UP_FWD);
+            const bool longest_first = grp.on && (g_unordered_mask.load() & LF_UNORD_LONGEST_FIRST);
+            for (int k = 0; k < 4; ++k) {
+                const int ph = longest_first ? (k + 3) % 4 : k;
                 LfTapArgs a = lf_no_args();
-                a.stats = stat0 + rows; a.stats_ld = lf_stat_ld(rows4);
-                LF_TRY(run_gemm(c, L.cv[0].fph[ph], c.at(L.x), c.at(L.b[0]), c.params[L.cv[0].p_b], LF_PRO_NONE,
-                                c.training ? LF_EPI_STATS_SQ : 0, a));
+                a.stats = stat0 + row0[ph]; a.stats_ld = lf_stat_ld(rows4);
+                LF_TRY(grp.run([&] { return run_gemm(c, L.cv[0].fph[ph], c.at(L.x), c.at(L.b[0]), c.params[L.cv[0].p_b], LF_PRO_NONE,
+                                                     c.training ? LF_EPI_STATS_SQ : 0, a); }));
+                if (c.last_rows != lf_tapgemm_stat_rows(L.cv[0].fph[ph].geom)) return lf_fail("erfnet forward: a phase wrote %d statistics rows", c.last_rows);
                 rows += c.last_rows;
             }
             parts[0] = lf_stat_part_tiles(stat0, rows, lf_stat_ld(rows4), L.Cout, 0, rows / 4, npo / 4);
@@ -539,7 +580,7 @@
 int run_wgrad(const Ctx& c, const GemmOp& op, const ConvRef& cv, const float* x, const float* g, const float* pro_sc,
               const float* pro_sh, int bias_accumulate, bool batch_off = false, BiasChain* chain = nullptr) {
     const lf_erfnet_plan* P = c.P;
-    c.wgrad_launched = false;
+    c.wgrad_launched = c.wgrad_batched = false;
     if (!c.grads[cv.p_w]) return 0;
     hipStream_t ws = c.st;
     LfWgradArgs a;
@@ -561,6 +602,7 @@
         LF_TRY(lf_tapwgrad_launch(op.geom, a, pro_sc ? LF_PRO_BNRELU : LF_PRO_NONE, ws));
     }
     c.wgrad_launched = true;
+    c.wgrad_batched = batched;
     const LfPackEntry& e = P->packs[op.pack];
     const int nsplit = lf_tapwgrad_splits_for(op.geom, a, pro_sc ? LF_PRO_BNRELU : LF_PRO_NONE);
     if (batched) {
@@ -709,8 +751,9 @@
             }
             const bool chained = !c.no_batch && c.wpart_used + wsum <= P->wpart_all_floats[c.s16] && c.bpart_used + bsum <= P->bpart_all_floats[c.s16];
             BiasChain bc;
+            Group grp(c, LF_UNORD_UP_BWD, chained);
             for (int ph = 0; ph < 4; ++ph) {
-                if (chained) LF_TRY(run_wgrad(c, L.cv[0].fph[ph], L.cv[0], c.at(L.x), X, nullptr, nullptr, 0, false, &bc));
+                if (chained) LF_TRY(grp.run([&] { return run_wgrad(c, L.cv[0].fph[ph], L.cv[0], c.at(L.x), X, nullptr, nullptr, 0, false, &bc); }, &c.wgrad_launched));
                 else LF_TRY(run_wgrad(c, L.cv[0].fph[ph], L.cv[0], c.at(L.x), X, nullptr, nullptr, ph > 0, true));
             }
             LfTapArgs a = lf_no_args();
@@ -720,7 +763,7 @@
                 epi |= LF_EPI_ADD;
             }
             add_prep(a, epi, L.cv[0].dg[0].geom);
-            LF_TRY(run_gemm(c, L.cv[0].dg[0], X, F, nullptr, LF_PRO_NONE, epi, a));
+            LF_TRY(grp.run([&] { return run_gemm(c, L.cv[0].dg[0], X, F, nullptr, LF_PRO_NONE, epi, a); }));
             out = F;
             if (can_prep) { prepped = true; prep_rows = c.last_rows; prep_ld = a.stats_ld; }
         } else if (L.x < 0) {
@@ -732,12 +775,19 @@
             }
             out = F;
         } else {
-            LF_TRY(run_wgrad(c, L.cv[0].fwd, L.cv[0], c.at(L.x), X, nullptr, nullptr, 0));
-            LF_TRY(lf_pool_bwd(c.at(L.x), X, N, L.Hin, L.Win, L.Cin, L.Cout, L.Cout - L.Cin, F, c.s16, c.st));
-            for (int ph = 0; ph < 4; ++ph) {
+            {
+                LF_TRY(run_wgrad(c, L.cv[0].fwd, L.cv[0], c.at(L.x), X, nullptr, nullptr, 0));
+                Group grp(c, LF_UNORD_DOWN_WGRAD, c.wgrad_launched && c.wgrad_batched);
+                grp.first = false;
+                LF_TRY(grp.run([&] { return lf_pool_bwd(c.at(L.x), X, N, L.Hin, L.Win, L.Cin, L.Cout, L.Cout - L.Cin, F, c.s16, c.st); }));
+            }
+            Group grp(c, LF_UNORD_DOWN_DGRAD);
+            const bool longest_first = grp.on && (g_unordered_mask.load() & LF_UNORD_LONGEST_FIRST);
+            for (int k = 0; k < 4; ++k) {
+                const int ph = longest_first ? (k + 3) % 4 : k;
                 LfTapArgs a = lf_no_args();
                 a.add_src = F;
-                LF_TRY(run_gemm(c, L.cv[0].dg[ph], X, F, nullptr, LF_PRO_NONE, LF_EPI_ADD, a));
+                LF_TRY(grp.run([&] { return run_gemm(c, L.cv[0].dg[ph], X, F, nullptr, LF_PRO_NONE, LF_EPI_ADD, a); }));
             }
             out = F;
         }
@@ -760,10 +810,37 @@
     return 0;
 }
 
+int flush_reductions(const Ctx& c) {
+    if (c.reduce_jobs.empty()) return 0;
+    Group grp(c, LF_UNORD_REDUCE);
+    grp.first = false;
+    return grp.run([&] { return lf_wgrad_reduce_batch_launch(c.reduce_jobs.data(), (int)c.reduce_jobs.size(), c.st); });
+}
+
+int head_backward(const Ctx& c, const float* gout, int head, float* gx) {
+    const lf_erfnet_plan* P = c.P;
+    const int h = P->H / 2, w = P->W / 2, K = P->Cout + head;
+    const int pw = P->p_head_w[head], pb = P->p_head_b[head];
+    bool wgrad = false, batched = false;
+    if (c.grads[pw]) {
+        const int rows = lf_head_wgrad_rows(P->N, h, w);
+        const RowSums rs = row_sum_regions(c, (long)rows * 16 * K * 4, (long)rows * K);
+        LF_TRY(lf_head_wgrad(c.at(P->head_in), gout, rs.wrows, rs.brows, P->N, h, w, K, c.s16, c.st));
+        LF_TRY(row_sums_finish(c, rs, rows, 16 * K * 4, c.grads[pw], K, c.grads[pb]));
+        wgrad = true; batched = rs.batched;
+    }
+    Group grp(c, LF_UNORD_HEAD, wgrad && batched);
+    grp.first = false;
+    return grp.run([&] { return lf_head_bwd_data(gout, c.params[pw], gx, P->N, h, w, K, c.s16, c.st); });
+}
+
 }
 
 extern "C" {
 
+void lf_debug_set_unordered(unsigned mask) { g_unordered_mask = mask; }
+unsigned lf_debug_unordered_default(void) { return LF_UNORD_DEFAULT; }
+long lf_debug_unordered_count(int reset) { return lf_launch_unordered_count(reset); }
 
 int lf_erfnet_forward(const lf_erfnet_plan* P, const float* img, const float* const* params_host,
                       const float* const* params_dev, float* const* running_host, const float* dropmask, int training,
@@ -799,21 +876,11 @@
             return lf_fail("lf_erfnet_backward: copy of grad_encoder failed");
         c.g_enc = nullptr;
         LF_TRY(backward_layers(c, img, gA, gB, gC, ne));
-        if (!c.reduce_jobs.empty()) LF_TRY(lf_wgrad_reduce_batch_launch(c.reduce_jobs.data(), (int)c.reduce_jobs.size(), c.st));
-        return 0;
-    }
-    const int h = P->H / 2, w = P->W / 2, K = P->Cout + head;
-    const int pw = P->p_head_w[head], pb = P->p_head_b[head];
-    if (grads_host[pw]) {
-        const int rows = lf_head_wgrad_rows(P->N, h, w);
-        const RowSums rs = row_sum_regions(c, (long)rows * 16 * K * 4, (long)rows * K);
-        LF_TRY(lf_head_wgrad(c.at(P->head_in), grad_logits, rs.wrows, rs.brows, P->N, h, w, K, c.s16, c.st));
-        LF_TRY(row_sums_finish(c, rs, rows, 16 * K * 4, grads_host[pw], K, grads_host[pb]));
-    }
-    LF_TRY(lf_head_bwd_data(grad_logits, params_host[pw], gA, P->N, h, w, K, c.s16, c.st));
+        return flush_reductions(c);
+    }
+    LF_TRY(head_backward(c, grad_logits, head, gA));
     LF_TRY(backward_layers(c, img, gA, gB, gC, (int)P->layers.size()));
-    if (!c.reduce_jobs.empty()) LF_TRY(lf_wgrad_reduce_batch_launch(c.reduce_jobs.data(), (int)c.reduce_jobs.size(), c.st));
-    return 0;
+    return flush_reductions(c);
 }
 
 int lf_erfnet_profile(const lf_erfnet_plan* P, int enable) { P->prof_on = enable; return 0; }
@@ -960,21 +1027,13 @@
     float *gA = c.at(P->off_gA), *gB = c.at(P->off_gB), *gC = c.at(P->off_gC);
     const Layer& Ll = P->layers[last - 1];
     if (head >= 0) {
-        const int h = P->H / 2, w = P->W / 2, K = P->Cout + head;
-        const int pw = P->p_head_w[head], pb = P->p_head_b[head];
-        if (grads_host[pw]) {
-            const int rows = lf_head_wgrad_rows(P->N, h, w);
-            const RowSums rs = row_sum_regions(c, (long)rows * 16 * K * 4, (long)rows * K);
-            LF_TRY(lf_head_wgrad(c.at(P->head_in), gy, rs.wrows, rs.brows, P->N, h, w, K, c.s16, c.st));
-            LF_TRY(row_sums_finish(c, rs, rows, 16 * K * 4, grads_host[pw], K, grads_host[pb]));
-        }
-        LF_TRY(lf_head_bwd_data(gy, params_host[pw], gA, P->N, h, w, K, c.s16, c.st));
+        LF_TRY(head_backward(c, gy, head, gA));
     } else {
         LF_TRY(nchw_to_nhwc(gy, gA, P->N, Ll.Hout, Ll.Wout, Ll.Cout, c.s16, c.st));
     }
     float* gin = nullptr;
     LF_TRY(backward_layers(c, x, gA, gB, gC, last, first, &gin));
-    if (!c.reduce_jobs.empty()) LF_TRY(lf_wgrad_reduce_batch_launch(c.reduce_jobs.data(), (int)c.reduce_jobs.size(), c.st));
+    LF_TRY(flush_reductions(c));
     const Layer& Lf = P->layers[first];
     if (gx && first > 0) LF_TRY(nhwc_to_nchw(gin, gx, P->N, Lf.Hin, Lf.Win, Lf.Cin, c.s16, c.st));
     return 0;
diff --git a/profiles/summarize_unordered_sites.py b/profiles/summarize_unordered_sites.py
--- /dev/null
+++ b/profiles/summarize_unordered_sites.py
@@ -0,0 +1,119 @@
+import csv
+import gzip
+import re
+import sqlite3
+import statistics
+import sys
+
+GEMM = ("tapgemm_kernel", "tapgemm_lean_kernel", "tapstream_kernel")
+WGRAD = ("tapwgrad_kernel", "tapwgrad16_f32_kernel", "tapwgrad16_kernel")
+SKIP_STEPS = 6
+
+
+def short(name):
+    m = re.search(r"(\w+)\s*(<|\()", name.replace("(anonymous namespace)::", "").strip('"'))
+    return m.group(1) if m else name
+
+
+def steps_of(path):
+    if path.endswith(".db"):
+        cur = sqlite3.connect(path).cursor()
+        cols = [r[1] for r in cur.execute("pragma table_info(kernels)")]
+        name_col = "name" if "name" in cols else [c for c in cols if "name" in c][0]
+        rows = [(short(n), s, e) for n, s, e in cur.execute("select %s, start, end from kernels" % name_col)]
+    else:
+        op = gzip.open if path.endswith(".gz") else open
+        with op(path, "rt", newline="") as f:
+            rows = [(short(r["name"]), int(r["start"]), int(r["end"])) for r in csv.DictReader(f)]
+    rows.sort(key=lambda r: r[1])
+    steps, cur = [], None
+    for r in rows:
+        if r[0] == "stem_fwd_kernel":
+            if cur:
+                steps.append(cur)
+            cur = []
+        if cur is not None:
+            cur.append(r)
+    return steps
+
+
+def find_groups(step):
+    names = [r[0] for r in step]
+    head = names.index("head_fwd_kernel")
+    g = {}
+
+    def runs(kinds, lo, hi):
+        i = lo
+        while i < hi:
+            if names[i] in kinds:
+                j = i
+                while j + 1 < hi and names[j + 1] in kinds:
+                    j += 1
+                yield i, j
+                i = j + 1
+            else:
+                i += 1
+
+    up = [(i, j) for i, j in runs(GEMM, 0, head) if j - i == 3]
+    assert len(up) == 2, up
+    g["up 128->64 fwd: 4 phases"], g["up 64->16 fwd: 4 phases"] = up
+    pc = [i for i, n in enumerate(names) if n == "pool_concat_fwd_kernel"]
+    assert len(pc) == 2 and all(names[i - 1] in GEMM for i in pc)
+    g["down 16->64 fwd: conv + pool"], g["down 64->128 fwd: conv + pool"] = [(i - 1, i) for i in pc]
+    hw = names.index("head_wgrad_kernel")
+    assert names[hw + 1] == "head_bwd_data_kernel"
+    g["head bwd: wgrad + dgrad"] = (hw, hw + 1)
+    ub = [(i, j + 1) for i, j in runs(WGRAD, head, len(names)) if j - i == 3 and names[j + 1] in GEMM]
+    assert len(ub) == 2, ub
+    g["up 64->16 bwd: 4 wgrad phases + dgrad"], g["up 128->64 bwd: 4 wgrad phases + dgrad"] = ub
+    pb = [i for i, n in enumerate(names) if n == "pool_bwd_kernel"]
+    assert len(pb) == 2 and all(names[i - 1] in WGRAD and all(n in GEMM for n in names[i + 1:i + 5]) for i in pb)
+    for i, lab in zip(pb, ("down 64->128", "down 16->64")):
+        g[lab + " bwd: wgrad + pool"] = (i - 1, i)
+        g[lab + " bwd: 4 dgrad phases"] = (i + 1, i + 4)
+        g[lab + " bwd: all six"] = (i - 1, i + 4)
+    rd = [i for i, n in enumerate(names) if n == "wgrad_reduce_batch_kernel"]
+    assert rd and rd == list(range(rd[0], rd[0] + len(rd)))
+    g["end of pass: %d batched reductions" % len(rd)] = (rd[0], rd[-1])
+    g["engine, stem to last reduction"] = (0, rd[-1])
+    return g
+
+
+def spans(steps, groups, nlen):
+    out = {k: [] for k in groups}
+    for st in steps[SKIP_STEPS:]:
+        if len(st) != nlen:
+            continue
+        for k, (a, b) in groups.items():
+            seg = st[a:b + 1]
+            out[k].append((max(r[2] for r in seg) - min(r[1] for r in seg)) / 1e3)
+    return out
+
+
+def main(argv):
+    base = steps_of(argv[0])
+    ref = base[SKIP_STEPS]
+    groups = find_groups(ref)
+    traces = [("ordered", argv[0])] + [a.split("=", 1) for a in argv[1:]]
+    table = {}
+    for label, path in traces:
+        st = steps_of(path)
+        sp = spans(st, groups, len(ref))
+        starts = [s[0][1] for s in st[SKIP_STEPS:]]
+        step_us = statistics.median(b - a for a, b in zip(starts, starts[1:])) / 1e3
+        table[label] = ({k: (statistics.median(v), statistics.quantiles(v, n=4)) for k, v in sp.items()}, step_us, len(sp[next(iter(sp))]))
+    labels = [t[0] for t in traces]
+    print("# median span in us per group (first start to last end) over the steps of a run; step = stem_fwd to stem_fwd under the tracer")
+    print("%-46s" % "group" + "".join("%12s" % l for l in labels))
+    for k in groups:
+        print("%-46s" % k + "".join("%12.1f" % table[l][0][k][0] for l in labels))
+    print("%-46s" % "step under the tracer" + "".join("%12.1f" % table[l][1] for l in labels))
+    print("%-46s" % "steps read" + "".join("%12d" % table[l][2] for l in labels))
+    print("# quartiles of the first trace's spans (its own step-to-step spread)")
+    for k in groups:
+        q = table[labels[0]][0][k][1]
+        print("%-46s  q1 %.1f  q3 %.1f" % (k, q[0], q[2]))
+
+
+if __name__ == "__main__":
+    main(sys.argv[1:])
```

Result: no change. 2016 images/sec (-0.2%).
